# NVlabs/InstantSplat

Hardware: AMD Instinct MI355X
Metric: train_iters_per_sec (higher is better)
Workload: dtype f32

## Files before the change

### instantsplat_amd/csrc/api.hip

```cpp
#include <stdio.h>
#include "common.h"
#include <dlfcn.h>
#include <cstdlib>

int gs_launch_preprocess_fwd(hipStream_t, int, int, int, const float*, const float*, const float*, const float*, const float*, const float*,
                             const float*, const float*, const CamParams&, int32_t*, GsRec*, float*, uint2*, uint8_t*, float*, uint8_t*,
                             const GsPosed&, const GsPrologue&);
int gs_launch_count_tiles(hipStream_t, int, int, int, const uint2*, uint32_t*, uint32_t*, uint32_t*);
int gs_launch_preprocess_bwd(hipStream_t, int, int, int, const float*, const float*, const float*, const float*, const float*, int, int,
                             const CamParams&, const int32_t*, const GsRec*, const float*, const uint8_t*, const GsGrad*, float*, float*,
                             float*, float*, float*, float*, float*, float*, float*, const GsPosed&, float*, bool);
int gs_launch_mark_visible(hipStream_t, int, const float*, const float*, uint8_t*);
int gs_launch_scan_tiles(hipStream_t, int, const uint32_t*, uint32_t*, int32_t*, uint32_t*, uint32_t*, uint32_t*, uint32_t*, int);
int gs_launch_binning(hipStream_t, int, int, int, const float*, const uint2*, const uint32_t*, uint32_t*, uint64_t*, uint32_t*, uint32_t,
                      const uint32_t*, const uint32_t*, const uint32_t*);
int gs_launch_composite_fwd(hipStream_t, int, int, int, int, uint32_t, const uint32_t*, const uint32_t*, const GsRec*, const float*,
                            float*, float*, uint32_t*, const uint32_t*, const uint32_t*, const uint32_t*, uint4*, float4*, uint32_t,
                            const uint32_t*, unsigned long long*, uint32_t, uint32_t*, unsigned long long*, bool);
int gs_launch_composite_bwd(hipStream_t, int, int, int, uint32_t, const uint32_t*, const uint32_t*, const GsRec*, const float*,
                            const float*, const uint32_t*, const float*, GsGrad*, const float*, const uint4*,
                            const float4*, const uint32_t*, uint32_t, bool, const unsigned long long*, uint32_t, const uint32_t*,
                            unsigned long long*, const uint32_t*, float*);
int gs_launch_det_prepare(hipStream_t, int, int, int, uint32_t, const uint32_t*, const uint32_t*, const uint2*, char*, uint32_t*, float*);
int gs_launch_det_gather(hipStream_t, int, uint32_t, const char*, const float*, GsGrad*);
int gs_launch_frame_stats(hipStream_t, int, int, int, int, const uint32_t*, const uint32_t*, int64_t*);

namespace {
constexpr int PROF_KINDS = 6, PROF_MAX = 8192;
struct ProfState {
  bool on = false;
  unsigned long long* work_counters = nullptr;
  hipEvent_t ev[PROF_KINDS][PROF_MAX][2];
  int created[PROF_KINDS] = {};
  int used[PROF_KINDS] = {};
  int period = 1;
  int seen[PROF_KINDS] = {};
} g_prof;
}

GsProfScope::GsProfScope(int kind, hipStream_t stream) : s(stream) {
  if (!g_prof.on || kind < 0 || kind >= PROF_KINDS || g_prof.used[kind] >= PROF_MAX) return;
  if (g_prof.seen[kind]++ % g_prof.period != 0) return;
  const int i = g_prof.used[kind];
  if (i >= g_prof.created[kind]) {
    if (hipEventCreate(&g_prof.ev[kind][i][0]) != hipSuccess || hipEventCreate(&g_prof.ev[kind][i][1]) != hipSuccess) return;
    g_prof.created[kind] = i + 1;
  }
  (void)hipEventRecord(g_prof.ev[kind][i][0], s);
  stop = g_prof.ev[kind][i][1];
  g_prof.used[kind] = i + 1;
  active = true;
}
GsProfScope::~GsProfScope() { if (active) (void)hipEventRecord(stop, s); }
typedef GsProfScope ProfScope;

bool g_ranges_on = false;
thread_local bool g_krange_open = false;
namespace {
struct Roctx {
  int (*push)(const char*) = nullptr;
  int (*pop)() = nullptr;
  bool tried = false;
  unsigned long long pushed = 0;
} g_roctx;
bool roctx_open() {
  if (!g_roctx.tried) {
    g_roctx.tried = true;
    for (const char* name : {"librocprofiler-sdk-roctx.so", "librocprofiler-sdk-roctx.so.1", "libroctx64.so", "libroctx64.so.4"}) {
      void* h = dlopen(name, RTLD_NOW | RTLD_GLOBAL);
      if (!h) continue;
      g_roctx.push = (int (*)(const char*))dlsym(h, "roctxRangePushA");
      g_roctx.pop = (int (*)())dlsym(h, "roctxRangePop");
      if (g_roctx.push && g_roctx.pop) break;
      g_roctx.push = nullptr; g_roctx.pop = nullptr;
    }
  }
  return g_roctx.push != nullptr;
}
struct RoctxEnv {
  RoctxEnv() { const char* e = getenv("MI355GS_ROCTX"); if (e && e[0] == '1' && roctx_open()) g_ranges_on = true; }
} g_roctx_env;
}
void gs_range_push(const char* name) { ++g_roctx.pushed; (void)g_roctx.push(name); }
void gs_range_pop() { (void)g_roctx.pop(); }

void gs_log_error(const char* where, const char* what) { fprintf(stderr, "[mi355gs] %s failed: %s\n", where, what); }

static int g_scale_grad_exact = 0;
static int g_deterministic = 0;
GsKnobs gs_knobs() { return GsKnobs{gs_min_units(), g_deterministic}; }

static CamParams make_cam(const float* view, const float* proj, const float* campos, float tanfovx, float tanfovy,
                          float scale_modifier, int W, int H) {
  CamParams cp;
  cp.view = view; cp.proj = proj; cp.campos = campos;
  cp.tanfovx = tanfovx; cp.tanfovy = tanfovy;
  cp.focal_x = W / (2.0f * tanfovx); cp.focal_y = H / (2.0f * tanfovy);
  cp.scale_modifier = scale_modifier;
  cp.scale_grad_factor = g_scale_grad_exact ? scale_modifier : 1.0f;
  cp.W = W; cp.H = H;
  cp.gx = (W + GS_TILE - 1) / GS_TILE; cp.gy = (H + GS_TILE - 1) / GS_TILE;
  return cp;
}

static inline uint32_t clamp_capacity(int64_t c) { return c <= 0 ? 0u : (c > 0x7fffffffLL ? 0x7fffffffu : (uint32_t)c); }

namespace {
__global__ void k_view_consts(float* consts) {
  const int i = threadIdx.x;
  if (i < 16) consts[i] = (i % 5 == 0) ? 1.f : 0.f;
  else if (i < 19) consts[i] = 0.f;
}
}
int gs_write_view_consts(hipStream_t stream, float* consts, const char* name) {
  const int debug = 0;
  GS_KRANGE(name);
  hipLaunchKernelGGL(k_view_consts, dim3(1), dim3(64), 0, stream, consts);
  GS_CHECK_LAUNCH(name);
  return MI355GS_OK;
}


int gs_frame_project(hipStream_t stream, const GsScene& sc, const GsView& vw, const GsFrameBufs& fb, const GsFrameCtx& cx,
                     int32_t* num_rendered, uint8_t* visible, int debug) {
  GsRange range("mi355gs_raster_forward_preprocess");
  const int P = sc.P, D = sc.D, M = sc.M, W = vw.W, H = vw.H;
  if (P < 0 || W <= 0 || H <= 0 || W > 65535 * GS_TILE || H > 65535 * GS_TILE || D < 0 || D > 3) return MI355GS_EINVAL;
  if (!fb.geom || !fb.tiles || !num_rendered || !vw.view || !vw.proj || !vw.campos) return MI355GS_EINVAL;
  if (P > 0 && (!sc.means3D || !sc.opacities || !fb.radii)) return MI355GS_EINVAL;
  if (P > 0 && ((sc.shs == nullptr) == (sc.colors_precomp == nullptr))) return MI355GS_EINVAL;
  if (P > 0 && sc.shs && M < (D + 1) * (D + 1)) return MI355GS_EINVAL;
  if (sc.shs_rest && (!sc.shs || M < 2)) return MI355GS_EINVAL;
  if (P > 0 && !sc.cov3D_precomp && (!sc.scales || !sc.rotations)) return MI355GS_EINVAL;
  const GeomLayout gl(P);
  const TilesLayout tl(W, H);
  char* g = (char*)fb.geom;
  char* t = (char*)fb.tiles;
  GsPrologue pro;
  if (cx.prologue) {
    pro = *cx.prologue;
  } else {
    pro.tile_counters = (uint32_t*)(t + tl.count); pro.n_counters = (int)((tl.start - tl.count) / 4);
    if (fb.grad_scratch) { pro.grad_records = (float4*)fb.grad_scratch; pro.n_vec = gs_grad_gate_offset(P) / 16 + 2; }
    if (P <= 0) {
      if (hipMemsetAsync(t + tl.count, 0, tl.start - tl.count, stream) != hipSuccess) return MI355GS_ELAUNCH;
      if (fb.grad_scratch && hipMemsetAsync(fb.grad_scratch, 0, gs_grad_gate_offset(P) + 32, stream) != hipSuccess) return MI355GS_ELAUNCH;
    }
  }
  const CamParams cp = make_cam(vw.view, vw.proj, vw.campos, vw.tanfovx, vw.tanfovy, sc.scale_modifier, W, H);
  GS_KRANGE("preprocess_fwd");
  gs_launch_preprocess_fwd(stream, P, D, M, sc.means3D, sc.shs, sc.shs_rest, sc.colors_precomp, sc.opacities, sc.scales, sc.rotations,
                           sc.cov3D_precomp, cp, fb.radii, (GsRec*)(g + gl.rec), (float*)(g + gl.cov3D), (uint2*)(g + gl.rect),
                           (uint8_t*)(g + gl.clamped), (float*)(g + gl.depth), visible, cx.posed, pro);
  GS_CHECK_LAUNCH("preprocess_fwd");
  GS_KRANGE("count_tiles");
  gs_launch_count_tiles(stream, P, tl.T, tl.gx, (const uint2*)(g + gl.rect), (uint32_t*)(t + tl.count), (uint32_t*)(g + gl.bin_entries),
                        (uint32_t*)(g + gl.bin_n));
  GS_CHECK_LAUNCH("count_tiles");
  GS_KRANGE("scan_tiles");
  gs_launch_scan_tiles(stream, tl.T, (const uint32_t*)(t + tl.count), (uint32_t*)(t + tl.start), num_rendered,
                       (uint32_t*)(t + tl.order), (uint32_t*)(t + tl.meta), (uint32_t*)(t + tl.seg_first), (uint32_t*)(t + tl.part_first),
                       fb.knobs.min_units);
  GS_CHECK_LAUNCH("scan_tiles");
  return MI355GS_OK;
}

int gs_frame_render(hipStream_t stream, int P, const GsView& vw, const GsFrameBufs& fb, const float* bg, float* out_color, bool train,
                    int debug) {
  GsRange range(train ? "mi355gs_raster_forward_render" : "mi355gs_raster_forward_render_only");
  const int W = vw.W, H = vw.H;
  if (P < 0 || W <= 0 || H <= 0 || !fb.geom || !fb.tiles || !bg || !out_color) return MI355GS_EINVAL;
  const uint32_t cap = clamp_capacity(fb.capacity);
  if (cap > 0 && !fb.binning) return MI355GS_EINVAL;
  const GeomLayout gl(P);
  const TilesLayout tl(W, H);
  const BinningLayout bl(fb.capacity, tl.T, fb.knobs);
  const char* g = (const char*)fb.geom;
  char* t = (char*)fb.tiles;
  char* b = (char*)fb.binning;
  GS_KRANGE("binning");
  gs_launch_binning(stream, P, tl.T, tl.gx, (const float*)(g + gl.depth), (const uint2*)(g + gl.rect),
                    (const uint32_t*)(t + tl.start), (uint32_t*)(t + tl.cursor), (uint64_t*)(b + bl.keys),
                    (uint32_t*)(b + bl.list), cap, (const uint32_t*)(t + tl.order), (const uint32_t*)(g + gl.bin_entries),
                    (const uint32_t*)(g + gl.bin_n));
  GS_CHECK_LAUNCH("binning");
  {
    ProfScope prof(train ? 0 : 2, stream);
    GS_KRANGE("composite_fwd");
    gs_launch_composite_fwd(stream, tl.T, tl.gx, W, H, cap, (const uint32_t*)(t + tl.start), (const uint32_t*)(b + bl.list),
                            (const GsRec*)(g + gl.rec), bg, out_color, (float*)(t + tl.final_T), (uint32_t*)(t + tl.n_contrib),
                            (const uint32_t*)(t + tl.order), (const uint32_t*)(t + tl.seg_first), (const uint32_t*)(t + tl.part_first),
                            train ? (uint4*)(b + bl.unit_tile) : nullptr, train ? (float4*)(b + bl.bstate) : nullptr, bl.max_units,
                            (const uint32_t*)(t + tl.meta), train ? (unsigned long long*)(b + bl.hitmask) : nullptr, bl.max_chunks,
                            (uint32_t*)(t + tl.qmax), train ? g_prof.work_counters : nullptr, train);
  }
  GS_CHECK_LAUNCH("composite_fwd");
  return MI355GS_OK;
}

int gs_frame_backward(hipStream_t stream, const GsScene& sc, const GsView& vw, const GsFrameBufs& fb, const GsFrameCtx& cx,
                      const float* bg, const float* out_color, const float* dL_dpix, const GsGradOut& o, bool grad_scratch_is_clear,
                      int debug) {
  GsRange range("mi355gs_raster_backward");
  const int P = sc.P, D = sc.D, W = vw.W, H = vw.H;
  if (P < 0 || W <= 0 || H <= 0 || D < 0 || D > 3) return MI355GS_EINVAL;
  if (!fb.geom || !fb.tiles || !dL_dpix || !out_color || !fb.grad_scratch || !bg || !vw.view || !vw.proj || !vw.campos) return MI355GS_EINVAL;
  const bool outs = !(cx.pose_only && cx.posed.pose);
  if (P > 0 && (!sc.means3D || !fb.radii || (outs && (!o.means3D || !o.means2D || !o.opacities)))) return MI355GS_EINVAL;
  const int use_shs = sc.shs != nullptr, use_cov = sc.cov3D_precomp != nullptr;
  if (P > 0 && outs && use_shs && !o.shs) return MI355GS_EINVAL;
  if (sc.shs_rest && !use_shs) return MI355GS_EINVAL;
  if (P > 0 && outs && !use_shs && !o.colors) return MI355GS_EINVAL;
  if (P > 0 && !use_cov && (!sc.scales || !sc.rotations || (outs && (!o.scales || !o.rotations)))) return MI355GS_EINVAL;
  if (P > 0 && outs && use_cov && !o.cov3D) return MI355GS_EINVAL;
  if (P == 0) return MI355GS_OK;
  const uint32_t cap = clamp_capacity(fb.capacity);
  if (cap > 0 && !fb.binning) return MI355GS_EINVAL;
  const GeomLayout gl(P);
  const TilesLayout tl(W, H);
  const BinningLayout bl(fb.capacity, tl.T, fb.knobs);
  const char* g = (const char*)fb.geom;
  const char* t = (const char*)fb.tiles;
  char* b = (char*)fb.binning;
  GsGrad* grads = (GsGrad*)fb.grad_scratch;
  const size_t clear_bytes = cx.gate_tail ? gs_grad_gate_offset(P) + 8 * sizeof(float) : (size_t)P * sizeof(GsGrad);
  if (!cx.prologue && !grad_scratch_is_clear && hipMemsetAsync(grads, 0, clear_bytes, stream) != hipSuccess) return MI355GS_ELAUNCH;
  if (cap > 0) {
    const bool det = fb.knobs.det != 0;
    char* det_scratch = (char*)fb.grad_scratch + gs_grad_gate_offset(P) + 256;
    uint32_t* rowidx = det ? (uint32_t*)(b + bl.det_rowidx) : nullptr;
    float* rows = det ? (float*)(b + bl.det_rows) : nullptr;
    if (det) {
      GS_KRANGE("det_prepare");
      const int rc = gs_launch_det_prepare(stream, P, tl.T, tl.gx, cap, (const uint32_t*)(t + tl.start), (const uint32_t*)(b + bl.list),
                                           (const uint2*)(g + gl.rect), det_scratch, rowidx, rows);
      GS_CHECK_LAUNCH("det_prepare");
      if (rc != 0) return MI355GS_ELAUNCH;
    }
    {
      ProfScope prof(1, stream);
      GS_KRANGE("composite_bwd");
      gs_launch_composite_bwd(stream, tl.gx, W, H, cap, (const uint32_t*)(t + tl.start), (const uint32_t*)(b + bl.list),
                              (const GsRec*)(g + gl.rec), bg, (const float*)(t + tl.final_T), (const uint32_t*)(t + tl.n_contrib),
                              dL_dpix, grads, out_color, (const uint4*)(b + bl.unit_tile),
                              (const float4*)(b + bl.bstate), (const uint32_t*)(t + tl.meta), bl.max_units, bl.may_loop,
                              (const unsigned long long*)(b + bl.hitmask), bl.max_chunks, (const uint32_t*)(t + tl.qmax),
                              det ? nullptr : g_prof.work_counters, rowidx, rows);
    }
    GS_CHECK_LAUNCH("composite_bwd");
    if (det) {
      GS_KRANGE("det_gather");
      gs_launch_det_gather(stream, P, cap, det_scratch, rows, grads);
      GS_CHECK_LAUNCH("det_gather");
    }
  }
  const CamParams cp = make_cam(vw.view, vw.proj, vw.campos, vw.tanfovx, vw.tanfovy, sc.scale_modifier, W, H);
  GS_KRANGE("preprocess_bwd");
  gs_launch_preprocess_bwd(stream, P, D, sc.M, sc.means3D, sc.shs, sc.shs_rest, sc.scales, sc.rotations, use_shs, use_cov, cp, fb.radii,
                           (const GsRec*)(g + gl.rec), (const float*)(g + gl.cov3D), (const uint8_t*)(g + gl.clamped), grads, o.means3D,
                           o.means2D, o.shs, o.shs_rest, o.colors, o.opacities, o.scales, o.rotations, o.cov3D, cx.posed, cx.gate,
                           cx.pose_only);
  GS_CHECK_LAUNCH("preprocess_bwd");
  return MI355GS_OK;
}

extern "C" {

int mi355gs_abi_version(void) { return MI355GS_ABI_VERSION; }

const char* mi355gs_error_string(int code) {
  switch (code) {
    case MI355GS_OK: return "ok";
    case MI355GS_EINVAL: return "invalid argument";
    case MI355GS_ELAUNCH: return "HIP launch or runtime failure";
    case MI355GS_EOVERFLOW: return "instance capacity exceeded";
    default: return "unknown error";
  }
}

size_t mi355gs_raster_geom_bytes(int P) { return GeomLayout(P).total; }
size_t mi355gs_raster_tiles_bytes(int W, int H) { return (W > 0 && H > 0) ? TilesLayout(W, H).total : 0; }
size_t mi355gs_raster_binning_bytes(int64_t n, int W, int H) { return (W > 0 && H > 0) ? gs_binning_bytes(n, W, H, gs_knobs(), true) : 0; }
size_t mi355gs_raster_binning_bytes_render_only(int64_t n, int W, int H) { return (W > 0 && H > 0) ? gs_binning_bytes(n, W, H, gs_knobs(), false) : 0; }
size_t mi355gs_raster_grad_gate_offset(int P) { return gs_grad_gate_offset(P); }
size_t mi355gs_raster_grad_scratch_bytes(int P) { return gs_grad_scratch_bytes(P, g_deterministic); }

int mi355gs_raster_forward_preprocess(void* stream, int P, int D, int M, int W, int H, const float* means3D, const float* shs,
                                      const float* shs_rest, const float* colors_precomp, const float* opacities, const float* scales,
                                      float scale_modifier, const float* rotations, const float* cov3D_precomp,
                                      const float* viewmatrix, const float* projmatrix, const float* campos, float tanfovx,
                                      float tanfovy, int prefiltered, int32_t* radii, void* geom, void* tiles,
                                      int32_t* num_rendered, uint8_t* visible, void* grad_scratch, int debug) {
  (void)prefiltered;
  return gs_frame_project((hipStream_t)stream, {P, D, M, means3D, shs, shs_rest, colors_precomp, opacities, scales, rotations, cov3D_precomp, scale_modifier},
                          {W, H, viewmatrix, projmatrix, campos, tanfovx, tanfovy}, {geom, tiles, nullptr, 0, radii, grad_scratch, gs_knobs()},
                          GsFrameCtx(), num_rendered, visible, debug);
}

int mi355gs_raster_forward_render(void* stream, int P, int W, int H, int64_t capacity, const float* bg, const void* geom,
                                  void* tiles, void* binning, float* out_color, int debug) {
  return gs_frame_render((hipStream_t)stream, P, {W, H}, {const_cast<void*>(geom), tiles, binning, capacity, nullptr, nullptr, gs_knobs()}, bg,
                         out_color, true, debug);
}

int mi355gs_raster_forward_render_only(void* stream, int P, int W, int H, int64_t capacity, const float* bg, const void* geom,
                                       void* tiles, void* binning, float* out_color, int debug) {
  return gs_frame_render((hipStream_t)stream, P, {W, H}, {const_cast<void*>(geom), tiles, binning, capacity, nullptr, nullptr, gs_knobs()}, bg,
                         out_color, false, debug);
}

int mi355gs_raster_backward(void* stream, int P, int D, int M, int W, int H, const float* bg, const float* means3D,
                            const float* shs, const float* shs_rest, const float* colors_precomp, const float* opacities, const float* scales,
                            float scale_modifier, const float* rotations, const float* cov3D_precomp, const float* viewmatrix,
                            const float* projmatrix, const float* campos, float tanfovx, float tanfovy, const void* geom,
                            void* tiles, const void* binning, int64_t capacity, const int32_t* radii, const float* out_color,
                            const float* dL_dpix, void* grad_scratch, float* dL_dmeans3D, float* dL_dmeans2D, float* dL_dshs,
                            float* dL_dshs_rest, float* dL_dcolors, float* dL_dopacities, float* dL_dscales, float* dL_drotations, float* dL_dcov3D,
                            int grad_scratch_is_clear, int debug) {
  const GsGradOut o = {dL_dmeans3D, dL_dmeans2D, dL_dshs, dL_dshs_rest, dL_dcolors, dL_dopacities, dL_dscales, dL_drotations, dL_dcov3D};
  return gs_frame_backward((hipStream_t)stream, {P, D, M, means3D, shs, shs_rest, colors_precomp, opacities, scales, rotations, cov3D_precomp, scale_modifier},
                           {W, H, viewmatrix, projmatrix, campos, tanfovx, tanfovy},
                           {const_cast<void*>(geom), tiles, const_cast<void*>(binning), capacity, const_cast<int32_t*>(radii), grad_scratch, gs_knobs()},
                           GsFrameCtx(), bg, out_color, dL_dpix, o, grad_scratch_is_clear != 0, debug);
}

int mi355gs_tune_deterministic(int on) {
  const int old = g_deterministic;
  if (on >= 0) g_deterministic = on ? 1 : 0;
  return old;
}

int mi355gs_tune_scale_grad(int mode) {
  const int old = g_scale_grad_exact;
  if (mode >= 0) g_scale_grad_exact = mode ? 1 : 0;
  return old;
}

int mi355gs_raster_frame_stats(void* stream_, int W, int H, const void* tiles, int64_t* stats) {
  GS_RANGE();
  hipStream_t stream = (hipStream_t)stream_;
  const int debug = 0;
  if (W <= 0 || H <= 0 || !tiles || !stats) return MI355GS_EINVAL;
  const TilesLayout tl(W, H);
  const char* t = (const char*)tiles;
  if (hipMemsetAsync(stats, 0, 2 * sizeof(int64_t), stream) != hipSuccess) return MI355GS_ELAUNCH;
  GS_KRANGE("frame_stats");
  gs_launch_frame_stats(stream, tl.T, tl.gx, W, H, (const uint32_t*)(t + tl.start), (const uint32_t*)(t + tl.n_contrib), stats);
  GS_CHECK_LAUNCH("frame_stats");
  return MI355GS_OK;
}

int mi355gs_profile_begin(void) {
  g_prof.on = true;
  for (int k = 0; k < PROF_KINDS; ++k) g_prof.used[k] = g_prof.seen[k] = 0;
  return MI355GS_OK;
}

int mi355gs_profile_set_period(int every) {
  const int old = g_prof.period;
  if (every > 0) g_prof.period = every;
  return old;
}

int mi355gs_profile_work_counters(void* counters) {
  g_prof.work_counters = (unsigned long long*)counters;
  return MI355GS_OK;
}

int mi355gs_profile_read(int kind, double* total_ms, int* launches) {
  if (kind < 0 || kind >= PROF_KINDS || !total_ms || !launches) return MI355GS_EINVAL;
  double tot = 0.0;
  for (int i = 0; i < g_prof.used[kind]; ++i) {
    float ms = 0.f;
    if (hipEventSynchronize(g_prof.ev[kind][i][1]) != hipSuccess) return MI355GS_ELAUNCH;
    if (hipEventElapsedTime(&ms, g_prof.ev[kind][i][0], g_prof.ev[kind][i][1]) != hipSuccess) return MI355GS_ELAUNCH;
    tot += ms;
  }
  *total_ms = tot;
  *launches = g_prof.used[kind];
  return MI355GS_OK;
}

int mi355gs_profile_end(void) {
  g_prof.on = false;
  return MI355GS_OK;
}

int mi355gs_profile_ranges(int on) {
  if (on == 1) {
    if (!roctx_open()) return MI355GS_EINVAL;
    g_ranges_on = true;
  } else if (on == 0) {
    g_ranges_on = false;
  }
  return (int)(g_roctx.pushed & 0x7fffffffull);
}

int mi355gs_raster_mark_visible(void* stream_, int P, const float* means3D, const float* viewmatrix, const float* projmatrix,
                                uint8_t* present) {
  GS_RANGE();
  (void)projmatrix;
  const int debug = 0;
  void* stream = stream_;
  if (P < 0 || (P > 0 && (!means3D || !viewmatrix || !present))) return MI355GS_EINVAL;
  GS_KRANGE("mark_visible");
  gs_launch_mark_visible((hipStream_t)stream, P, means3D, viewmatrix, present);
  GS_CHECK_LAUNCH("mark_visible");
  return MI355GS_OK;
}

}
```

### instantsplat_amd/csrc/binning.hip

```cpp
#include "common.h"

namespace {

constexpr int SCAN_THREADS = 1024;
constexpr size_t SCAN_STAGE_MAX_BYTES = 48 * 1024;
constexpr int SORT_THREADS = 256;
constexpr int SORT_SMALL_CAP = GS_SORT_SMALL_CAP;
constexpr int SORT_LDS_CAP = 8192;

#ifdef GS_SCAN_PROBE
__device__ long long g_scan_probe[16];
#define SCAN_STAMP(k) do { if (threadIdx.x == 0) g_scan_probe[k] = wall_clock64(); } while (0)
#else
#define SCAN_STAMP(k) do { } while (0)
#endif
constexpr int SCAN_PER_MAX = (int)(SCAN_STAGE_MAX_BYTES / (SCAN_THREADS * 4));

template <bool STAGED>
__global__ __launch_bounds__(SCAN_THREADS) void k_scan_tiles(int T, const uint32_t* count, uint32_t* start, int32_t* num_rendered,
                                                               uint32_t* __restrict__ order, uint32_t* __restrict__ meta,
                                                               uint32_t* __restrict__ seg_first, uint32_t* __restrict__ part_first,
                                                               uint32_t min_units) {
  __shared__ uint32_t wave_tot[SCAN_THREADS / GS_WAVE];
  HIP_DYNAMIC_SHARED(uint32_t, s_stage)
  const int tid = threadIdx.x, lane = tid & 63, wave = tid >> 6;
  const int per = (T + SCAN_THREADS - 1) / SCAN_THREADS;
  const int lo = tid * per, hi = min(T, lo + per);
  SCAN_STAMP(0);
  uint32_t own[STAGED ? SCAN_PER_MAX : 1];
  if constexpr (STAGED) {
    for (int e = tid; e < T; e += SCAN_THREADS) s_stage[e] = count[e];
    __syncthreads();
#pragma unroll
    for (int k = 0; k < SCAN_PER_MAX; ++k) own[k] = lo + k < hi ? s_stage[lo + k] : 0u;
  }
  auto for_own = [&](auto&& f) {
    if constexpr (STAGED) {
#pragma unroll
      for (int k = 0; k < SCAN_PER_MAX; ++k)
        if (lo + k < hi) f(lo + k, own[k]);
    } else {
      for (int i = lo; i < hi; ++i) f(i, count[i]);
    }
  };
  auto emit = [&](uint32_t* out, auto&& value) {
    if constexpr (STAGED) {
      __syncthreads();
      for_own([&](int i, uint32_t c) { s_stage[i] = value(i, c); });
      __syncthreads();
      for (int e = tid; e < T; e += SCAN_THREADS) out[e] = s_stage[e];
    } else {
      for_own([&](int i, uint32_t c) { out[i] = value(i, c); });
    }
  };
  SCAN_STAMP(1);
  uint32_t local = 0;
  for_own([&](int, uint32_t c) { local += c; });
  const uint32_t incl = gs_wave_scan_incl_u32(local);
  if (lane == 63) wave_tot[wave] = incl;
  __syncthreads();
  uint32_t wave_off = 0, total = 0;
#pragma unroll
  for (int w = 0; w < SCAN_THREADS / GS_WAVE; ++w) {
    const uint32_t v = wave_tot[w];
    if (w < wave) wave_off += v;
    total += v;
  }
  SCAN_STAMP(2);
  if (order) {
    __shared__ uint32_t hist[SCAN_THREADS];
    __shared__ uint32_t s_max;
    uint32_t mx = 0;
    for_own([&](int, uint32_t c) { mx = max(mx, c); });
    mx = gs_wave_max_u32(mx);
    hist[tid] = 0u;
    if (tid == 0) s_max = 0u;
    __syncthreads();
    if (lane == 0) atomicMax(&s_max, mx);
    __syncthreads();
    const uint32_t cmax = max(s_max, 1u);
    const float bscale = (float)(SCAN_THREADS - 1) / (float)cmax;
    auto bucket = [&](uint32_t c) { return (uint32_t)(SCAN_THREADS - 1) - min((uint32_t)(SCAN_THREADS - 1), (uint32_t)((float)c * bscale)); };
    SCAN_STAMP(3);
    for_own([&](int, uint32_t c) { atomicAdd(&hist[bucket(c)], 1u); });
    __syncthreads();
    SCAN_STAMP(4);
    const uint32_t h = hist[tid];
    const uint32_t hi_ = gs_wave_scan_incl_u32(h);
    __shared__ uint32_t hist_wave[SCAN_THREADS / GS_WAVE];
    if (lane == 63) hist_wave[wave] = hi_;
    __syncthreads();
    uint32_t hoff = 0;
#pragma unroll
    for (int w = 0; w < SCAN_THREADS / GS_WAVE; ++w)
      if (w < wave) hoff += hist_wave[w];
    hist[tid] = hoff + hi_ - h;
    __syncthreads();
    SCAN_STAMP(5);
    if constexpr (STAGED) {
      for_own([&](int i, uint32_t c) { s_stage[atomicAdd(&hist[bucket(c)], 1u)] = (uint32_t)i; });
      __syncthreads();
      for (int e = tid; e < T; e += SCAN_THREADS) order[e] = s_stage[e];
    } else {
      for_own([&](int i, uint32_t c) { order[atomicAdd(&hist[bucket(c)], 1u)] = (uint32_t)i; });
    }
    __syncthreads();
    SCAN_STAMP(6);
  }
  if (seg_first) {
    const uint32_t level = (uint32_t)gs_unit_level_for((long long)total, (long long)min_units);
    const uint32_t chunks = 1u << level;
    const uint32_t seg_len = chunks * GS_SEG;
    static_assert((GS_SEG & (GS_SEG - 1)) == 0, "GS_SEG must be a power of two");
    const uint32_t seg_shift = level + (uint32_t)__builtin_ctz(GS_SEG), seg_mask = seg_len - 1u;
    auto units_of = [&](uint32_t c) { return (c + seg_mask) >> seg_shift; };
    auto short_of = [&](uint32_t c) { return (uint32_t)((c & seg_mask) != 0u); };
    uint32_t lseg = 0, lpart = 0;
    for_own([&](int, uint32_t c) { lseg += units_of(c); lpart += short_of(c); });
    const uint32_t iseg = gs_wave_scan_incl_u32(lseg), ipart = gs_wave_scan_incl_u32(lpart);
    __shared__ uint32_t seg_wave[SCAN_THREADS / GS_WAVE];
    __shared__ uint32_t part_wave[SCAN_THREADS / GS_WAVE];
    if (lane == 63) { seg_wave[wave] = iseg; part_wave[wave] = ipart; }
    __syncthreads();
    uint32_t soff = 0, stot = 0, poff = 0, ptot = 0;
#pragma unroll
    for (int w = 0; w < SCAN_THREADS / GS_WAVE; ++w) {
      if (w < wave) { soff += seg_wave[w]; poff += part_wave[w]; }
      stot += seg_wave[w]; ptot += part_wave[w];
    }
    uint32_t srun = soff + iseg - lseg, prun = poff + ipart - lpart;
    emit(seg_first, [&](int, uint32_t c) { const uint32_t v = srun; srun += units_of(c); return v; });
    emit(part_first, [&](int, uint32_t c) { const uint32_t v = prun; prun += short_of(c); return v; });
    if (tid == 0) { part_first[T] = ptot; meta[3] = ptot; }
    if (tid == 0) { seg_first[T] = stot; meta[1] = stot; meta[2] = chunks; }
  }
  SCAN_STAMP(7);
  uint32_t run = wave_off + incl - local;
  emit(start, [&](int, uint32_t c) { const uint32_t v = run; run += c; return v; });
  if (tid == 0) {
    start[T] = total;
    *num_rendered = (int32_t)total;
  }
  SCAN_STAMP(8);
}

constexpr int SCAN_CHUNK = 4096;

template <bool RECT>
__device__ __forceinline__ uint32_t scan_input(const uint32_t* __restrict__ in, int i, int n) {
  if (i >= n) return 0u;
  if constexpr (!RECT) return in[i];
  else {
    if (i == n - 1) return 0u;
    const uint2 r = reinterpret_cast<const uint2*>(in)[i];
    const int x0 = r.x & 0xffff, y0 = r.x >> 16, x1 = r.y & 0xffff, y1 = r.y >> 16;
    return (x1 > x0 && y1 > y0) ? (uint32_t)((x1 - x0) * (y1 - y0)) : 0u;
  }
}

template <bool RECT>
__global__ __launch_bounds__(256) void k_scan_block_sums(int n, const uint32_t* __restrict__ in, uint32_t* __restrict__ sums) {
  __shared__ uint32_t s_red[4];
  const int base = blockIdx.x * SCAN_CHUNK;
  uint32_t acc = 0;
  for (int i = threadIdx.x; i < SCAN_CHUNK; i += 256) acc += scan_input<RECT>(in, base + i, n);
#pragma unroll
  for (int m = 32; m >= 1; m >>= 1) acc += __shfl_xor(acc, m);
  if ((threadIdx.x & 63) == 0) s_red[threadIdx.x >> 6] = acc;
  __syncthreads();
  if (threadIdx.x == 0) sums[blockIdx.x] = s_red[0] + s_red[1] + s_red[2] + s_red[3];
}

template <bool RECT>
__global__ __launch_bounds__(256) void k_scan_apply(int n, const uint32_t* __restrict__ in, const uint32_t* __restrict__ block_off,
                                                    uint32_t* __restrict__ out) {
  __shared__ uint32_t s_wave[4];
  const int tid = threadIdx.x, lane = tid & 63, wave = tid >> 6;
  uint32_t run = block_off[blockIdx.x];
  for (int it = 0; it < SCAN_CHUNK / 256; ++it) {
    const int i = blockIdx.x * SCAN_CHUNK + it * 256 + tid;
    const uint32_t v = scan_input<RECT>(in, i, n);
    const uint32_t incl = gs_wave_scan_incl_u32(v);
    __syncthreads();
    if (lane == 63) s_wave[wave] = incl;
    __syncthreads();
    uint32_t woff = 0;
#pragma unroll
    for (int w = 0; w < 4; ++w) woff += w < wave ? s_wave[w] : 0u;
    if (i < n) out[i] = run + woff + incl - v;
    run += s_wave[0] + s_wave[1] + s_wave[2] + s_wave[3];
  }
}

constexpr int BIN_CHUNK = GS_BIN_CHUNK;
static_assert(BIN_CHUNK == 512, "two Gaussians per thread (own_depth selection in k_scatter_lds)");
constexpr int BIN_MAX_LDS_TILES = 16384;
static_assert(BIN_MAX_LDS_TILES <= 64 * 256, "k_count_tiles_lds keeps one bit per bin of a thread in a 64-bit mask");

__device__ __forceinline__ bool unpack_rect(uint2 r, int& x0, int& y0, int& x1, int& y1) {
  x0 = r.x & 0xffff; y0 = r.x >> 16; x1 = r.y & 0xffff; y1 = r.y >> 16;
  return x1 > x0 && y1 > y0;
}

constexpr int BIN_WIDE = 8;

constexpr int BIN_PER_THREAD = BIN_CHUNK / 256;

template <class F>
__device__ __forceinline__ void for_each_instance(int lo, int hi, const uint2 (&own)[BIN_PER_THREAD], const uint2* __restrict__ rects,
                                                  uint32_t* s_wide, uint2* s_wide_rect, uint32_t* s_nwide, F&& f) {
  const int tid = threadIdx.x;
#pragma unroll
  for (int j = 0; j < BIN_PER_THREAD; ++j) {
    const int i = lo + tid + 256 * j;
    int x0, y0, x1, y1;
    if (i >= hi || !unpack_rect(own[j], x0, y0, x1, y1)) continue;
    if ((x1 - x0) * (y1 - y0) > BIN_WIDE) {
      const uint32_t slot = atomicAdd(s_nwide, 1u);
      s_wide[slot] = (uint32_t)i; s_wide_rect[slot] = own[j];
      continue;
    }
    for (int y = y0; y < y1; ++y)
      for (int x = x0; x < x1; ++x) f(i, j, x, y);
  }
  __syncthreads();
  const int nwide = (int)*s_nwide;
  for (int q = tid >> 4; q < nwide; q += 16) {
    const int i = (int)s_wide[q];
    int x0, y0, x1, y1;
    unpack_rect(s_wide_rect[q], x0, y0, x1, y1);
    const int w = x1 - x0, n = w * (y1 - y0);
    const int dq = 16 / w, dr = 16 - dq * w;
    int j = tid & 15, row = j / w, col = j - row * w;
    for (; j < n; j += 16) {
      f(i, -1, x0 + col, y0 + row);
      col += dr; row += dq;
      if (col >= w) { col -= w; row += 1; }
    }
  }
}

__global__ __launch_bounds__(256) void k_count_tiles_lds(int P, int T, int gx, const uint2* __restrict__ rects,
                                                          uint32_t* __restrict__ tile_count, uint32_t* __restrict__ entries,
                                                          uint32_t* __restrict__ entry_n) {
  HIP_DYNAMIC_SHARED(uint32_t, s_bins)
  __shared__ uint32_t s_wide[BIN_CHUNK];
  __shared__ uint2 s_wide_rect[BIN_CHUNK];
  __shared__ uint32_t s_nwide;
  __shared__ uint32_t s_wave_nz[4];
  const int tid = threadIdx.x;
  const int lo = blockIdx.x * BIN_CHUNK, hi = min(P, lo + BIN_CHUNK);
  uint2 own[BIN_PER_THREAD];
#pragma unroll
  for (int j = 0; j < BIN_PER_THREAD; ++j) own[j] = rects[min(lo + tid + 256 * j, P - 1)];
  for (int t = tid; t < T; t += 256) s_bins[t] = 0;
  if (tid == 0) s_nwide = 0;
  __syncthreads();
  for_each_instance(lo, hi, own, rects, s_wide, s_wide_rect, &s_nwide, [&](int, int, int x, int y) { atomicAdd(&s_bins[y * gx + x], 1u); });
  __syncthreads();
  unsigned long long mask = 0ull;
  {
    int k = 0;
    for (int t = tid; t < T; t += 256, ++k) {
      const uint32_t c = s_bins[t];
      if (c) { atomicAdd(&tile_count[t], c); mask |= 1ull << k; }
    }
  }
  const uint32_t nz = (uint32_t)__popcll(mask);
  const uint32_t incl = gs_wave_scan_incl_u32(nz);
  if ((tid & 63) == 63) s_wave_nz[tid >> 6] = incl;
  __syncthreads();
  uint32_t off = incl - nz, total = 0;
#pragma unroll
  for (int w = 0; w < 4; ++w) {
    if (w < (tid >> 6)) off += s_wave_nz[w];
    total += s_wave_nz[w];
  }
  if (tid == 0) entry_n[blockIdx.x] = total <= (uint32_t)GS_BIN_ENTRIES ? total : 0xffffffffu;
  if (total > (uint32_t)GS_BIN_ENTRIES) return;
  uint32_t* mine = entries + (size_t)blockIdx.x * GS_BIN_ENTRIES + off;
  while (mask) {
    const int t = tid + 256 * (__ffsll((long long)mask) - 1);
    mask &= mask - 1ull;
    *mine++ = (uint32_t)t | (s_bins[t] << 16);
  }
}

__global__ __launch_bounds__(256) void k_scatter_lds(int P, int T, int gx, const float* __restrict__ depths,
                                                      const uint2* __restrict__ rects, const uint32_t* __restrict__ start,
                                                      uint32_t* __restrict__ cursor, uint64_t* __restrict__ keys, uint32_t capacity,
                                                      const uint32_t* __restrict__ entries, const uint32_t* __restrict__ entry_n) {
  HIP_DYNAMIC_SHARED(uint32_t, s_bins)
  __shared__ uint32_t s_wide[BIN_CHUNK];
  __shared__ uint2 s_wide_rect[BIN_CHUNK];
  __shared__ uint32_t s_nwide;
  const int tid = threadIdx.x;
  const int lo = blockIdx.x * BIN_CHUNK, hi = min(P, lo + BIN_CHUNK);
  uint2 own[BIN_PER_THREAD];
  uint32_t own_depth[BIN_PER_THREAD];
#pragma unroll
  for (int j = 0; j < BIN_PER_THREAD; ++j) {
    const int ic = min(lo + tid + 256 * j, P - 1);
    own[j] = rects[ic];
    own_depth[j] = __float_as_uint(depths[ic]);
  }
  const uint32_t n_entries = entry_n[blockIdx.x];
  if (n_entries != 0xffffffffu) {
    const uint32_t* mine = entries + (size_t)blockIdx.x * GS_BIN_ENTRIES;
    for (uint32_t e0 = 0; e0 < n_entries; e0 += 1024) {
      uint32_t en[4], r[4], st[4];
#pragma unroll
      for (int j = 0; j < 4; ++j) {
        const uint32_t e = e0 + tid + 256 * j;
        en[j] = e < n_entries ? mine[e] : 0u;
      }
#pragma unroll
      for (int j = 0; j < 4; ++j) {
        r[j] = 0u; st[j] = 0u;
        if (en[j]) { r[j] = atomicAdd(&cursor[en[j] & 0xffffu], en[j] >> 16); st[j] = start[en[j] & 0xffffu]; }
      }
#pragma unroll
      for (int j = 0; j < 4; ++j)
        if (en[j]) s_bins[en[j] & 0xffffu] = st[j] + r[j];
    }
  } else {
    for (int t = tid; t < T; t += 256) s_bins[t] = 0;
    if (tid == 0) s_nwide = 0;
    __syncthreads();
    for_each_instance(lo, hi, own, rects, s_wide, s_wide_rect, &s_nwide, [&](int, int, int x, int y) { atomicAdd(&s_bins[y * gx + x], 1u); });
    __syncthreads();
    for (int t0 = 0; t0 < T; t0 += 1024) {
      uint32_t c[4], r[4], st[4];
#pragma unroll
      for (int j = 0; j < 4; ++j) {
        const int t = t0 + tid + 256 * j;
        c[j] = t < T ? s_bins[t] : 0u;
      }
#pragma unroll
      for (int j = 0; j < 4; ++j) {
        const int t = t0 + tid + 256 * j;
        r[j] = 0u; st[j] = 0u;
        if (c[j]) { r[j] = atomicAdd(&cursor[t], c[j]); st[j] = start[t]; }
      }
#pragma unroll
      for (int j = 0; j < 4; ++j)
        if (c[j]) s_bins[t0 + tid + 256 * j] = st[j] + r[j];
    }
  }
  if (tid == 0) s_nwide = 0;
  __syncthreads();
  for_each_instance(lo, hi, own, rects, s_wide, s_wide_rect, &s_nwide, [&](int i, int j, int x, int y) {
    const uint32_t depth = j == 0 ? own_depth[0] : (j == 1 ? own_depth[BIN_PER_THREAD - 1] : __float_as_uint(depths[i]));
    const uint64_t key = ((uint64_t)depth << 32) | (uint32_t)i;
    const uint32_t pos = atomicAdd(&s_bins[y * gx + x], 1u);
    if (pos < capacity) keys[pos] = key;
  });
}

__global__ __launch_bounds__(256) void k_count_tiles_direct(int P, int gx, const uint2* __restrict__ rects,
                                                             uint32_t* __restrict__ tile_count) {
  const int i = blockIdx.x * blockDim.x + threadIdx.x;
  if (i >= P) return;
  int x0, y0, x1, y1;
  if (!unpack_rect(rects[i], x0, y0, x1, y1)) return;
  for (int y = y0; y < y1; ++y)
    for (int x = x0; x < x1; ++x) atomicAdd(&tile_count[y * gx + x], 1u);
}

__global__ __launch_bounds__(256) void k_scatter_direct(int P, int gx, const float* __restrict__ depths, const uint2* __restrict__ rects,
                                                         const uint32_t* __restrict__ start, uint32_t* __restrict__ cursor,
                                                         uint64_t* __restrict__ keys, uint32_t capacity) {
  const int i = blockIdx.x * blockDim.x + threadIdx.x;
  if (i >= P) return;
  int x0, y0, x1, y1;
  if (!unpack_rect(rects[i], x0, y0, x1, y1)) return;
  const uint64_t key = ((uint64_t)__float_as_uint(depths[i]) << 32) | (uint32_t)i;
  for (int y = y0; y < y1; ++y)
    for (int x = x0; x < x1; ++x) {
      const int t = y * gx + x;
      const uint32_t pos = start[t] + atomicAdd(&cursor[t], 1u);
      if (pos < capacity) keys[pos] = key;
    }
}

template <class KeyPtr>
__device__ __forceinline__ void bitonic_sort_any(KeyPtr a, int n, int tid, int nthreads) {
  int np2 = 1;
  while (np2 < n) np2 <<= 1;
  const int half = np2 >> 1;
  for (int k = 2; k <= np2; k <<= 1) {
    const int hk = k >> 1;
    for (int t = tid; t < half; t += nthreads) {
      const int blk = t / hk, off = t - blk * hk;
      const int i = blk * k + off, j = blk * k + (k - 1 - off);
      if (j < n) {
        const uint64_t x = a[i], y = a[j];
        if (x > y) { a[i] = y; a[j] = x; }
      }
    }
    __syncthreads();
    for (int d = hk >> 1; d >= 1; d >>= 1) {
      for (int t = tid; t < half; t += nthreads) {
        const int i = (t / d) * (2 * d) + (t % d), j = i + d;
        if (j < n) {
          const uint64_t x = a[i], y = a[j];
          if (x > y) { a[i] = y; a[j] = x; }
        }
      }
      __syncthreads();
    }
  }
}

template <int CTRL>
__device__ __forceinline__ uint32_t sort_dpp(uint32_t v) {
  return (uint32_t)__builtin_amdgcn_update_dpp(0, (int)v, CTRL, 0xF, 0xF, true);
}
template <int LM>
__device__ __forceinline__ uint32_t lane_xchg32(uint32_t v) {
  if constexpr (LM >= 16) return (uint32_t)__builtin_amdgcn_ds_bpermute((int)(((threadIdx.x & 63) ^ LM) << 2), (int)v);
  else if constexpr (LM == 1) return sort_dpp<0xB1>(v);
  else if constexpr (LM == 2) return sort_dpp<0x4E>(v);
  else if constexpr (LM == 3) return sort_dpp<0x1B>(v);
  else if constexpr (LM == 4) {
    const int lo = __builtin_amdgcn_update_dpp(0, (int)v, 0x104, 0xF, 0x5, false);
    return (uint32_t)__builtin_amdgcn_update_dpp(lo, (int)v, 0x114, 0xF, 0xA, false);
  }
  else if constexpr (LM == 7) return sort_dpp<0x141>(v);
  else if constexpr (LM == 8) return sort_dpp<0x128>(v);
  else {
    static_assert(LM == 15, "lane mask of a bitonic network inside a wave64");
    return sort_dpp<0x140>(v);
  }
}
template <int LM>
__device__ __forceinline__ uint64_t lane_xchg64(uint64_t v) {
  return ((uint64_t)lane_xchg32<LM>((uint32_t)(v >> 32)) << 32) | lane_xchg32<LM>((uint32_t)v);
}

template <int E, int KK>
__device__ __forceinline__ void sort_flip_stage(uint64_t (&k)[E], uint64_t* __restrict__ s_keys, int base) {
  constexpr int m = KK - 1;
  if constexpr (KK <= E) {
#pragma unroll
    for (int e = 0; e < E; ++e) {
      const int pe = e ^ (m & (E - 1));
      if (e < pe) { const uint64_t a = k[e], b = k[pe]; if (a > b) { k[e] = b; k[pe] = a; } }
    }
  } else if constexpr (KK <= 64 * E) {
    constexpr int lm = (m / E) & 63;
    uint64_t other[E];
#pragma unroll
    for (int e = 0; e < E; ++e) other[e] = lane_xchg64<lm>(k[E - 1 - e]);
    const bool lower = (base & (KK >> 1)) == 0;
#pragma unroll
    for (int e = 0; e < E; ++e) { const uint64_t a = k[e], b = other[e]; k[e] = ((b < a) == lower) ? b : a; }
  } else {
    __syncthreads();
#pragma unroll
    for (int e = 0; e < E; ++e) s_keys[base + e] = k[e];
    __syncthreads();
    const bool lower = (base & (KK >> 1)) == 0;
#pragma unroll
    for (int e = 0; e < E; ++e) { const uint64_t a = k[e], b = s_keys[(base + e) ^ m]; k[e] = ((b < a) == lower) ? b : a; }
  }
}

template <int E, int D>
__device__ __forceinline__ void sort_disperse_from(uint64_t (&k)[E], uint64_t* __restrict__ s_keys, int base) {
  if constexpr (D >= 1) {
    if constexpr (D < E) {
#pragma unroll
      for (int e = 0; e < E; ++e) {
        const int pe = e ^ D;
        if (e < pe) { const uint64_t a = k[e], b = k[pe]; if (a > b) { k[e] = b; k[pe] = a; } }
      }
    } else if constexpr (D < 64 * E) {
      const bool lower = (base & D) == 0;
#pragma unroll
      for (int e = 0; e < E; ++e) { const uint64_t a = k[e], b = lane_xchg64<D / E>(a); k[e] = ((b < a) == lower) ? b : a; }
    } else {
      __syncthreads();
#pragma unroll
      for (int e = 0; e < E; ++e) s_keys[base + e] = k[e];
      __syncthreads();
      const bool lower = (base & D) == 0;
#pragma unroll
      for (int e = 0; e < E; ++e) { const uint64_t a = k[e], b = s_keys[(base + e) ^ D]; k[e] = ((b < a) == lower) ? b : a; }
    }
    sort_disperse_from<E, D / 2>(k, s_keys, base);
  }
}

template <int E, int KK, int NP2>
__device__ __forceinline__ void sort_merge_from(uint64_t (&k)[E], uint64_t* __restrict__ s_keys, int base) {
  if constexpr (KK <= NP2) {
    sort_flip_stage<E, KK>(k, s_keys, base);
    sort_disperse_from<E, KK / 4>(k, s_keys, base);
    sort_merge_from<E, KK * 2, NP2>(k, s_keys, base);
  }
}

template <int E>
__device__ __forceinline__ void sort_tile_regs(uint64_t* __restrict__ s_keys, const uint64_t* keys, uint32_t* __restrict__ list,
                                               uint32_t s, int n, uint64_t* keys_out = nullptr) {
  const int tid = threadIdx.x, lane = tid & 63, wave = tid >> 6;
  const int base = wave * (64 * E) + lane * E;
  uint64_t k[E];
#pragma unroll
  for (int e = 0; e < E; ++e) k[e] = (base + e < n) ? keys[s + base + e] : ~0ull;
  sort_merge_from<E, 2, SORT_THREADS * E>(k, s_keys, base);
  if (keys_out) {
#pragma unroll
    for (int e = 0; e < E; ++e)
      if (base + e < n) keys_out[s + base + e] = k[e];
  } else {
#pragma unroll
    for (int e = 0; e < E; ++e)
      if (base + e < n) list[s + base + e] = (uint32_t)k[e];
  }
}

template <int NMAX>
__device__ __forceinline__ uint32_t sort_count_below(const uint64_t* __restrict__ run, int n, uint64_t key) {
  int lo = 0;
#pragma unroll
  for (int step = NMAX; step >= 1; step >>= 1)
    if (lo + step <= n && run[lo + step - 1] < key) lo += step;
  return (uint32_t)lo;
}
template <int EA, int EB>
__device__ __forceinline__ void sort_tile_two_runs(uint64_t* __restrict__ s_keys, const uint64_t* keys, uint32_t* __restrict__ list,
                                                   uint32_t s, int n) {
  constexpr int NA = SORT_THREADS * EA, NBMAX = SORT_THREADS * EB;
  static_assert(NA + NBMAX <= SORT_SMALL_CAP, "both sorted runs are parked in the kernel's LDS array");
  const int tid = threadIdx.x, lane = tid & 63, wave = tid >> 6;
  const int base_a = wave * (64 * EA) + lane * EA, base_b = wave * (64 * EB) + lane * EB, nb = n - NA;
  uint64_t ka[EA], kb[EB];
#pragma unroll
  for (int e = 0; e < EA; ++e) ka[e] = keys[s + base_a + e];
#pragma unroll
  for (int e = 0; e < EB; ++e) kb[e] = (base_b + e < nb) ? keys[s + NA + base_b + e] : ~0ull;
  sort_merge_from<EA, 2, NA>(ka, s_keys, base_a);
  sort_merge_from<EB, 2, NBMAX>(kb, s_keys, base_b);
  __syncthreads();
#pragma unroll
  for (int e = 0; e < EA; ++e) s_keys[base_a + e] = ka[e];
#pragma unroll
  for (int e = 0; e < EB; ++e) s_keys[NA + base_b + e] = kb[e];
  __syncthreads();
#pragma unroll
  for (int e = 0; e < EA; ++e) list[s + base_a + e + sort_count_below<NBMAX>(s_keys + NA, nb, ka[e])] = (uint32_t)ka[e];
#pragma unroll
  for (int e = 0; e < EB; ++e)
    if (base_b + e < nb) list[s + base_b + e + sort_count_below<NA>(s_keys, NA, kb[e])] = (uint32_t)kb[e];
}

__device__ __forceinline__ void sort_long_tile(uint64_t* __restrict__ s_keys, uint64_t* keys, uint32_t* __restrict__ list, uint32_t s, int n) {
  constexpr int RUN = SORT_SMALL_CAP, E = RUN / SORT_THREADS;
  const int nrun = (n + RUN - 1) / RUN, tid = threadIdx.x;
  for (int r = 0; r < nrun; ++r) {
    __syncthreads();
    sort_tile_regs<E>(s_keys, keys, list, s + (uint32_t)r * RUN, min(RUN, n - r * RUN), keys);
  }
  for (int r = 0; r < nrun; ++r) {
    const int rn = min(RUN, n - r * RUN);
    uint64_t k[E];
    uint32_t rank[E];
    __syncthreads();
#pragma unroll
    for (int e = 0; e < E; ++e) {
      const int i = tid * E + e;
      k[e] = i < rn ? keys[s + (uint32_t)r * RUN + i] : ~0ull;
      rank[e] = (uint32_t)i;
    }
    for (int r2 = 0; r2 < nrun; ++r2) {
      if (r2 == r) continue;
      const int n2 = min(RUN, n - r2 * RUN);
      __syncthreads();
      for (int i = tid; i < n2; i += SORT_THREADS) s_keys[i] = keys[s + (uint32_t)r2 * RUN + i];
      __syncthreads();
#pragma unroll
      for (int e = 0; e < E; ++e) {
        int lo = 0, hi = n2;
        while (lo < hi) {
          const int mid = (lo + hi) >> 1;
          if (s_keys[mid] < k[e]) lo = mid + 1; else hi = mid;
        }
        rank[e] += (uint32_t)lo;
      }
    }
#pragma unroll
    for (int e = 0; e < E; ++e)
      if (tid * E + e < rn) list[s + rank[e]] = (uint32_t)k[e];
  }
}

__device__ __forceinline__ void sort_one_tile(int tile, const uint32_t* __restrict__ start, uint64_t* keys,
                                              uint32_t* __restrict__ list, uint32_t capacity) {
  __shared__ uint64_t s_keys[SORT_SMALL_CAP];
  const uint32_t s = min(start[tile], capacity), e = min(start[tile + 1], capacity);
  const int n = (int)(e - s);
  if (n <= 0) return;
  if (n <= SORT_THREADS) sort_tile_regs<1>(s_keys, keys, list, s, n);
  else if (n <= SORT_THREADS * 2) sort_tile_regs<2>(s_keys, keys, list, s, n);
  else if (n <= SORT_THREADS * 3) sort_tile_two_runs<2, 1>(s_keys, keys, list, s, n);
  else if (n <= SORT_THREADS * 4) sort_tile_regs<4>(s_keys, keys, list, s, n);
  else if (n <= SORT_THREADS * 5) sort_tile_two_runs<4, 1>(s_keys, keys, list, s, n);
  else if (n <= SORT_THREADS * 6) sort_tile_two_runs<4, 2>(s_keys, keys, list, s, n);
  else if (n <= SORT_SMALL_CAP) sort_tile_regs<8>(s_keys, keys, list, s, n);
  else if (n <= SORT_LDS_CAP) sort_long_tile(s_keys, keys, list, s, n);
  else {
    uint64_t* seg = keys + s;
    bitonic_sort_any(seg, n, (int)threadIdx.x, SORT_THREADS);
    for (int i = threadIdx.x; i < n; i += SORT_THREADS) list[s + i] = (uint32_t)seg[i];
  }
}

__global__ __launch_bounds__(SORT_THREADS) void k_sort_tiles(int T, const uint32_t* __restrict__ start, uint64_t* keys,
                                                              uint32_t* __restrict__ list, uint32_t capacity,
                                                              const uint32_t* __restrict__ order) {
  sort_one_tile((int)order[blockIdx.x], start, keys, list, capacity);
}

}

static int g_min_units = GS_MIN_UNITS;
extern "C" int mi355gs_tune_min_units(int min_units) {
  const int old = g_min_units;
  if (min_units > 0) g_min_units = min_units;
  return old;
}
int gs_min_units() { return g_min_units; }

int gs_launch_scan_tiles(hipStream_t stream, int T, const uint32_t* count, uint32_t* start, int32_t* num_rendered, uint32_t* order,
                         uint32_t* meta, uint32_t* seg_first, uint32_t* part_first, int min_units) {
  const size_t stage_bytes = (size_t)((T + SCAN_THREADS - 1) / SCAN_THREADS) * SCAN_THREADS * 4;
  if (T > SCAN_THREADS && stage_bytes <= SCAN_STAGE_MAX_BYTES)
    hipLaunchKernelGGL(k_scan_tiles<true>, dim3(1), dim3(SCAN_THREADS), stage_bytes, stream, T, count, start, num_rendered, order, meta,
                       seg_first, part_first, (uint32_t)min_units);
  else
    hipLaunchKernelGGL(k_scan_tiles<false>, dim3(1), dim3(SCAN_THREADS), 0, stream, T, count, start, num_rendered, order, meta, seg_first,
                       part_first, (uint32_t)min_units);
  return 0;
}

template <bool RECT>
static int scan_large(hipStream_t stream, int n, const uint32_t* in, uint32_t* out, uint32_t* block_sums, int32_t* total) {
  const int nb = (n + SCAN_CHUNK - 1) / SCAN_CHUNK;
  hipLaunchKernelGGL(k_scan_block_sums<RECT>, dim3(nb), dim3(256), 0, stream, n, in, block_sums);
  hipLaunchKernelGGL(k_scan_tiles<false>, dim3(1), dim3(SCAN_THREADS), 0, stream, nb, (const uint32_t*)block_sums, block_sums, total,
                     (uint32_t*)nullptr, (uint32_t*)nullptr, (uint32_t*)nullptr, (uint32_t*)nullptr, 0u);
  hipLaunchKernelGGL(k_scan_apply<RECT>, dim3(nb), dim3(256), 0, stream, n, in, (const uint32_t*)block_sums, out);
  return 0;
}
int gs_launch_scan_large(hipStream_t stream, int n, const uint32_t* in, uint32_t* out, uint32_t* block_sums, int32_t* total) {
  return scan_large<false>(stream, n, in, out, block_sums, total);
}
int gs_launch_scan_rect_areas(hipStream_t stream, int P, const uint2* rects, uint32_t* off, uint32_t* block_sums, int32_t* total) {
  return scan_large<true>(stream, P + 1, reinterpret_cast<const uint32_t*>(rects), off, block_sums, total);
}

int gs_launch_count_tiles(hipStream_t stream, int P, int T, int gx, const uint2* rects, uint32_t* tile_count, uint32_t* entries,
                          uint32_t* entry_n) {
  if (P <= 0) return 0;
  if (T <= BIN_MAX_LDS_TILES) {
    GsProfScope prof(5, stream);
    hipLaunchKernelGGL(k_count_tiles_lds, dim3((P + BIN_CHUNK - 1) / BIN_CHUNK), dim3(256), (size_t)T * 4, stream, P, T, gx, rects, tile_count,
                       entries, entry_n);
  }
  else
    hipLaunchKernelGGL(k_count_tiles_direct, dim3((P + 255) / 256), dim3(256), 0, stream, P, gx, rects, tile_count);
  return 0;
}

int gs_launch_binning(hipStream_t stream, int P, int T, int gx, const float* depths, const uint2* rects, const uint32_t* start,
                      uint32_t* cursor, uint64_t* keys, uint32_t* list, uint32_t capacity, const uint32_t* order, const uint32_t* entries,
                      const uint32_t* entry_n) {
  if (P <= 0 || capacity == 0) return 0;
  if (T <= BIN_MAX_LDS_TILES)
    hipLaunchKernelGGL(k_scatter_lds, dim3((P + BIN_CHUNK - 1) / BIN_CHUNK), dim3(256), (size_t)T * 4, stream, P, T, gx, depths, rects,
                       start, cursor, keys, capacity, entries, entry_n);
  else
    hipLaunchKernelGGL(k_scatter_direct, dim3((P + 255) / 256), dim3(256), 0, stream, P, gx, depths, rects, start, cursor, keys, capacity);
  {
    GsProfScope prof(4, stream);
    hipLaunchKernelGGL(k_sort_tiles, dim3(T), dim3(SORT_THREADS), 0, stream, T, start, keys, list, capacity, order);
  }
  return 0;
}
```

### instantsplat_amd/csrc/common.h

```cpp
#pragma once
#include <hip/hip_runtime.h>
#include <stdint.h>
#include <stddef.h>
#include "../../include/mi355gs.h"
#include <type_traits>

#define GS_LOG2E 1.4426950408889634f
#define GS_TILE 16
#define GS_TILE_PIX 256
#define GS_WAVE 64

struct alignas(16) GsRec {
  float4 q0;
  float4 q1;
  float4 q2;
};

struct alignas(16) GsGrad {
  float4 g0;
  float4 g1;
  float4 g2;
};

static inline size_t gs_align(size_t x) { return (x + 255) & ~(size_t)255; }

struct GsCarver {
  char* base;
  size_t off = 0;
  template <class T> T* take(size_t n) {
    T* p = base ? (T*)(base + off) : nullptr;
    off += gs_align(n * sizeof(T));
    return p;
  }
};
int gs_write_view_consts(hipStream_t stream, float* consts, const char* name);

constexpr int GS_BIN_CHUNK = 512;
constexpr int GS_BIN_ENTRIES = 1024;

struct GeomLayout {
  size_t rec, cov3D, rect, clamped, depth, bin_entries, bin_n, total;
  __host__ explicit GeomLayout(int P) {
    size_t n = P > 0 ? (size_t)P : 1, o = 0;
    rec = o; o += gs_align(n * sizeof(GsRec));
    cov3D = o; o += gs_align(n * 6 * sizeof(float));
    rect = o; o += gs_align(n * sizeof(uint2));
    clamped = o; o += gs_align(n);
    depth = o; o += gs_align(n * sizeof(float));
    const size_t chunks = (n + GS_BIN_CHUNK - 1) / GS_BIN_CHUNK;
    bin_entries = o; o += gs_align(chunks * GS_BIN_ENTRIES * sizeof(uint32_t));
    bin_n = o; o += gs_align(chunks * sizeof(uint32_t));
    total = o;
  }
};

constexpr int GS_SORT_SMALL_CAP = 2048;

constexpr int GS_UNIT_LEVELS = 4;
__host__ __device__ inline int gs_unit_level_for(long long instances, long long min_units) {
  int level = 0;
  while (level + 1 < GS_UNIT_LEVELS && (instances >> (7 + level)) >= min_units) ++level;
  return level;
}
struct GsKnobs {
  int min_units;
  int det;
};
GsKnobs gs_knobs();
struct DetScratchLayout {
  size_t off, block_sums, total;
  __host__ explicit DetScratchLayout(int P) {
    const size_t n = (size_t)(P > 0 ? P : 1) + 1;
    size_t o = 0;
    off = o; o += gs_align((n + 1) * 4);
    block_sums = o; o += gs_align(((n + 4095) / 4096 + 2) * 4);
    total = o;
  }
};
int gs_min_units();
constexpr int GS_MIN_UNITS = 40960;

struct TilesLayout {
  size_t count, start, cursor, final_T, n_contrib, order, seg_first, part_first, meta, qmax, total;
  int gx, gy, T;
  __host__ TilesLayout(int W, int H) {
    gx = (W + GS_TILE - 1) / GS_TILE; gy = (H + GS_TILE - 1) / GS_TILE; T = gx * gy;
    size_t o = 0, npix = (size_t)W * H;
    count = o; o += gs_align((size_t)T * 4);
    cursor = o; o += gs_align((size_t)T * 4);
    start = o; o += gs_align(((size_t)T + 1) * 4);
    final_T = o; o += gs_align(npix * 4);
    n_contrib = o; o += gs_align(npix * 4);
    order = o; o += gs_align((size_t)T * 4);
    seg_first = o; o += gs_align(((size_t)T + 1) * 4);
    part_first = o; o += gs_align(((size_t)T + 1) * 4);
    meta = o; o += gs_align(16);
    qmax = o; o += gs_align((size_t)T * 4 * 4);
    total = o;
  }
};

constexpr int GS_SEG = 64;

struct BinningLayout {
  size_t keys, list, unit_tile, bstate, hitmask, det_rows, det_rowidx, total;
  uint32_t max_chunks;
  uint32_t max_units;
  bool may_loop;
  __host__ BinningLayout(int64_t R, int T, const GsKnobs& knobs) {
    size_t n = R > 0 ? (size_t)R : 1, o = 0;
    keys = o; o += gs_align(n * 8);
    list = o; o += gs_align(n * 4);
    const size_t mu = (size_t)knobs.min_units, top = (size_t)GS_SEG << (GS_UNIT_LEVELS - 1);
    const size_t by_chunks = (n + GS_SEG - 1) / GS_SEG, by_rule = 2 * mu + 1, by_top = (n + top - 1) / top;
    const size_t lim = by_chunks < by_rule ? by_chunks : by_rule;
    may_loop = gs_unit_level_for((long long)n, (long long)mu) > 0;
    max_units = (uint32_t)((lim > by_top ? lim : by_top) + (size_t)(T > 0 ? T : 1));
    unit_tile = o; o += gs_align((size_t)max_units * 16);
    bstate = o; o += gs_align((size_t)max_units * 256 * sizeof(float4));
    max_chunks = (uint32_t)(by_chunks + 8 * (size_t)(T > 0 ? T : 1) + 8);
    hitmask = o; o += gs_align((size_t)max_chunks * 4 * sizeof(uint64_t));
    det_rows = det_rowidx = o;
    if (knobs.det) {
      det_rows = o; o += gs_align(n * sizeof(GsGrad));
      det_rowidx = o; o += gs_align(n * 4);
    }
    total = o;
  }
};


__device__ __forceinline__ float3 gs_tp43(const float* m, float3 p) {
  return make_float3(m[0] * p.x + m[4] * p.y + m[8] * p.z + m[12], m[1] * p.x + m[5] * p.y + m[9] * p.z + m[13],
                     m[2] * p.x + m[6] * p.y + m[10] * p.z + m[14]);
}
__device__ __forceinline__ float4 gs_tp44(const float* m, float3 p) {
  return make_float4(m[0] * p.x + m[4] * p.y + m[8] * p.z + m[12], m[1] * p.x + m[5] * p.y + m[9] * p.z + m[13],
                     m[2] * p.x + m[6] * p.y + m[10] * p.z + m[14], m[3] * p.x + m[7] * p.y + m[11] * p.z + m[15]);
}

struct CamParams {
  const float* view;
  const float* proj;
  const float* campos;
  float tanfovx, tanfovy, focal_x, focal_y, scale_modifier;
  float scale_grad_factor;
  int W, H, gx, gy;
};

template <int CTRL, int ROW_MASK = 0xF, class T>
__device__ __forceinline__ T gs_dpp(T v) {
  static_assert(sizeof(T) == 4 || sizeof(T) == 8, "one or two 32-bit moves");
  uint32_t w[sizeof(T) / 4];
  __builtin_memcpy(w, &v, sizeof(T));
  for (size_t i = 0; i < sizeof(T) / 4; ++i) w[i] = (uint32_t)__builtin_amdgcn_update_dpp(0, (int)w[i], CTRL, ROW_MASK, 0xF, false);
  __builtin_memcpy(&v, w, sizeof(T));
  return v;
}
template <class T>
__device__ __forceinline__ T gs_wave_sum_row3(T v) {
  v += gs_dpp<0xB1>(v);
  v += gs_dpp<0x4E>(v);
  v += gs_dpp<0x141>(v);
  v += gs_dpp<0x140>(v);
  v += gs_dpp<0x142, 0xA>(v);
  v += gs_dpp<0x143, 0xC>(v);
  return v;
}
__device__ __forceinline__ double gs_wave_sum_row3_f64(double v) { return gs_wave_sum_row3(v); }

__device__ __forceinline__ void gs_finish_two_means(int nblocks, double inv_n, const float* __restrict__ partial, float& mean0, float& mean1) {
  __shared__ double s_a[16], s_b[16];
  double a = 0.0, b = 0.0;
  for (int i = threadIdx.x; i < nblocks; i += 1024) { a += (double)partial[2 * i]; b += (double)partial[2 * i + 1]; }
  a = gs_wave_sum_row3(a); b = gs_wave_sum_row3(b);
  if ((threadIdx.x & 63) == 63) { s_a[threadIdx.x >> 6] = a; s_b[threadIdx.x >> 6] = b; }
  __syncthreads();
  if (threadIdx.x != 0) return;
  double ta = 0.0, tb = 0.0;
  for (int w = 0; w < 16; ++w) { ta += s_a[w]; tb += s_b[w]; }
  mean0 = (float)(ta * inv_n); mean1 = (float)(tb * inv_n);
}
__device__ __forceinline__ float gs_l1_ssim_loss(float lambda_dssim, float l1_mean, float ssim_mean) {
  return (1.0f - lambda_dssim) * l1_mean + lambda_dssim * (1.0f - ssim_mean);
}

typedef float gs_v2f __attribute__((vector_size(8)));
__device__ __forceinline__ gs_v2f gs_fma2(gs_v2f a, gs_v2f b, gs_v2f c) { return a * b + c; }

__device__ __forceinline__ uint32_t gs_wave_max_u32(uint32_t v) {
  auto dpp = [](uint32_t x, auto ctrl) { return (uint32_t)__builtin_amdgcn_update_dpp(0, (int)x, decltype(ctrl)::value, 0xF, 0xF, true); };
  v = max(v, dpp(v, std::integral_constant<int, 0xB1>{}));
  v = max(v, dpp(v, std::integral_constant<int, 0x4E>{}));
  v = max(v, dpp(v, std::integral_constant<int, 0x141>{}));
  v = max(v, dpp(v, std::integral_constant<int, 0x140>{}));
  const auto a = __builtin_amdgcn_permlane16_swap(v, v, false, false);
  v = max(a[0], a[1]);
  const auto b = __builtin_amdgcn_permlane32_swap(v, v, false, false);
  return max(b[0], b[1]);
}

__device__ __forceinline__ uint32_t gs_wave_scan_incl_u32(uint32_t v) {
  auto up = [](uint32_t x, auto ctrl, auto rows) {
    return (uint32_t)__builtin_amdgcn_update_dpp(0, (int)x, decltype(ctrl)::value, decltype(rows)::value, 0xF, false);
  };
  using all = std::integral_constant<int, 0xF>;
  v += up(v, std::integral_constant<int, 0x111>{}, all{});
  v += up(v, std::integral_constant<int, 0x112>{}, all{});
  v += up(v, std::integral_constant<int, 0x114>{}, all{});
  v += up(v, std::integral_constant<int, 0x118>{}, all{});
  v += up(v, std::integral_constant<int, 0x142>{}, std::integral_constant<int, 0xA>{});
  v += up(v, std::integral_constant<int, 0x143>{}, std::integral_constant<int, 0xC>{});
  return v;
}

__device__ __forceinline__ float gs_sum_rows(float v) {
  const unsigned u = __float_as_uint(v);
  const auto a = __builtin_amdgcn_permlane16_swap(u, u, false, false);
  const float s = __uint_as_float(a[0]) + __uint_as_float(a[1]);
  const unsigned w = __float_as_uint(s);
  const auto b = __builtin_amdgcn_permlane32_swap(w, w, false, false);
  return __uint_as_float(b[0]) + __uint_as_float(b[1]);
}

__device__ __forceinline__ uint32_t gs_physical_cu() {
  const uint32_t hw = __builtin_amdgcn_s_getreg(4 | (31 << 11));
  const uint32_t xcc = __builtin_amdgcn_s_getreg(20 | (3 << 11));
  return ((xcc & 7u) << 6) | (((hw >> 13) & 3u) << 4) | ((hw >> 8) & 15u);
}

extern thread_local bool g_krange_open;
void gs_range_pop();
#define GS_CHECK_LAUNCH(name)                                                   \
  do {                                                                          \
    if (g_krange_open) { g_krange_open = false; gs_range_pop(); }               \
    hipError_t e_ = hipGetLastError();                                          \
    if (e_ == hipSuccess && debug) e_ = hipStreamSynchronize((hipStream_t)stream); \
    if (e_ != hipSuccess) {                                                     \
      gs_log_error(name, hipGetErrorString(e_));                                \
      return MI355GS_ELAUNCH;                                                   \
    }                                                                           \
  } while (0)

void gs_log_error(const char* where, const char* what);

extern bool g_ranges_on;
void gs_range_push(const char* name);
void gs_range_pop();
struct GsRange {
  bool active;
  explicit GsRange(const char* name) : active(g_ranges_on) { if (active) gs_range_push(name); }
  ~GsRange() { if (active) gs_range_pop(); }
  GsRange(const GsRange&) = delete;
  GsRange& operator=(const GsRange&) = delete;
};
#define GS_RANGE() GsRange gs_range_(__func__)
extern thread_local bool g_krange_open;
#define GS_KRANGE(name) do { if (g_ranges_on) { gs_range_push(name); g_krange_open = true; } } while (0)

struct GsProfScope {
  hipStream_t s; hipEvent_t stop; bool active = false;
  GsProfScope(int kind, hipStream_t stream);
  ~GsProfScope();
};


struct GsPrologue {
  float4* grad_records = nullptr; size_t n_vec = 0;
  uint32_t* tile_counters = nullptr; int n_counters = 0;
  float* g_poses = nullptr; int n_pose = 0;
  float* pose_scratch = nullptr;
  float* adam_scratch = nullptr;
};
struct GsPosed {
  const float* pose = nullptr;
  float* acc = nullptr;
  float* partial = nullptr;
};
enum { GS_GATE_XYZ = 0, GS_GATE_SH = 1, GS_GATE_SH_REST = 2, GS_GATE_OPACITY = 3, GS_GATE_SCALING = 4, GS_GATE_ROT = 5, GS_GATE_POSE = 6 };

struct GsScene {
  int P, D, M;
  const float *means3D, *shs, *shs_rest, *colors_precomp, *opacities, *scales, *rotations, *cov3D_precomp;
  float scale_modifier;
};
struct GsView {
  int W, H;
  const float *view, *proj, *campos;
  float tanfovx, tanfovy;
};
struct GsFrameBufs {
  void *geom, *tiles, *binning;
  int64_t capacity;
  int32_t* radii;
  void* grad_scratch;
  GsKnobs knobs;
};
struct GsFrameCtx {
  const GsPrologue* prologue = nullptr;
  GsPosed posed;
  float* gate = nullptr;
  bool gate_tail = false;
  bool pose_only = false;
};
struct GsGradOut { float *means3D, *means2D, *shs, *shs_rest, *colors, *opacities, *scales, *rotations, *cov3D; };
static inline size_t gs_grad_gate_offset(int P) { return gs_align((size_t)(P > 0 ? P : 1) * sizeof(GsGrad)); }
static inline size_t gs_grad_scratch_bytes(int P, int det) { return gs_grad_gate_offset(P) + 256 + (det ? DetScratchLayout(P).total : 0); }
static inline size_t gs_binning_bytes(int64_t n, int W, int H, const GsKnobs& k, bool train) {
  const BinningLayout bl(n, TilesLayout(W, H).T, k);
  return train ? bl.total : bl.unit_tile;
}
static inline const uint32_t* gs_frame_count(const void* tiles, int W, int H) {
  const TilesLayout tl(W, H);
  return (const uint32_t*)((const char*)tiles + tl.start) + tl.T;
}
int gs_frame_project(hipStream_t stream, const GsScene& sc, const GsView& vw, const GsFrameBufs& fb, const GsFrameCtx& cx,
                     int32_t* num_rendered, uint8_t* visible, int debug);
int gs_frame_render(hipStream_t stream, int P, const GsView& vw, const GsFrameBufs& fb, const float* bg, float* out_color, bool train,
                    int debug);
int gs_frame_backward(hipStream_t stream, const GsScene& sc, const GsView& vw, const GsFrameBufs& fb, const GsFrameCtx& cx,
                      const float* bg, const float* out_color, const float* dL_dpix, const GsGradOut& out, bool grad_scratch_is_clear,
                      int debug);

struct GsAdamFused {
  uint32_t* live; uint32_t seq;
  const uint32_t* commit_count; unsigned long long commit_capacity;
  uint32_t* commit_poison;
};
int gs_adam_multi(hipStream_t stream, int ntensors, const int64_t* numel, const int32_t* row, float* const* params,
                  const float* const* grads, float* const* exp_avg, float* const* exp_avg_sq, const float* const* per_point_lr,
                  const float* lr, float beta1, float beta2, float eps, const int32_t* step, float* scratch, const float* gate,
                  const int32_t* gate_index, uint32_t* live, uint32_t seq, const GsAdamFused* fused);

struct GsFrozenScene {
  int P, M, W, H;
  int64_t capacity;
  const float *xyz, *f_dc, *f_rest, *opacity, *scaling, *rotation;
  char *geom, *tiles, *binning;
  float *image, *consts;
  int32_t *radii, *num_rendered;

  bool init(int P_, int M_, int W_, int H_, int64_t capacity_, const float* xyz_, const float* f_dc_, const float* f_rest_,
            const float* opacity_, const float* scaling_, const float* rotation_, const void* workspace) {
    if (P_ <= 0 || M_ < 1 || M_ > 16 || W_ <= 0 || H_ <= 0 || W_ > 65535 * GS_TILE || H_ > 65535 * GS_TILE || capacity_ <= 0 || !workspace)
      return false;
    if (!xyz_ || !f_dc_ || (M_ > 1 && !f_rest_) || !opacity_ || !scaling_ || !rotation_) return false;
    P = P_; M = M_; W = W_; H = H_; capacity = capacity_;
    xyz = xyz_; f_dc = f_dc_; f_rest = M_ > 1 ? f_rest_ : nullptr; opacity = opacity_; scaling = scaling_; rotation = rotation_;
    return true;
  }
  void carve(GsCarver& c, const GsKnobs& knobs, bool train) {
    geom = c.take<char>(GeomLayout(P).total);
    tiles = c.take<char>(TilesLayout(W, H).total);
    binning = c.take<char>(gs_binning_bytes(capacity, W, H, knobs, train));
    image = c.take<float>(3 * (size_t)W * H);
    consts = c.take<float>(32);
    radii = c.take<int32_t>((size_t)P);
    num_rendered = c.take<int32_t>(1);
  }
  bool degree_ok(int D) const { return D >= 0 && D <= 3 && (D + 1) * (D + 1) <= M; }
  GsScene scene(int D) const {
    return {P, D, D == 0 ? 1 : M, xyz, f_dc, D == 0 ? nullptr : f_rest, nullptr, opacity, scaling, rotation, nullptr, 1.0f};
  }
  GsView view(const float* proj, float tanfovx, float tanfovy) const { return {W, H, consts, proj, consts + 16, tanfovx, tanfovy}; }
  GsFrameBufs bufs(const GsKnobs& knobs, void* grad_scratch) const { return {geom, tiles, binning, capacity, radii, grad_scratch, knobs}; }
  const uint32_t* count() const { return gs_frame_count(tiles, W, H); }
};
```

### instantsplat_amd/csrc/path.hip

```cpp
#include <stdlib.h>
#include <string.h>
#include "common.h"

namespace {

constexpr int RGB8_VEC = 4;

struct Rgb8x4 { uint32_t a, b, c; };

__device__ __forceinline__ uint32_t rgb8_quantize(float x) {
#pragma clang fp contract(off)
  const float y = x * 255.0f;
  const float z = y + 0.5f;
  return z > 0.0f ? (uint32_t)fminf(z, 255.0f) : 0u;
}

__global__ __launch_bounds__(256) void k_rgb8_from_planar(int npix, const float* __restrict__ img, uint8_t* __restrict__ out,
                                                          const uint32_t* __restrict__ count_src, int32_t* __restrict__ count_dst) {
  if (count_dst && blockIdx.x == 0 && threadIdx.x == 0) *count_dst = (int32_t)*count_src;
  const int i0 = (int)(blockIdx.x * 256u + threadIdx.x) * RGB8_VEC;
  if (i0 >= npix) return;
  const float* __restrict__ r = img;
  const float* __restrict__ g = img + npix;
  const float* __restrict__ b = img + 2 * (size_t)npix;
  if ((npix & (RGB8_VEC - 1)) == 0 && (((uintptr_t)img & 15) | ((uintptr_t)out & 3)) == 0) {
    const float4 R = reinterpret_cast<const float4*>(r)[i0 >> 2], G = reinterpret_cast<const float4*>(g)[i0 >> 2],
                 B = reinterpret_cast<const float4*>(b)[i0 >> 2];
    Rgb8x4 p;
    p.a = rgb8_quantize(R.x) | rgb8_quantize(G.x) << 8 | rgb8_quantize(B.x) << 16 | rgb8_quantize(R.y) << 24;
    p.b = rgb8_quantize(G.y) | rgb8_quantize(B.y) << 8 | rgb8_quantize(R.z) << 16 | rgb8_quantize(G.z) << 24;
    p.c = rgb8_quantize(B.z) | rgb8_quantize(R.w) << 8 | rgb8_quantize(G.w) << 16 | rgb8_quantize(B.w) << 24;
    *reinterpret_cast<Rgb8x4*>(out + 3 * (size_t)i0) = p;
  } else {
    const int i1 = min(npix, i0 + RGB8_VEC);
    for (int i = i0; i < i1; ++i) {
      out[3 * (size_t)i] = (uint8_t)rgb8_quantize(r[i]);
      out[3 * (size_t)i + 1] = (uint8_t)rgb8_quantize(g[i]);
      out[3 * (size_t)i + 2] = (uint8_t)rgb8_quantize(b[i]);
    }
  }
}

bool rgb8_size_ok(int W, int H) { return W > 0 && H > 0 && (long long)W * H <= 0x7fffffffLL - 256 * RGB8_VEC; }

int launch_rgb8(hipStream_t stream, int W, int H, const float* img, uint8_t* out, const uint32_t* count_src, int32_t* count_dst) {
  const int debug = 0;
  const int npix = W * H;
  const int per_block = 256 * RGB8_VEC;
  GS_KRANGE("rgb8_from_planar");
  hipLaunchKernelGGL(k_rgb8_from_planar, dim3((npix + per_block - 1) / per_block), dim3(256), 0, stream, npix, img, out, count_src,
                     count_dst);
  GS_CHECK_LAUNCH("rgb8_from_planar");
  return MI355GS_OK;
}

typedef GsFrozenScene Path;

size_t carve(Path& t, void* workspace) {
  GsCarver c{(char*)workspace};
  t.carve(c, gs_knobs(), false);
  return c.off;
}

}

extern "C" {

int mi355gs_rgb8_from_planar(void* stream, int H, int W, const float* img, uint8_t* out) {
  GS_RANGE();
  if (!img || !out || !rgb8_size_ok(W, H)) return MI355GS_EINVAL;
  return launch_rgb8((hipStream_t)stream, W, H, img, out, nullptr, nullptr);
}

size_t mi355gs_path_workspace_bytes(int P, int W, int H, int64_t capacity) {
  if (P <= 0 || !rgb8_size_ok(W, H) || capacity <= 0) return 0;
  Path t;
  memset(&t, 0, sizeof(t));
  t.P = P; t.W = W; t.H = H; t.capacity = capacity;
  return carve(t, nullptr);
}

void* mi355gs_path_create(int P, int M, int W, int H, int64_t capacity, const float* xyz, const float* f_dc, const float* f_rest,
                          const float* opacity, const float* scaling, const float* rotation, void* workspace) {
  if (!rgb8_size_ok(W, H)) return nullptr;
  Path* t = (Path*)calloc(1, sizeof(Path));
  if (!t) return nullptr;
  if (!t->init(P, M, W, H, capacity, xyz, f_dc, f_rest, opacity, scaling, rotation, workspace)) { free(t); return nullptr; }
  carve(*t, workspace);
  return t;
}

void mi355gs_path_destroy(void* handle) { free(handle); }

int mi355gs_path_render(void* handle, void* stream_, int sh_degree, const float* projmatrix, float tanfovx, float tanfovy,
                        const float* bg, const float* poses, int first, int n, uint8_t* frames, int32_t* counts) {
  GS_RANGE();
  Path* t = (Path*)handle;
  hipStream_t stream = (hipStream_t)stream_;
  if (!t || !t->degree_ok(sh_degree) || !projmatrix || !bg || !poses || !frames || !counts) return MI355GS_EINVAL;
  if (first < 0 || n < 0 || n > 0x7fffffff - first) return MI355GS_EINVAL;
  if (n == 0) return MI355GS_OK;
  int rc;
  if ((rc = gs_write_view_consts(stream, t->consts, "view_consts"))) return rc;
  const GsScene scene = t->scene(sh_degree);
  const GsView view = t->view(projmatrix, tanfovx, tanfovy);
  const GsFrameBufs bufs = t->bufs(gs_knobs(), nullptr);
  const size_t frame_bytes = (size_t)t->W * t->H * 3;
  for (int i = first; i < first + n; ++i) {
    GsFrameCtx cx;
    cx.posed.pose = poses + 7 * (size_t)i;
    if ((rc = gs_frame_project(stream, scene, view, bufs, cx, t->num_rendered, nullptr, 0))) return rc;
    if ((rc = gs_frame_render(stream, t->P, view, bufs, bg, t->image, false, 0))) return rc;
    if ((rc = launch_rgb8(stream, t->W, t->H, t->image, frames + frame_bytes * (size_t)i, t->count(), counts + i))) return rc;
  }
  return MI355GS_OK;
}

}
```

### instantsplat_amd/csrc/preprocess.hip

```cpp
#include "pose_math.h"

namespace {

constexpr float SH_C0 = 0.28209479177387814f;
constexpr float SH_C1 = 0.4886025119029199f;
constexpr float SH_C2_0 = 1.0925484305920792f, SH_C2_1 = -1.0925484305920792f, SH_C2_2 = 0.31539156525252005f,
                SH_C2_3 = -1.0925484305920792f, SH_C2_4 = 0.5462742152960396f;
constexpr float SH_C3_0 = -0.5900435899266435f, SH_C3_1 = 2.890611442640554f, SH_C3_2 = -0.4570457994644658f,
                SH_C3_3 = 0.3731763325901154f, SH_C3_4 = -0.4570457994644658f, SH_C3_5 = 1.445305721320277f,
                SH_C3_6 = -0.5900435899266435f;

struct Cov2D {
  float a, b, c;
};

struct Ewa {
  float tx, ty, tz, xmul, ymul;
  float M[6];
};

__device__ __forceinline__ Ewa ewa_setup(float3 pv, const float* view, const CamParams& cp) {
  Ewa e;
  const float limx = 1.3f * cp.tanfovx, limy = 1.3f * cp.tanfovy;
  const float txtz = pv.x / pv.z, tytz = pv.y / pv.z;
  e.tx = fminf(limx, fmaxf(-limx, txtz)) * pv.z;
  e.ty = fminf(limy, fmaxf(-limy, tytz)) * pv.z;
  e.tz = pv.z;
  e.xmul = (txtz < -limx || txtz > limx) ? 0.f : 1.f;
  e.ymul = (tytz < -limy || tytz > limy) ? 0.f : 1.f;
  const float j00 = cp.focal_x / e.tz, j02 = -(cp.focal_x * e.tx) / (e.tz * e.tz);
  const float j11 = cp.focal_y / e.tz, j12 = -(cp.focal_y * e.ty) / (e.tz * e.tz);
  e.M[0] = j00 * view[0] + j02 * view[2];
  e.M[1] = j00 * view[4] + j02 * view[6];
  e.M[2] = j00 * view[8] + j02 * view[10];
  e.M[3] = j11 * view[1] + j12 * view[2];
  e.M[4] = j11 * view[5] + j12 * view[6];
  e.M[5] = j11 * view[9] + j12 * view[10];
  return e;
}

__device__ __forceinline__ Cov2D ewa_cov2d(const Ewa& e, const float* cov) {
  const float* M = e.M;
  float MS[6];
  MS[0] = M[0] * cov[0] + M[1] * cov[1] + M[2] * cov[2];
  MS[1] = M[0] * cov[1] + M[1] * cov[3] + M[2] * cov[4];
  MS[2] = M[0] * cov[2] + M[1] * cov[4] + M[2] * cov[5];
  MS[3] = M[3] * cov[0] + M[4] * cov[1] + M[5] * cov[2];
  MS[4] = M[3] * cov[1] + M[4] * cov[3] + M[5] * cov[4];
  MS[5] = M[3] * cov[2] + M[4] * cov[4] + M[5] * cov[5];
  Cov2D c;
  c.a = MS[0] * M[0] + MS[1] * M[1] + MS[2] * M[2] + 0.3f;
  c.b = MS[0] * M[3] + MS[1] * M[4] + MS[2] * M[5];
  c.c = MS[3] * M[3] + MS[4] * M[4] + MS[5] * M[5] + 0.3f;
  return c;
}

__device__ __forceinline__ void quat_to_R(float r, float x, float y, float z, float* R) {
  R[0] = 1.f - 2.f * (y * y + z * z); R[1] = 2.f * (x * y - r * z); R[2] = 2.f * (x * z + r * y);
  R[3] = 2.f * (x * y + r * z); R[4] = 1.f - 2.f * (x * x + z * z); R[5] = 2.f * (y * z - r * x);
  R[6] = 2.f * (x * z - r * y); R[7] = 2.f * (y * z + r * x); R[8] = 1.f - 2.f * (x * x + y * y);
}

template <int NB>
__device__ __forceinline__ void sh_basis(float x, float y, float z, float* b) {
  b[0] = SH_C0;
  if (NB > 1) { b[1] = -SH_C1 * y; b[2] = SH_C1 * z; b[3] = -SH_C1 * x; }
  if (NB > 4) {
    const float xx = x * x, yy = y * y, zz = z * z, xy = x * y, yz = y * z, xz = x * z;
    b[4] = SH_C2_0 * xy; b[5] = SH_C2_1 * yz; b[6] = SH_C2_2 * (2.f * zz - xx - yy);
    b[7] = SH_C2_3 * xz; b[8] = SH_C2_4 * (xx - yy);
    if (NB > 9) {
      b[9] = SH_C3_0 * y * (3.f * xx - yy); b[10] = SH_C3_1 * xy * z;
      b[11] = SH_C3_2 * y * (4.f * zz - xx - yy); b[12] = SH_C3_3 * z * (2.f * zz - 3.f * xx - 3.f * yy);
      b[13] = SH_C3_4 * x * (4.f * zz - xx - yy); b[14] = SH_C3_5 * z * (xx - yy);
      b[15] = SH_C3_6 * x * (xx - 3.f * yy);
    }
  }
}

template <int NB>
__device__ __forceinline__ float3 sh_eval(const float* sh , float x, float y, float z) {
  float b[NB];
  sh_basis<NB>(x, y, z, b);
  float3 acc = make_float3(0.f, 0.f, 0.f);
#pragma unroll
  for (int k = 0; k < NB; ++k) {
    acc.x += b[k] * sh[3 * k]; acc.y += b[k] * sh[3 * k + 1]; acc.z += b[k] * sh[3 * k + 2];
  }
  return acc;
}

template <bool POSED, int D>
__global__ __launch_bounds__(256) void k_preprocess_fwd(
    int P, int M, const float* __restrict__ means3D, const float* __restrict__ shs, const float* __restrict__ shs_rest,
    const float* __restrict__ colors_precomp, const float* __restrict__ opacities, const float* __restrict__ scales,
    const float* __restrict__ rotations, const float* __restrict__ cov3D_precomp, CamParams cp,
    int32_t* __restrict__ radii, GsRec* __restrict__ recs, float* __restrict__ cov3Ds, uint2* __restrict__ rects,
    uint8_t* __restrict__ clamped, float* __restrict__ depths, uint8_t* __restrict__ visible, GsPosed posed, GsPrologue pro) {
  const int i = blockIdx.x * blockDim.x + threadIdx.x;
  {
    const size_t gid = (size_t)i, stride = (size_t)gridDim.x * blockDim.x;
    if (pro.grad_records) {
      const float4 z = make_float4(0.f, 0.f, 0.f, 0.f);
      for (size_t k = gid; k < pro.n_vec; k += stride) pro.grad_records[k] = z;
    }
    if (pro.tile_counters)
      for (size_t k = gid; k < (size_t)pro.n_counters; k += stride) pro.tile_counters[k] = 0u;
    if (pro.g_poses && gid < (size_t)pro.n_pose) pro.g_poses[gid] = 0.f;
    if (pro.pose_scratch && gid < 32) pro.pose_scratch[gid] = 0.f;
    if (pro.adam_scratch && gid < 8) pro.adam_scratch[gid] = 0.f;
  }
  if (i >= P) return;
  radii[i] = 0;
  if (visible) visible[i] = 0;
  rects[i] = make_uint2(0u, 0u);
  const float* view = cp.view;
  const float* proj = cp.proj;
  PoseMat pm;
  if (POSED) pm = load_pose(posed.pose);
  float3 m = make_float3(means3D[3 * (size_t)i], means3D[3 * (size_t)i + 1], means3D[3 * (size_t)i + 2]);
  if (POSED) m = pose_mean(pm, m.x, m.y, m.z);
  const float3 pv = gs_tp43(view, m);
  if (pv.z <= 0.2f) return;
  const float4 ph = gs_tp44(proj, m);
  const float pw = 1.0f / (ph.w + 0.0000001f);
  const float ndcx = ph.x * pw, ndcy = ph.y * pw;

  float cov[6];
  if (cov3D_precomp) {
#pragma unroll
    for (int k = 0; k < 6; ++k) cov[k] = cov3D_precomp[6 * (size_t)i + k];
  } else {
    float4 q = *reinterpret_cast<const float4*>(rotations + 4 * (size_t)i);
    float sc[3] = {scales[3 * (size_t)i], scales[3 * (size_t)i + 1], scales[3 * (size_t)i + 2]};
    if (POSED) {
      q = pose_rot(pm, q);
#pragma unroll
      for (int k = 0; k < 3; ++k) sc[k] = pose_scale(sc[k]);
    }
    float R[9];
    quat_to_R(q.x, q.y, q.z, q.w, R);
    const float s0 = cp.scale_modifier * sc[0], s1 = cp.scale_modifier * sc[1], s2 = cp.scale_modifier * sc[2];
    float L[9];
#pragma unroll
    for (int r = 0; r < 3; ++r) { L[3 * r] = R[3 * r] * s0; L[3 * r + 1] = R[3 * r + 1] * s1; L[3 * r + 2] = R[3 * r + 2] * s2; }
    cov[0] = L[0] * L[0] + L[1] * L[1] + L[2] * L[2];
    cov[1] = L[0] * L[3] + L[1] * L[4] + L[2] * L[5];
    cov[2] = L[0] * L[6] + L[1] * L[7] + L[2] * L[8];
    cov[3] = L[3] * L[3] + L[4] * L[4] + L[5] * L[5];
    cov[4] = L[3] * L[6] + L[4] * L[7] + L[5] * L[8];
    cov[5] = L[6] * L[6] + L[7] * L[7] + L[8] * L[8];
  }
#pragma unroll
  for (int k = 0; k < 6; ++k) cov3Ds[6 * (size_t)i + k] = cov[k];

  const Ewa e = ewa_setup(pv, view, cp);
  const Cov2D c2 = ewa_cov2d(e, cov);
  const float det = c2.a * c2.c - c2.b * c2.b;
  if (det == 0.0f) return;
  const float det_inv = 1.f / det;
  const float ca = c2.c * det_inv, cb = -c2.b * det_inv, cc = c2.a * det_inv;
  const float mid = 0.5f * (c2.a + c2.c);
  const float sq = sqrtf(fmaxf(0.1f, mid * mid - det));
  const float radius = ceilf(3.f * sqrtf(fmaxf(mid + sq, mid - sq)));
  const float px = ((ndcx + 1.0f) * cp.W - 1.0f) * 0.5f, py = ((ndcy + 1.0f) * cp.H - 1.0f) * 0.5f;
  const int rminx = min(cp.gx, max(0, (int)((px - radius) / GS_TILE)));
  const int rminy = min(cp.gy, max(0, (int)((py - radius) / GS_TILE)));
  const int rmaxx = min(cp.gx, max(0, (int)((px + radius + GS_TILE - 1) / GS_TILE)));
  const int rmaxy = min(cp.gy, max(0, (int)((py + radius + GS_TILE - 1) / GS_TILE)));
  if ((rmaxx - rminx) * (rmaxy - rminy) == 0) return;

  float3 rgb;
  uint8_t clamp_bits = 0;
  if (colors_precomp) {
    rgb = make_float3(colors_precomp[3 * (size_t)i], colors_precomp[3 * (size_t)i + 1], colors_precomp[3 * (size_t)i + 2]);
  } else {
    float dx = m.x - cp.campos[0], dy = m.y - cp.campos[1], dz = m.z - cp.campos[2];
    const float inv = 1.0f / sqrtf(dx * dx + dy * dy + dz * dz);
    dx *= inv; dy *= inv; dz *= inv;
    float3 v;
    constexpr int NBF = (D + 1) * (D + 1);
    if (shs_rest == nullptr) {
      v = sh_eval<NBF>(shs + (size_t)i * M * 3, dx, dy, dz);
    } else {
      float shl[NBF * 3];
      shl[0] = shs[3 * (size_t)i]; shl[1] = shs[3 * (size_t)i + 1]; shl[2] = shs[3 * (size_t)i + 2];
      const float* rest = shs_rest + (size_t)i * (M - 1) * 3;
#pragma unroll
      for (int k = 3; k < NBF * 3; ++k) shl[k] = rest[k - 3];
      v = sh_eval<NBF>(shl, dx, dy, dz);
    }
    v.x += 0.5f; v.y += 0.5f; v.z += 0.5f;
    clamp_bits = (uint8_t)((v.x < 0.f ? 1 : 0) | (v.y < 0.f ? 2 : 0) | (v.z < 0.f ? 4 : 0));
    rgb = make_float3(fmaxf(v.x, 0.f), fmaxf(v.y, 0.f), fmaxf(v.z, 0.f));
  }

  const float opac = POSED ? pose_opacity(opacities[i]) : opacities[i];
  float hx, hy;
  const float tau = __logf(255.0f * opac);
  const float cdet = ca * cc - cb * cb;
  if (!(tau > 0.f)) { hx = hy = -1e30f; }
  else if (!(cdet > 0.f) || ca * cc > 1000.f * cdet) { hx = hy = 1e30f; }
  else {
    const float s = 2.f * tau / cdet;
    hx = sqrtf(s * cc) * 1.01f + 0.5f;
    hy = sqrtf(s * ca) * 1.01f + 0.5f;
  }

  radii[i] = (int)radius;
  if (visible) visible[i] = 1;
  clamped[i] = clamp_bits;
  int bminx = rminx, bminy = rminy, bmaxx = rmaxx, bmaxy = rmaxy;
  if (hx < 1e29f) {
    if (hx < 0.f) { bmaxx = bminx; bmaxy = bminy; }
    else {
      bminx = max(bminx, (int)floorf((px - hx) * (1.0f / GS_TILE)));
      bminy = max(bminy, (int)floorf((py - hy) * (1.0f / GS_TILE)));
      bmaxx = min(bmaxx, (int)floorf((px + hx) * (1.0f / GS_TILE)) + 1);
      bmaxy = min(bmaxy, (int)floorf((py + hy) * (1.0f / GS_TILE)) + 1);
      if (bmaxx <= bminx || bmaxy <= bminy) { bmaxx = bminx; bmaxy = bminy; }
    }
  }
  rects[i] = make_uint2((uint32_t)bminx | ((uint32_t)bminy << 16), (uint32_t)bmaxx | ((uint32_t)bmaxy << 16));
  GsRec rec;
  rec.q0 = make_float4(px, py, hx, hy);
  rec.q1 = make_float4(-0.5f * GS_LOG2E * ca, -0.5f * GS_LOG2E * cc, -GS_LOG2E * cb, opac);
  rec.q2 = make_float4(rgb.x, rgb.y, rgb.z, pv.z);
  recs[i] = rec;
  depths[i] = pv.z;
}

template <int NB>
__device__ __forceinline__ void sh_backward(const float* sh, float* gsh, float x, float y, float z, float3 gr, float* gd) {
  float b[NB];
  sh_basis<NB>(x, y, z, b);
#pragma unroll
  for (int k = 0; k < NB; ++k) { gsh[3 * k] = b[k] * gr.x; gsh[3 * k + 1] = b[k] * gr.y; gsh[3 * k + 2] = b[k] * gr.z; }
  float w[NB];
#pragma unroll
  for (int k = 0; k < NB; ++k) w[k] = sh[3 * k] * gr.x + sh[3 * k + 1] * gr.y + sh[3 * k + 2] * gr.z;
  float gx = 0.f, gy = 0.f, gz = 0.f;
  if (NB > 1) { gy += -SH_C1 * w[1]; gz += SH_C1 * w[2]; gx += -SH_C1 * w[3]; }
  if (NB > 4) {
    const float xx = x * x, yy = y * y, zz = z * z;
    gx += SH_C2_0 * y * w[4]; gy += SH_C2_0 * x * w[4];
    gy += SH_C2_1 * z * w[5]; gz += SH_C2_1 * y * w[5];
    gx += SH_C2_2 * -2.f * x * w[6]; gy += SH_C2_2 * -2.f * y * w[6]; gz += SH_C2_2 * 4.f * z * w[6];
    gx += SH_C2_3 * z * w[7]; gz += SH_C2_3 * x * w[7];
    gx += SH_C2_4 * 2.f * x * w[8]; gy += SH_C2_4 * -2.f * y * w[8];
    if (NB > 9) {
      gx += SH_C3_0 * 6.f * x * y * w[9]; gy += SH_C3_0 * (3.f * xx - 3.f * yy) * w[9];
      gx += SH_C3_1 * y * z * w[10]; gy += SH_C3_1 * x * z * w[10]; gz += SH_C3_1 * x * y * w[10];
      gx += SH_C3_2 * -2.f * x * y * w[11]; gy += SH_C3_2 * (4.f * zz - xx - 3.f * yy) * w[11]; gz += SH_C3_2 * 8.f * y * z * w[11];
      gx += SH_C3_3 * -6.f * x * z * w[12]; gy += SH_C3_3 * -6.f * y * z * w[12]; gz += SH_C3_3 * (6.f * zz - 3.f * xx - 3.f * yy) * w[12];
      gx += SH_C3_4 * (4.f * zz - 3.f * xx - yy) * w[13]; gy += SH_C3_4 * -2.f * x * y * w[13]; gz += SH_C3_4 * 8.f * x * z * w[13];
      gx += SH_C3_5 * 2.f * x * z * w[14]; gy += SH_C3_5 * -2.f * y * z * w[14]; gz += SH_C3_5 * (xx - yy) * w[14];
      gx += SH_C3_6 * (3.f * xx - 3.f * yy) * w[15]; gy += SH_C3_6 * -6.f * x * y * w[15];
    }
  }
  gd[0] = gx; gd[1] = gy; gd[2] = gz;
}

template <bool POSED, int D, bool POSE_ONLY = false>
__global__ __launch_bounds__(256) void k_preprocess_bwd(
    int P, int M, const float* __restrict__ means3D, const float* __restrict__ shs, const float* __restrict__ shs_rest,
    const float* __restrict__ scales, const float* __restrict__ rotations, int use_shs, int use_cov_precomp, CamParams cp, const int32_t* __restrict__ radii,
    const GsRec* __restrict__ recs, const float* __restrict__ cov3Ds, const uint8_t* __restrict__ clamped, const GsGrad* __restrict__ grads,
    float* __restrict__ dL_dmeans3D, float* __restrict__ dL_dmeans2D, float* __restrict__ dL_dshs, float* __restrict__ dL_dshs_rest,
    float* __restrict__ dL_dcolors, float* __restrict__ dL_dopac, float* __restrict__ dL_dscales,
    float* __restrict__ dL_drots, float* __restrict__ dL_dcov3D, float* __restrict__ sh_gate, float* __restrict__ sh_rest_gate,
    GsPosed posed, float* __restrict__ gate, int gi_xyz, int gi_rot, int gi_scaling, int gi_opacity) {
  __shared__ float s_red[POSED ? 4 : 1][16];
  const int i_raw = blockIdx.x * blockDim.x + threadIdx.x;
  if (!POSED && i_raw >= P) return;
  const bool live = i_raw < P;
  const int i = live ? i_raw : 0;
  const bool vis = live && radii[i] > 0;
  PoseMat pm;
  if (POSED) pm = load_pose(posed.pose);
  GsGrad g;
  g.g0 = make_float4(0, 0, 0, 0); g.g1 = g.g0; g.g2 = g.g0;
  if (vis) {
    const GsGrad mo = grads[i];
    const float4 pre = recs[i].q1;
    const float4 con = make_float4(pre.x * (-2.0f / GS_LOG2E), pre.z * (-1.0f / GS_LOG2E), pre.y * (-2.0f / GS_LOG2E), pre.w);
    const float m1 = mo.g0.x, m2 = mo.g0.y, m3 = mo.g0.z, m4 = mo.g0.w, m5 = mo.g1.x, m0 = mo.g1.y;
    g.g0.x = -(con.x * m1 + con.y * m2) * (0.5f * cp.W);
    g.g0.y = -(con.z * m2 + con.y * m1) * (0.5f * cp.H);
    g.g0.z = -0.5f * m3;
    g.g0.w = -m4;
    g.g1.x = -0.5f * m5;
    g.g1.y = con.w != 0.f ? m0 / con.w : 0.f;
    g.g1.z = mo.g1.z; g.g1.w = mo.g1.w; g.g2.x = mo.g2.x;
  }
  float gm[3] = {0.f, 0.f, 0.f};
  float gcov[6] = {0.f, 0.f, 0.f, 0.f, 0.f, 0.f};
  float gs[3] = {0.f, 0.f, 0.f}, gq[4] = {0.f, 0.f, 0.f, 0.f};
  const float3 gcol = make_float3(g.g1.z, g.g1.w, g.g2.x);
  constexpr int nb = (D + 1) * (D + 1);
  const bool split = shs_rest != nullptr;
  float gsh_local[nb * 3];

  if (vis) {
    const float* view = cp.view;
    const float* proj = cp.proj;
    float3 m = make_float3(means3D[3 * (size_t)i], means3D[3 * (size_t)i + 1], means3D[3 * (size_t)i + 2]);
    if (POSED) m = pose_mean(pm, m.x, m.y, m.z);
    float cov[6];
#pragma unroll
    for (int k = 0; k < 6; ++k) cov[k] = cov3Ds[6 * (size_t)i + k];
    {
      const float3 pv = gs_tp43(view, m);
      const Ewa e = ewa_setup(pv, view, cp);
      const Cov2D c2 = ewa_cov2d(e, cov);
      const float a = c2.a, b = c2.b, c = c2.c;
      const float det = a * c - b * b;
      const float Dv = 1.f / (det * det + 0.0000001f);
      const float gA = g.g0.z, gB = g.g0.w, gC = g.g1.x;
      const float ga = Dv * (-c * c * gA + b * c * gB + (det - a * c) * gC);
      const float gc = Dv * ((det - a * c) * gA + a * b * gB - a * a * gC);
      const float gb = Dv * (2.f * b * c * gA - (det + 2.f * b * b) * gB + 2.f * a * b * gC);
      const float* Mx = e.M;
      float GM[6];
#pragma unroll
      for (int k = 0; k < 3; ++k) { GM[k] = ga * Mx[k] + 0.5f * gb * Mx[3 + k]; GM[3 + k] = 0.5f * gb * Mx[k] + gc * Mx[3 + k]; }
      gcov[0] = Mx[0] * GM[0] + Mx[3] * GM[3];
      gcov[1] = 2.f * (Mx[0] * GM[1] + Mx[3] * GM[4]);
      gcov[2] = 2.f * (Mx[0] * GM[2] + Mx[3] * GM[5]);
      gcov[3] = Mx[1] * GM[1] + Mx[4] * GM[4];
      gcov[4] = 2.f * (Mx[1] * GM[2] + Mx[4] * GM[5]);
      gcov[5] = Mx[2] * GM[2] + Mx[5] * GM[5];
      float gM[6];
      gM[0] = 2.f * (GM[0] * cov[0] + GM[1] * cov[1] + GM[2] * cov[2]);
      gM[1] = 2.f * (GM[0] * cov[1] + GM[1] * cov[3] + GM[2] * cov[4]);
      gM[2] = 2.f * (GM[0] * cov[2] + GM[1] * cov[4] + GM[2] * cov[5]);
      gM[3] = 2.f * (GM[3] * cov[0] + GM[4] * cov[1] + GM[5] * cov[2]);
      gM[4] = 2.f * (GM[3] * cov[1] + GM[4] * cov[3] + GM[5] * cov[4]);
      gM[5] = 2.f * (GM[3] * cov[2] + GM[4] * cov[4] + GM[5] * cov[5]);
      const float gJ00 = gM[0] * view[0] + gM[1] * view[4] + gM[2] * view[8];
      const float gJ02 = gM[0] * view[2] + gM[1] * view[6] + gM[2] * view[10];
      const float gJ11 = gM[3] * view[1] + gM[4] * view[5] + gM[5] * view[9];
      const float gJ12 = gM[3] * view[2] + gM[4] * view[6] + gM[5] * view[10];
      const float tz2 = 1.f / (e.tz * e.tz), tz3 = tz2 / e.tz;
      const float gtx = e.xmul * -cp.focal_x * tz2 * gJ02;
      const float gty = e.ymul * -cp.focal_y * tz2 * gJ12;
      const float gtz = -cp.focal_x * tz2 * gJ00 - cp.focal_y * tz2 * gJ11 + 2.f * cp.focal_x * e.tx * tz3 * gJ02 +
                        2.f * cp.focal_y * e.ty * tz3 * gJ12;
      gm[0] = view[0] * gtx + view[1] * gty + view[2] * gtz;
      gm[1] = view[4] * gtx + view[5] * gty + view[6] * gtz;
      gm[2] = view[8] * gtx + view[9] * gty + view[10] * gtz;
    }
    {
      const float4 ph = gs_tp44(proj, m);
      const float mw = 1.0f / (ph.w + 0.0000001f);
      const float mul1 = ph.x * mw * mw, mul2 = ph.y * mw * mw;
      const float g2x = g.g0.x, g2y = g.g0.y;
      gm[0] += (proj[0] * mw - proj[3] * mul1) * g2x + (proj[1] * mw - proj[3] * mul2) * g2y;
      gm[1] += (proj[4] * mw - proj[7] * mul1) * g2x + (proj[5] * mw - proj[7] * mul2) * g2y;
      gm[2] += (proj[8] * mw - proj[11] * mul1) * g2x + (proj[9] * mw - proj[11] * mul2) * g2y;
    }
    if (use_shs) {
      float dx = m.x - cp.campos[0], dy = m.y - cp.campos[1], dz = m.z - cp.campos[2];
      const float inv = 1.0f / sqrtf(dx * dx + dy * dy + dz * dz);
      dx *= inv; dy *= inv; dz *= inv;
      const uint8_t cl = clamped[i];
      const float3 gr = make_float3((cl & 1) ? 0.f : gcol.x, (cl & 2) ? 0.f : gcol.y, (cl & 4) ? 0.f : gcol.z);
      float shl[nb * 3];
      if (split) {
        shl[0] = shs[3 * (size_t)i]; shl[1] = shs[3 * (size_t)i + 1]; shl[2] = shs[3 * (size_t)i + 2];
        const float* rest = shs_rest + (size_t)i * (M - 1) * 3;
#pragma unroll
        for (int k = 3; k < nb * 3; ++k) shl[k] = rest[k - 3];
      } else {
        const float* src = shs + (size_t)i * M * 3;
#pragma unroll
        for (int k = 0; k < nb * 3; ++k) shl[k] = src[k];
      }
      float gd[3];
      sh_backward<nb>(shl, gsh_local, dx, dy, dz, gr, gd);
      const float dot = dx * gd[0] + dy * gd[1] + dz * gd[2];
      gm[0] += (gd[0] - dx * dot) * inv; gm[1] += (gd[1] - dy * dot) * inv; gm[2] += (gd[2] - dz * dot) * inv;
    }
    if (!use_cov_precomp) {
      float4 q = *reinterpret_cast<const float4*>(rotations + 4 * (size_t)i);
      float sc[3] = {scales[3 * (size_t)i], scales[3 * (size_t)i + 1], scales[3 * (size_t)i + 2]};
      if (POSED) {
        q = pose_rot(pm, q);
#pragma unroll
        for (int k = 0; k < 3; ++k) sc[k] = pose_scale(sc[k]);
      }
      float R[9];
      quat_to_R(q.x, q.y, q.z, q.w, R);
      const float mod = cp.scale_modifier;
      const float s[3] = {mod * sc[0], mod * sc[1], mod * sc[2]};
      float L[9];
#pragma unroll
      for (int r = 0; r < 3; ++r) { L[3 * r] = R[3 * r] * s[0]; L[3 * r + 1] = R[3 * r + 1] * s[1]; L[3 * r + 2] = R[3 * r + 2] * s[2]; }
      const float Gs[9] = {gcov[0], 0.5f * gcov[1], 0.5f * gcov[2], 0.5f * gcov[1], gcov[3], 0.5f * gcov[4],
                           0.5f * gcov[2], 0.5f * gcov[4], gcov[5]};
      float gL[9];
#pragma unroll
      for (int r = 0; r < 3; ++r)
#pragma unroll
        for (int k = 0; k < 3; ++k) gL[3 * r + k] = 2.f * (Gs[3 * r] * L[k] + Gs[3 * r + 1] * L[3 + k] + Gs[3 * r + 2] * L[6 + k]);
      float Rp[9];
#pragma unroll
      for (int k = 0; k < 3; ++k) {
        gs[k] = cp.scale_grad_factor * (R[k] * gL[k] + R[3 + k] * gL[3 + k] + R[6 + k] * gL[6 + k]);
#pragma unroll
        for (int r = 0; r < 3; ++r) Rp[3 * r + k] = gL[3 * r + k] * s[k];
      }
      const float r_ = q.x, x = q.y, y = q.z, z = q.w;
      gq[0] = 2.f * (z * (Rp[3] - Rp[1]) + y * (Rp[2] - Rp[6]) + x * (Rp[7] - Rp[5]));
      gq[1] = 2.f * (y * (Rp[1] + Rp[3]) + z * (Rp[2] + Rp[6]) + r_ * (Rp[7] - Rp[5])) - 4.f * x * (Rp[4] + Rp[8]);
      gq[2] = 2.f * (x * (Rp[1] + Rp[3]) + r_ * (Rp[2] - Rp[6]) + z * (Rp[5] + Rp[7])) - 4.f * y * (Rp[0] + Rp[8]);
      gq[3] = 2.f * (r_ * (Rp[3] - Rp[1]) + x * (Rp[2] + Rp[6]) + y * (Rp[5] + Rp[7])) - 4.f * z * (Rp[0] + Rp[4]);
    }
  }

  if (live && !POSE_ONLY) {
    if (!POSED) {
      dL_dmeans3D[3 * (size_t)i] = gm[0]; dL_dmeans3D[3 * (size_t)i + 1] = gm[1]; dL_dmeans3D[3 * (size_t)i + 2] = gm[2];
      dL_dopac[i] = g.g1.y;
      if (dL_dscales) { dL_dscales[3 * (size_t)i] = gs[0]; dL_dscales[3 * (size_t)i + 1] = gs[1]; dL_dscales[3 * (size_t)i + 2] = gs[2]; }
      if (dL_drots) *reinterpret_cast<float4*>(dL_drots + 4 * (size_t)i) = make_float4(gq[0], gq[1], gq[2], gq[3]);
    }
    dL_dmeans2D[3 * (size_t)i] = g.g0.x; dL_dmeans2D[3 * (size_t)i + 1] = g.g0.y; dL_dmeans2D[3 * (size_t)i + 2] = 0.f;
    if (dL_dcolors) { dL_dcolors[3 * (size_t)i] = gcol.x; dL_dcolors[3 * (size_t)i + 1] = gcol.y; dL_dcolors[3 * (size_t)i + 2] = gcol.z; }
    if (dL_dshs) {
      const bool have = vis && use_shs;
      bool nz_dc = false, nz_rest = false;
      if (!split) {
        float* gdst = dL_dshs + (size_t)i * M * 3;
#pragma unroll
        for (int k = 0; k < nb * 3; ++k) { const float v = have ? gsh_local[k] : 0.f; gdst[k] = v; nz_dc = nz_dc || v != 0.f; }
        for (int k = nb * 3; k < M * 3; ++k) gdst[k] = 0.f;
      } else {
        float* gdc = dL_dshs + 3 * (size_t)i;
#pragma unroll
        for (int c = 0; c < 3; ++c) { const float v = have ? gsh_local[c] : 0.f; gdc[c] = v; nz_dc = nz_dc || v != 0.f; }
        if (dL_dshs_rest) {
          float* grest = dL_dshs_rest + (size_t)i * (M - 1) * 3;
#pragma unroll
          for (int k = 3; k < nb * 3; ++k) { const float v = have ? gsh_local[k] : 0.f; grest[k - 3] = v; nz_rest = nz_rest || v != 0.f; }
          for (int k = nb * 3; k < M * 3; ++k) grest[k - 3] = 0.f;
        }
      }
      if (sh_gate && nz_dc) *sh_gate = 1.0f;
      if (sh_rest_gate && nz_rest) *sh_rest_gate = 1.0f;
    }
    if (dL_dcov3D) {
      const bool on = vis && use_cov_precomp;
#pragma unroll
      for (int k = 0; k < 6; ++k) dL_dcov3D[6 * (size_t)i + k] = on ? gcov[k] : 0.f;
    }
  }
  if (POSED) {
    float a[16];
#pragma unroll
    for (int k = 0; k < 16; ++k) a[k] = 0.f;
    bool nz_xyz = false, nz_rot = false, nz_sc = false, nz_op = false;
    if (live) {
      float act[3];
#pragma unroll
      for (int k = 0; k < 3; ++k) act[k] = pose_scale(scales[3 * (size_t)i + k]);
      const float o = vis ? recs[i].q1.w : 0.5f;
      const PoseGradOut r = pose_backward_one(pm, means3D[3 * (size_t)i], means3D[3 * (size_t)i + 1], means3D[3 * (size_t)i + 2],
                                              *reinterpret_cast<const float4*>(rotations + 4 * (size_t)i), act, o, gm[0], gm[1], gm[2],
                                              make_float4(gq[0], gq[1], gq[2], gq[3]), gs, g.g1.y, a);
      if (!POSE_ONLY) {
#pragma unroll
        for (int k = 0; k < 3; ++k) {
          dL_dmeans3D[3 * (size_t)i + k] = r.d_xyz[k];
          dL_dscales[3 * (size_t)i + k] = r.d_scaling[k];
          nz_xyz = nz_xyz || r.d_xyz[k] != 0.f;
          nz_sc = nz_sc || r.d_scaling[k] != 0.f;
        }
        *reinterpret_cast<float4*>(dL_drots + 4 * (size_t)i) = r.d_rot;
        nz_rot = nz_rot || r.d_rot.x != 0.f || r.d_rot.y != 0.f || r.d_rot.z != 0.f || r.d_rot.w != 0.f;
        dL_dopac[i] = r.d_opacity_logit;
        nz_op = nz_op || r.d_opacity_logit != 0.f;
      }
    }
    pose_accumulate(a, posed.acc, posed.partial, s_red);
    if (!POSE_ONLY && gate) {
      if (gi_xyz >= 0 && nz_xyz) gate[gi_xyz] = 1.0f;
      if (gi_rot >= 0 && nz_rot) gate[gi_rot] = 1.0f;
      if (gi_scaling >= 0 && nz_sc) gate[gi_scaling] = 1.0f;
      if (gi_opacity >= 0 && nz_op) gate[gi_opacity] = 1.0f;
    }
  }
}

__global__ __launch_bounds__(256) void k_mark_visible(int P, const float* __restrict__ means3D, const float* __restrict__ view,
                                                      uint8_t* __restrict__ present) {
  const int i = blockIdx.x * blockDim.x + threadIdx.x;
  if (i >= P) return;
  const float3 m = make_float3(means3D[3 * (size_t)i], means3D[3 * (size_t)i + 1], means3D[3 * (size_t)i + 2]);
  present[i] = gs_tp43(view, m).z > 0.2f ? 1 : 0;
}

}

int gs_launch_preprocess_fwd(hipStream_t stream, int P, int D, int M, const float* means3D, const float* shs, const float* shs_rest,
                             const float* colors_precomp, const float* opacities, const float* scales,
                             const float* rotations, const float* cov3D_precomp, const CamParams& cp, int32_t* radii,
                             GsRec* recs, float* cov3Ds, uint2* rects, uint8_t* clamped, float* depths, uint8_t* visible,
                             const GsPosed& posed_args, const GsPrologue& pro) {
  if (P <= 0) return 0;
  const bool posed = posed_args.pose != nullptr;
  const GsPosed pa = posed ? posed_args : GsPosed();
#define GS_FWD(POSED, DEG)                                                                                                              \
  hipLaunchKernelGGL((k_preprocess_fwd<POSED, DEG>), dim3((P + 255) / 256), dim3(256), 0, stream, P, M, means3D, shs, shs_rest,         \
                     colors_precomp, opacities, scales, rotations, cov3D_precomp, cp, radii, recs, cov3Ds, rects, clamped, depths, visible, pa, pro)
  const int deg = shs ? D : 0;
  if (posed) { if (deg == 0) GS_FWD(true, 0); else if (deg == 1) GS_FWD(true, 1); else if (deg == 2) GS_FWD(true, 2); else GS_FWD(true, 3); }
  else { if (deg == 0) GS_FWD(false, 0); else if (deg == 1) GS_FWD(false, 1); else if (deg == 2) GS_FWD(false, 2); else GS_FWD(false, 3); }
#undef GS_FWD
  return 0;
}

int gs_launch_preprocess_bwd(hipStream_t stream, int P, int D, int M, const float* means3D, const float* shs, const float* shs_rest,
                             const float* scales, const float* rotations, int use_shs, int use_cov_precomp,
                             const CamParams& cp, const int32_t* radii, const GsRec* recs, const float* cov3Ds, const uint8_t* clamped,
                             const GsGrad* grads, float* dL_dmeans3D, float* dL_dmeans2D, float* dL_dshs, float* dL_dshs_rest,
                             float* dL_dcolors, float* dL_dopac, float* dL_dscales, float* dL_drots, float* dL_dcov3D,
                             const GsPosed& posed_args, float* gate_flags, bool pose_only) {
  if (P <= 0) return 0;
  const bool posed = posed_args.pose != nullptr;
  const GsPosed pa = posed ? posed_args : GsPosed();
  float* sh_gate = gate_flags ? gate_flags + GS_GATE_SH : nullptr;
  float* sh_rest_gate = gate_flags ? gate_flags + GS_GATE_SH_REST : nullptr;
  float* gate = posed ? gate_flags : nullptr;
  const bool gi_on = posed && gate_flags;
  const int gi[4] = {gi_on ? GS_GATE_XYZ : -1, gi_on ? GS_GATE_ROT : -1, gi_on ? GS_GATE_SCALING : -1, gi_on ? GS_GATE_OPACITY : -1};
#define GS_BWD(POSED, DEG, ...)                                                                                                         \
  hipLaunchKernelGGL((k_preprocess_bwd<POSED, DEG, ##__VA_ARGS__>), dim3((P + 255) / 256), dim3(256), 0, stream, P, M, means3D, shs, shs_rest, scales, \
                     rotations, use_shs, use_cov_precomp, cp, radii, recs, cov3Ds, clamped, grads, dL_dmeans3D, dL_dmeans2D, dL_dshs,  \
                     dL_dshs_rest, dL_dcolors, dL_dopac, dL_dscales, dL_drots, dL_dcov3D, sh_gate, sh_rest_gate, pa, gate, gi[0],     \
                     gi[1], gi[2], gi[3])
  const int deg = use_shs ? D : 0;
  if (posed && pose_only) {
    if (deg == 0) GS_BWD(true, 0, true); else if (deg == 1) GS_BWD(true, 1, true); else if (deg == 2) GS_BWD(true, 2, true); else GS_BWD(true, 3, true);
  } else if (posed) { if (deg == 0) GS_BWD(true, 0); else if (deg == 1) GS_BWD(true, 1); else if (deg == 2) GS_BWD(true, 2); else GS_BWD(true, 3); }
  else { if (deg == 0) GS_BWD(false, 0); else if (deg == 1) GS_BWD(false, 1); else if (deg == 2) GS_BWD(false, 2); else GS_BWD(false, 3); }
#undef GS_BWD
  return 0;
}

int gs_launch_mark_visible(hipStream_t stream, int P, const float* means3D, const float* view, uint8_t* present) {
  if (P <= 0) return 0;
  hipLaunchKernelGGL(k_mark_visible, dim3((P + 255) / 256), dim3(256), 0, stream, P, means3D, view, present);
  return 0;
}
```

### instantsplat_amd/csrc/tracker.hip

```cpp
#include <stdlib.h>
#include <string.h>
#include <math.h>
#include "pose_math.h"

namespace {

constexpr int L1_PER_THREAD = 4;
constexpr int L1_BLOCK = 256 * L1_PER_THREAD;

int l1_nblocks(int W, int H) { return (int)((3LL * W * H + L1_BLOCK - 1) / L1_BLOCK); }

struct Tracker : GsFrozenScene {
  char* grad_scratch;
  float *dL_dimg, *loss_partial, *pose_partial;
  bool consts_ready;
  GsKnobs knobs;
};

size_t carve(Tracker& t, void* workspace) {
  GsCarver c{(char*)workspace};
  t.GsFrozenScene::carve(c, t.knobs, true);
  t.grad_scratch = c.take<char>(gs_grad_scratch_bytes(t.P, t.knobs.det));
  t.dL_dimg = c.take<float>(3 * (size_t)t.W * t.H);
  t.loss_partial = c.take<float>(2 * (size_t)l1_nblocks(t.W, t.H));
  t.pose_partial = c.take<float>(16 * (((size_t)t.P + 255) / 256));
  return c.off;
}

__global__ __launch_bounds__(256) void k_masked_l1(int n, const float* __restrict__ img, const float* __restrict__ gt,
                                                   float* __restrict__ dL_dimg, float* __restrict__ partial) {
  __shared__ float s_red[4][2];
  float a = 0.f, b = 0.f;
  const int base = blockIdx.x * L1_BLOCK + threadIdx.x;
#pragma unroll
  for (int j = 0; j < L1_PER_THREAD; ++j) {
    const int idx = base + j * 256;
    if (idx < n) {
      const float r = img[idx], d = r - gt[idx];
      const float m = r > 0.f ? 1.f : 0.f;
      const float sg = d > 0.f ? 1.f : (d < 0.f ? -1.f : d * 0.f);
      dL_dimg[idx] = sg * m;
      a += fabsf(d) * m;
      b += m;
    }
  }
  a = gs_wave_sum_row3(a); b = gs_wave_sum_row3(b);
  const int wave = threadIdx.x >> 6;
  if ((threadIdx.x & 63) == 63) { s_red[wave][0] = a; s_red[wave][1] = b; }
  __syncthreads();
  if (threadIdx.x == 0) {
    partial[2 * blockIdx.x] = (s_red[0][0] + s_red[1][0]) + (s_red[2][0] + s_red[3][0]);
    partial[2 * blockIdx.x + 1] = (s_red[0][1] + s_red[1][1]) + (s_red[2][1] + s_red[3][1]);
  }
}

constexpr float ADAM_WD = (float)1e-4;
constexpr float ADAM_LERP_W = (float)(1.0 - 0.9);
constexpr float ADAM_BETA2 = (float)0.999;
constexpr float ADAM_ONE_MINUS_BETA2 = (float)(1.0 - 0.999);
constexpr float ADAM_EPS = (float)1e-8;

__device__ __forceinline__ float tracker_adam(float p, float d, float& m, float& v, float step_size, float bc2_sqrt) {
#ifdef __clang__
#pragma clang fp contract(off)
#endif
  const float gr = fmaf(ADAM_WD, p, d);
  m = fmaf(ADAM_LERP_W, gr - m, m);
  const float gg = gr * gr;
  v = fmaf(ADAM_ONE_MINUS_BETA2, gg, v * ADAM_BETA2);
  const float denom = sqrtf(v) / bc2_sqrt + ADAM_EPS;
  const float q = m / denom;
  return fmaf(step_size, q, p);
}

__global__ __launch_bounds__(1024) void k_tracker_finish(const float* __restrict__ partial, int nrows, const float* __restrict__ loss_partial,
                                                         int loss_nblocks, const uint32_t* __restrict__ count, const uint32_t* __restrict__ qmax,
                                                         int nq, unsigned long long capacity,
                                                         const float4* __restrict__ sched, int iter, float* __restrict__ state,
                                                         float* __restrict__ pose_trace, float* __restrict__ loss_trace,
                                                         float* __restrict__ grad_trace) {
  __shared__ float s_sum[16][17];
  __shared__ float s_tot[16];
  __shared__ double s_la[16], s_lb[16];
  __shared__ uint32_t s_blended;
  const int k = threadIdx.x & 15, g = threadIdx.x >> 4;
  if (threadIdx.x == 0) s_blended = 0u;
  float v0 = 0.f, v1 = 0.f, v2 = 0.f, v3 = 0.f;
  {
    int r = g;
    for (; r + 192 < nrows; r += 256) {
      v0 += partial[(size_t)r * 16 + k]; v1 += partial[(size_t)(r + 64) * 16 + k];
      v2 += partial[(size_t)(r + 128) * 16 + k]; v3 += partial[(size_t)(r + 192) * 16 + k];
    }
    for (; r < nrows; r += 64) v0 += partial[(size_t)r * 16 + k];
  }
  {
    double a = 0.0, b = 0.0;
    for (int i = threadIdx.x; i < loss_nblocks; i += 1024) { a += (double)loss_partial[2 * i]; b += (double)loss_partial[2 * i + 1]; }
    a = gs_wave_sum_row3_f64(a); b = gs_wave_sum_row3_f64(b);
    if ((threadIdx.x & 63) == 63) { s_la[threadIdx.x >> 6] = a; s_lb[threadIdx.x >> 6] = b; }
  }
  const float wsum = gs_sum_rows((v0 + v1) + (v2 + v3));
  if ((threadIdx.x & 63) < 16) s_sum[threadIdx.x >> 6][k] = wsum;
  __syncthreads();
  bool masked_out = true;
  for (int w = 0; w < 16; ++w) masked_out = masked_out && s_lb[w] == 0.0;
  if (masked_out && *count > 0u) {
    uint32_t any = 0u;
    for (int i = threadIdx.x; i < nq; i += 1024) any |= qmax[i];
    if (any) s_blended = 1u;
  }
  if (threadIdx.x < 16) {
    float t = 0.f;
#pragma unroll
    for (int q = 0; q < 16; ++q) t += s_sum[q][threadIdx.x];
    s_tot[threadIdx.x] = t;
  }
  __syncthreads();
  if (threadIdx.x != 0) return;
  double la = 0.0, lb = 0.0;
  for (int w = 0; w < 16; ++w) { la += s_la[w]; lb += s_lb[w]; }
  float total[16];
#pragma unroll
  for (int c = 0; c < 16; ++c) total[c] = s_tot[c];
  float* pose = state + MI355GS_TRACKER_POSE;
  float d[7];
  pose_grad_from_sums(load_pose(pose), total, d);
  const uint32_t cnt = *count;
  const float loss = (float)(la / lb);
  const float inv = lb > 0.0 ? 1.0f / (float)lb : (s_blended ? __int_as_float(0x7fc00000) : 0.0f);
#pragma unroll
  for (int c = 0; c < 7; ++c) d[c] = lb > 0.0 ? d[c] * inv : inv;
  if (pose_trace)
    for (int c = 0; c < 7; ++c) pose_trace[7 * (size_t)iter + c] = pose[c];
  if (loss_trace) loss_trace[iter] = loss;
  if (grad_trace)
    for (int c = 0; c < 7; ++c) grad_trace[7 * (size_t)iter + c] = d[c];
  uint32_t* flag = reinterpret_cast<uint32_t*>(state + MI355GS_TRACKER_FLAG);
  uint32_t* seen = reinterpret_cast<uint32_t*>(state + MI355GS_TRACKER_COUNT);
  if (cnt > *seen) *seen = cnt;
  if ((unsigned long long)cnt > capacity) *flag = 1u;
  if (*flag) return;
  if (iter == 0) state[MI355GS_TRACKER_INITIAL] = loss;
  const float4 s = sched[iter];
  float* m = state + MI355GS_TRACKER_EXP_AVG;
  float* v = state + MI355GS_TRACKER_EXP_AVG_SQ;
#pragma unroll
  for (int c = 0; c < 7; ++c) {
    float mc = m[c], vc = v[c];
    pose[c] = tracker_adam(pose[c], d[c], mc, vc, c < 4 ? s.y : s.x, s.z);
    m[c] = mc; v[c] = vc;
  }
  if (loss < state[MI355GS_TRACKER_BEST]) {
    state[MI355GS_TRACKER_BEST] = loss;
    for (int c = 0; c < 7; ++c) state[MI355GS_TRACKER_CAND + c] = pose[c];
  }
}

int ensure_consts(Tracker* t, hipStream_t stream) {
  if (t->consts_ready) return MI355GS_OK;
  const int rc = gs_write_view_consts(stream, t->consts, "tracker_consts");
  t->consts_ready = rc == MI355GS_OK;
  return rc;
}

}

extern "C" {

size_t mi355gs_tracker_workspace_bytes(int P, int W, int H, int64_t capacity) {
  if (P <= 0 || W <= 0 || H <= 0 || capacity <= 0) return 0;
  Tracker t;
  memset(&t, 0, sizeof(t));
  t.P = P; t.W = W; t.H = H; t.capacity = capacity; t.knobs = gs_knobs();
  return carve(t, nullptr);
}

void* mi355gs_tracker_create(int P, int M, int W, int H, int64_t capacity, const float* xyz, const float* f_dc, const float* f_rest,
                             const float* opacity, const float* scaling, const float* rotation, void* workspace) {
  Tracker* t = (Tracker*)calloc(1, sizeof(Tracker));
  if (!t) return nullptr;
  if (!t->init(P, M, W, H, capacity, xyz, f_dc, f_rest, opacity, scaling, rotation, workspace)) { free(t); return nullptr; }
  t->knobs = gs_knobs();
  carve(*t, workspace);
  return t;
}

void mi355gs_tracker_destroy(void* handle) { free(handle); }

int mi355gs_tracker_count(void* handle, void* stream_, int sh_degree, const float* projmatrix, float tanfovx, float tanfovy,
                          const float* pose, int32_t* count_out) {
  GS_RANGE();
  Tracker* t = (Tracker*)handle;
  hipStream_t stream = (hipStream_t)stream_;
  if (!t || !t->degree_ok(sh_degree) || !projmatrix || !pose || !count_out) return MI355GS_EINVAL;
  int rc;
  if ((rc = ensure_consts(t, stream))) return rc;
  GsFrameCtx cx;
  cx.posed.pose = pose;
  return gs_frame_project(stream, t->scene(sh_degree), t->view(projmatrix, tanfovx, tanfovy), t->bufs(t->knobs, nullptr), cx, count_out,
                          nullptr, 0);
}

int mi355gs_tracker_run(void* handle, void* stream_, int sh_degree, const float* gt_image, const float* projmatrix, float tanfovx,
                        float tanfovy, const float* bg, const float* sched, int num_iter, int first_iter, int n_iters, float* state,
                        float* pose_trace, float* loss_trace, float* grad_trace) {
  GS_RANGE();
  Tracker* t = (Tracker*)handle;
  hipStream_t stream = (hipStream_t)stream_;
  const int debug = 0;
  if (!t || !t->degree_ok(sh_degree) || !gt_image || !projmatrix || !bg || !sched || !state) return MI355GS_EINVAL;
  if (num_iter <= 0 || first_iter < 0 || n_iters < 0 || first_iter > num_iter || n_iters > num_iter - first_iter) return MI355GS_EINVAL;
  if (n_iters == 0) return MI355GS_OK;
  int rc;
  if ((rc = ensure_consts(t, stream))) return rc;
  const int P = t->P, W = t->W, H = t->H;
  const TilesLayout tl(W, H);
  const int n_pix = 3 * W * H, l1_blocks = l1_nblocks(W, H), rows = (P + 255) / 256;
  const GsScene scene = t->scene(sh_degree);
  const GsView view = t->view(projmatrix, tanfovx, tanfovy);
  const GsFrameBufs bufs = t->bufs(t->knobs, t->grad_scratch);
  GsPrologue pro;
  pro.grad_records = (float4*)t->grad_scratch; pro.n_vec = (size_t)P * 3;
  pro.tile_counters = (uint32_t*)(t->tiles + tl.count); pro.n_counters = (int)((tl.start - tl.count) / 4);
  GsFrameCtx cx;
  cx.prologue = &pro;
  cx.posed.pose = state + MI355GS_TRACKER_POSE;
  cx.posed.acc = t->pose_partial;
  cx.posed.partial = t->pose_partial;
  cx.pose_only = true;
  for (int it = first_iter; it < first_iter + n_iters; ++it) {
    if ((rc = gs_frame_project(stream, scene, view, bufs, cx, t->num_rendered, nullptr, 0))) return rc;
    if ((rc = gs_frame_render(stream, P, view, bufs, bg, t->image, true, 0))) return rc;
    GS_KRANGE("masked_l1");
    hipLaunchKernelGGL(k_masked_l1, dim3(l1_blocks), dim3(256), 0, stream, n_pix, t->image, gt_image, t->dL_dimg, t->loss_partial);
    GS_CHECK_LAUNCH("masked_l1");
    if ((rc = gs_frame_backward(stream, scene, view, bufs, cx, bg, t->image, t->dL_dimg, GsGradOut(), false, 0))) return rc;
    GS_KRANGE("tracker_finish");
    hipLaunchKernelGGL(k_tracker_finish, dim3(1), dim3(1024), 0, stream, (const float*)t->pose_partial, rows,
                       (const float*)t->loss_partial, l1_blocks, t->count(), (const uint32_t*)(t->tiles + tl.qmax), 4 * tl.T,
                       (unsigned long long)t->capacity, (const float4*)sched, it, state,
                       pose_trace, loss_trace, grad_trace);
    GS_CHECK_LAUNCH("tracker_finish");
  }
  return MI355GS_OK;
}

}
```

### instantsplat_amd/csrc/trainer.hip

```cpp
#include <stdlib.h>
#include <string.h>
#include "common.h"

int gs_loss_fused(hipStream_t, int, int, int, const float*, const float*, float, float*, void*);
int gs_loss_fused_nblocks(int, int, int);
int gs_launch_pose_finish_partials(hipStream_t, const float*, const float*, int, float*, float*, const float*, int, double, float, float*, int,
                                   int);

namespace {

struct Trainer {
  int P, W, H, V;
  int64_t capacity;
  float *xyz, *f_dc, *f_rest, *opacity, *scaling, *rotation, *poses;
  float* m[7];
  float* v[7];
  const float* pplr;
  char *geom, *tiles, *binning, *grad_scratch, *ssim_scratch;
  float *image, *dL_dimg;
  int32_t* radii;
  float *g_means2D, *g_colors;
  float *g_xyz, *g_rot, *g_scaling, *g_opacity, *g_fdc, *g_frest, *g_poses;
  float *pose_scratch, *pose_partial, *adam_scratch, *consts;
  uint32_t* adam_live;
  uint32_t adam_seq;
  bool consts_ready;
  GsKnobs knobs;
};

size_t carve(Trainer& t, void* workspace) {
  GsCarver c{(char*)workspace};
  const size_t P = (size_t)(t.P > 0 ? t.P : 1), npix = (size_t)t.W * t.H;
  t.geom = c.take<char>(GeomLayout(t.P).total);
  t.tiles = c.take<char>(TilesLayout(t.W, t.H).total);
  t.binning = c.take<char>(gs_binning_bytes(t.capacity, t.W, t.H, t.knobs, true));
  t.grad_scratch = c.take<char>(gs_grad_scratch_bytes(t.P, t.knobs.det));
  t.ssim_scratch = c.take<char>(mi355gs_ssim_scratch_bytes(1, 3, t.H, t.W));
  t.image = c.take<float>(3 * npix); t.dL_dimg = c.take<float>(3 * npix);
  t.radii = c.take<int32_t>(P);
  t.g_means2D = c.take<float>(3 * P); t.g_colors = c.take<float>(3 * P);
  t.g_xyz = c.take<float>(3 * P); t.g_rot = c.take<float>(4 * P); t.g_scaling = c.take<float>(3 * P); t.g_opacity = c.take<float>(P);
  t.g_fdc = c.take<float>(3 * P); t.g_frest = c.take<float>(45 * P); t.g_poses = c.take<float>(7 * (size_t)t.V);
  t.pose_scratch = c.take<float>(32); t.pose_partial = c.take<float>(16 * ((P + 255) / 256)); t.adam_scratch = c.take<float>(8); t.consts = c.take<float>(32);
  t.adam_live = c.take<uint32_t>(16);
  return c.off;
}

int trainer_adam(Trainer* t, hipStream_t stream, const float* lr, const int32_t* step, float beta1, float beta2, float eps,
                 bool commit_gate) {
  const int P = t->P;
  const int64_t numel[7] = {3LL * P, 3LL * P, 45LL * P, (int64_t)P, 3LL * P, 4LL * P, 7LL * t->V};
  const int32_t row[7] = {3, 1, 1, 1, 1, 1, 1};
  float* params[7] = {t->xyz, t->f_dc, t->f_rest, t->opacity, t->scaling, t->rotation, t->poses};
  const float* grads[7] = {t->g_xyz, t->g_fdc, t->g_frest, t->g_opacity, t->g_scaling, t->g_rot, t->g_poses};
  const float* pplr[7] = {t->pplr, nullptr, nullptr, nullptr, nullptr, nullptr, nullptr};
  if (++t->adam_seq == 0u) t->adam_seq = 1u;
  GsAdamFused fused = {t->adam_live, t->adam_seq, nullptr, 0, nullptr};
  if (commit_gate) {
    fused.commit_count = gs_frame_count(t->tiles, t->W, t->H);
    fused.commit_capacity = (unsigned long long)t->capacity;
    fused.commit_poison = t->adam_live + 15;
  }
  return gs_adam_multi(stream, 7, numel, row, params, grads, t->m, t->v, pplr, lr, beta1, beta2, eps, step, t->adam_scratch, nullptr, nullptr,
                       nullptr, 0u, &fused);
}

GsScene posed_scene(int P, int D, const float* xyz, const float* f_dc, const float* f_rest, const float* opacity_logit,
                    const float* log_scales, float scale_modifier, const float* rotation) {
  return {P, D, D == 0 ? 1 : 16, xyz, f_dc, D == 0 ? nullptr : f_rest, nullptr, opacity_logit, log_scales, rotation, nullptr, scale_modifier};
}

}

extern "C" {

int mi355gs_posed_forward_preprocess(void* stream, int P, int D, int W, int H, const float* xyz, const float* f_dc,
                                     const float* f_rest, const float* opacity_logit, const float* log_scales, float scale_modifier,
                                     const float* rotation, const float* pose, const float* view_identity, const float* projmatrix,
                                     const float* origin, float tanfovx, float tanfovy, int32_t* radii, void* geom, void* tiles,
                                     int32_t* num_rendered, uint8_t* visible, void* grad_scratch, int debug) {
  GS_RANGE();
  if (!pose || D < 0 || D > 3 || (D > 0 && !f_rest)) return MI355GS_EINVAL;
  GsFrameCtx cx;
  cx.posed.pose = pose;
  return gs_frame_project((hipStream_t)stream, posed_scene(P, D, xyz, f_dc, f_rest, opacity_logit, log_scales, scale_modifier, rotation),
                          {W, H, view_identity, projmatrix, origin, tanfovx, tanfovy}, {geom, tiles, nullptr, 0, radii, grad_scratch, gs_knobs()},
                          cx, num_rendered, visible, debug);
}

int mi355gs_posed_backward(void* stream_, int P, int D, int W, int H, const float* bg, const float* xyz, const float* f_dc,
                           const float* f_rest, const float* opacity_logit, const float* log_scales, float scale_modifier,
                           const float* rotation, const float* pose, const float* view_identity, const float* projmatrix,
                           const float* origin, float tanfovx, float tanfovy, const void* geom, void* tiles, const void* binning,
                           int64_t capacity, const int32_t* radii, const float* out_color, const float* dL_dpix,
                           void* grad_scratch, float* pose_scratch, float* d_xyz, float* d_means2D, float* d_f_dc, float* d_f_rest,
                           float* d_opacity_logit, float* d_log_scales, float* d_rotation, float* d_pose, int pose_rows, int pose_row,
                           int grad_scratch_is_clear, int debug) {
  GS_RANGE();
  hipStream_t stream = (hipStream_t)stream_;
  if (!pose || !pose_scratch || !d_pose || D < 0 || D > 3 || (D > 0 && (!f_rest || !d_f_rest))) return MI355GS_EINVAL;
  if (pose_rows < 0 || (pose_rows > 0 && (pose_row < 0 || pose_row >= pose_rows))) return MI355GS_EINVAL;
  if (P <= 0)
    return hipMemsetAsync(d_pose, 0, (size_t)(pose_rows > 0 ? pose_rows : 1) * 7 * sizeof(float), stream) == hipSuccess ? MI355GS_OK : MI355GS_ELAUNCH;
  const int rows = (P + 255) / 256;
  float* gate = (float*)((char*)grad_scratch + gs_grad_gate_offset(P));
  GsFrameCtx cx;
  cx.posed.pose = pose;
  cx.posed.acc = pose_scratch + (size_t)16 * rows;
  cx.posed.partial = pose_scratch;
  cx.gate = gate; cx.gate_tail = true;
  const GsGradOut o = {d_xyz, d_means2D, d_f_dc, D == 0 ? nullptr : d_f_rest, nullptr, d_opacity_logit, d_log_scales, d_rotation, nullptr};
  const int rc = gs_frame_backward(stream, posed_scene(P, D, xyz, f_dc, f_rest, opacity_logit, log_scales, scale_modifier, rotation),
                                   {W, H, view_identity, projmatrix, origin, tanfovx, tanfovy},
                                   {const_cast<void*>(geom), tiles, const_cast<void*>(binning), capacity, const_cast<int32_t*>(radii), grad_scratch, gs_knobs()},
                                   cx, bg, out_color, dL_dpix, o, grad_scratch_is_clear != 0, debug);
  if (rc) return rc;
  GS_KRANGE("pose_finish");
  gs_launch_pose_finish_partials(stream, pose, pose_scratch, rows, d_pose, gate + GS_GATE_POSE, nullptr, 0, 0.0, 0.f, nullptr, pose_rows, pose_row);
  GS_CHECK_LAUNCH("pose_finish");
  return MI355GS_OK;
}

size_t mi355gs_trainer_workspace_bytes(int P, int W, int H, int V, int64_t capacity) {
  if (P < 0 || W <= 0 || H <= 0 || V <= 0 || capacity < 0) return 0;
  Trainer t;
  memset(&t, 0, sizeof(t));
  t.P = P; t.W = W; t.H = H; t.V = V; t.capacity = capacity; t.knobs = gs_knobs();
  return carve(t, nullptr);
}

void* mi355gs_trainer_create(int P, int W, int H, int V, int64_t capacity, float* xyz, float* f_dc, float* f_rest, float* opacity,
                             float* scaling, float* rotation, float* poses, float* const* exp_avg, float* const* exp_avg_sq,
                             const float* per_point_lr, void* workspace) {
  if (P <= 0 || W <= 0 || H <= 0 || V <= 0 || capacity <= 0 || !workspace || !exp_avg || !exp_avg_sq) return nullptr;
  if (!xyz || !f_dc || !f_rest || !opacity || !scaling || !rotation || !poses) return nullptr;
  Trainer* t = (Trainer*)calloc(1, sizeof(Trainer));
  if (!t) return nullptr;
  t->P = P; t->W = W; t->H = H; t->V = V; t->capacity = capacity;
  t->xyz = xyz; t->f_dc = f_dc; t->f_rest = f_rest; t->opacity = opacity; t->scaling = scaling; t->rotation = rotation; t->poses = poses;
  for (int k = 0; k < 7; ++k) {
    if (!exp_avg[k] || !exp_avg_sq[k]) { free(t); return nullptr; }
    t->m[k] = exp_avg[k]; t->v[k] = exp_avg_sq[k];
  }
  t->pplr = per_point_lr;
  t->knobs = gs_knobs();
  carve(*t, workspace);
  t->consts_ready = false;
  return t;
}

void mi355gs_trainer_destroy(void* handle) { free(handle); }

const float* mi355gs_trainer_grad(void* handle, int k) {
  Trainer* t = (Trainer*)handle;
  if (!t || k < 0 || k > 6) return nullptr;
  const float* g[7] = {t->g_xyz, t->g_fdc, t->g_frest, t->g_opacity, t->g_scaling, t->g_rot, t->g_poses};
  return g[k];
}

int mi355gs_trainer_step(void* handle, void* stream_, int view, int sh_degree, const float* gt_image, const float* projmatrix,
                         float tanfovx, float tanfovy, const float* bg, const float* lr, const int32_t* step, float beta1, float beta2, float eps,
                         float lambda_dssim, int do_optimizer_step, float* loss_out, int32_t* num_rendered_out) {
  GS_RANGE();
  Trainer* t = (Trainer*)handle;
  hipStream_t stream = (hipStream_t)stream_;
  const int debug = 0;
  if (!t || view < 0 || view >= t->V || sh_degree < 0 || sh_degree > 3 || !gt_image || !projmatrix || !bg || !lr || !step || !loss_out || !num_rendered_out)
    return MI355GS_EINVAL;
  const int P = t->P, W = t->W, H = t->H;
  if (!t->consts_ready) {
    if (int rc = gs_write_view_consts(stream, t->consts, "trainer_consts")) return rc;
    if (hipMemsetAsync(t->g_frest, 0, (size_t)P * 45 * sizeof(float), stream) != hipSuccess) return MI355GS_ELAUNCH;
    if (hipMemsetAsync(t->adam_live, 0, 16 * sizeof(uint32_t), stream) != hipSuccess) return MI355GS_ELAUNCH;
    t->consts_ready = true;
  }
  GsPrologue pro;
  {
    const TilesLayout tl(W, H);
    pro.grad_records = (float4*)t->grad_scratch; pro.n_vec = (size_t)P * 3;
    pro.tile_counters = (uint32_t*)(t->tiles + tl.count); pro.n_counters = (int)((tl.start - tl.count) / 4);
    pro.g_poses = t->g_poses; pro.n_pose = 7 * t->V; pro.pose_scratch = t->pose_scratch; pro.adam_scratch = t->adam_scratch;
  }
  const float* pose = t->poses + 7 * (size_t)view;
  GsFrameCtx cx;
  cx.prologue = &pro;
  cx.posed.pose = pose; cx.posed.acc = t->pose_scratch; cx.posed.partial = t->pose_partial;
  cx.gate = t->adam_scratch;
  const int D = sh_degree;
  const GsScene scene = posed_scene(P, D, t->xyz, t->f_dc, t->f_rest, t->opacity, t->scaling, 1.0f, t->rotation);
  const GsView vw = {W, H, t->consts, projmatrix, t->consts + 16, tanfovx, tanfovy};
  const GsFrameBufs bufs = {t->geom, t->tiles, t->binning, t->capacity, t->radii, t->grad_scratch, t->knobs};
  int rc;
  if ((rc = gs_frame_project(stream, scene, vw, bufs, cx, num_rendered_out, nullptr, 0))) return rc;
  if ((rc = gs_frame_render(stream, P, vw, bufs, bg, t->image, true, 0))) return rc;
  if ((rc = gs_loss_fused(stream, 3, H, W, t->image, gt_image, lambda_dssim, t->dL_dimg, t->ssim_scratch))) return rc;
  const GsGradOut o = {t->g_xyz, t->g_means2D, t->g_fdc, D == 0 ? nullptr : t->g_frest, t->g_colors, t->g_opacity, t->g_scaling, t->g_rot, nullptr};
  if ((rc = gs_frame_backward(stream, scene, vw, bufs, cx, bg, t->image, t->dL_dimg, o, false, 0))) return rc;
  GS_KRANGE("pose_finish");
  gs_launch_pose_finish_partials(stream, pose, t->pose_partial, (P + 255) / 256, t->g_poses + 7 * (size_t)view, t->adam_scratch + GS_GATE_POSE,
                                 (const float*)t->ssim_scratch, gs_loss_fused_nblocks(3, H, W), 1.0 / (3.0 * H * W), lambda_dssim, loss_out, 0, 0);
  GS_CHECK_LAUNCH("pose_finish");
  if (do_optimizer_step) return trainer_adam(t, stream, lr, step, beta1, beta2, eps, true);
  return MI355GS_OK;
}

int mi355gs_trainer_optimizer_step(void* handle, void* stream_, const float* lr, const int32_t* step, float beta1, float beta2,
                                   float eps, int commit_gate) {
  GS_RANGE();
  Trainer* t = (Trainer*)handle;
  if (!t || !lr || !step || !t->consts_ready) return MI355GS_EINVAL;
  return trainer_adam(t, (hipStream_t)stream_, lr, step, beta1, beta2, eps, commit_gate != 0);
}

}
```

Measured before the change: 3539.

## Fuse per-tile Gaussian counting into projection kernel and split binning into scatter and sort

The per-tile instance histogram that a separate count_tiles kernel used to compute is now built inside the preprocess/projection kernel using LDS bins, one Gaussian per thread. The scan kernel clears the tile counts after reading them, so the per-frame prologue no longer has to zero them, and the counts stay clean across iterations. The old binning kernel is split into a scatter kernel and a per-tile sort kernel. This saves a launch and a reread of the rects, but adds LDS pressure and extra syncs to the projection kernel, which may lower its occupancy.

```diff
diff --git a/instantsplat_amd/csrc/api.hip b/instantsplat_amd/csrc/api.hip
--- a/instantsplat_amd/csrc/api.hip
+++ b/instantsplat_amd/csrc/api.hip
@@ -5,15 +5,17 @@
 
 int gs_launch_preprocess_fwd(hipStream_t, int, int, int, const float*, const float*, const float*, const float*, const float*, const float*,
                              const float*, const float*, const CamParams&, int32_t*, GsRec*, float*, uint2*, uint8_t*, float*, uint8_t*,
-                             const GsPosed&, const GsPrologue&);
-int gs_launch_count_tiles(hipStream_t, int, int, int, const uint2*, uint32_t*, uint32_t*, uint32_t*);
+                             const GsPosed&, const GsPrologue&, const GsTileCount&);
+bool gs_bin_counts_in_projection(int);
+int gs_launch_count_tiles_direct(hipStream_t, int, int, const uint2*, uint32_t*);
 int gs_launch_preprocess_bwd(hipStream_t, int, int, int, const float*, const float*, const float*, const float*, const float*, int, int,
                              const CamParams&, const int32_t*, const GsRec*, const float*, const uint8_t*, const GsGrad*, float*, float*,
                              float*, float*, float*, float*, float*, float*, float*, const GsPosed&, float*, bool);
 int gs_launch_mark_visible(hipStream_t, int, const float*, const float*, uint8_t*);
-int gs_launch_scan_tiles(hipStream_t, int, const uint32_t*, uint32_t*, int32_t*, uint32_t*, uint32_t*, uint32_t*, uint32_t*, int);
-int gs_launch_binning(hipStream_t, int, int, int, const float*, const uint2*, const uint32_t*, uint32_t*, uint64_t*, uint32_t*, uint32_t,
-                      const uint32_t*, const uint32_t*, const uint32_t*);
+int gs_launch_scan_tiles(hipStream_t, int, uint32_t*, uint32_t*, int32_t*, uint32_t*, uint32_t*, uint32_t*, uint32_t*, int, bool);
+int gs_launch_scatter(hipStream_t, int, int, int, const float*, const uint2*, const uint32_t*, uint32_t*, uint64_t*, uint32_t, const uint32_t*,
+                      const uint32_t*);
+int gs_launch_sort_tiles(hipStream_t, int, int, const uint32_t*, uint64_t*, uint32_t*, uint32_t, const uint32_t*);
 int gs_launch_composite_fwd(hipStream_t, int, int, int, int, uint32_t, const uint32_t*, const uint32_t*, const GsRec*, const float*,
                             float*, float*, uint32_t*, const uint32_t*, const uint32_t*, const uint32_t*, uint4*, float4*, uint32_t,
                             const uint32_t*, unsigned long long*, uint32_t, uint32_t*, unsigned long long*, bool);
@@ -112,6 +114,12 @@
   else if (i < 19) consts[i] = 0.f;
 }
 }
+namespace {
+__global__ __launch_bounds__(256) void k_clear_words(uint32_t* words, int n) {
+  const int i = blockIdx.x * 256 + threadIdx.x;
+  if (i < n) words[i] = 0u;
+}
+}
 int gs_write_view_consts(hipStream_t stream, float* consts, const char* name) {
   const int debug = 0;
   GS_KRANGE(name);
@@ -136,11 +144,16 @@
   const TilesLayout tl(W, H);
   char* g = (char*)fb.geom;
   char* t = (char*)fb.tiles;
+  if (!cx.counters_clean && P > 0) {
+    GS_KRANGE("clear_tile_counts");
+    hipLaunchKernelGGL(k_clear_words, dim3((tl.T + 255) / 256), dim3(256), 0, stream, (uint32_t*)(t + tl.count), tl.T);
+    GS_CHECK_LAUNCH("clear_tile_counts");
+  }
   GsPrologue pro;
   if (cx.prologue) {
     pro = *cx.prologue;
   } else {
-    pro.tile_counters = (uint32_t*)(t + tl.count); pro.n_counters = (int)((tl.start - tl.count) / 4);
+    pro.tile_counters = (uint32_t*)(t + tl.cursor); pro.n_counters = (int)((tl.start - tl.cursor) / 4);
     if (fb.grad_scratch) { pro.grad_records = (float4*)fb.grad_scratch; pro.n_vec = gs_grad_gate_offset(P) / 16 + 2; }
     if (P <= 0) {
       if (hipMemsetAsync(t + tl.count, 0, tl.start - tl.count, stream) != hipSuccess) return MI355GS_ELAUNCH;
@@ -148,19 +161,26 @@
     }
   }
   const CamParams cp = make_cam(vw.view, vw.proj, vw.campos, vw.tanfovx, vw.tanfovy, sc.scale_modifier, W, H);
+  const bool in_projection = gs_bin_counts_in_projection(tl.T);
+  GsTileCount tc;
+  if (in_projection) {
+    tc.tile_count = (uint32_t*)(t + tl.count); tc.entries = (uint32_t*)(g + gl.bin_entries); tc.entry_n = (uint32_t*)(g + gl.bin_n);
+    tc.T = tl.T;
+  }
   GS_KRANGE("preprocess_fwd");
   gs_launch_preprocess_fwd(stream, P, D, M, sc.means3D, sc.shs, sc.shs_rest, sc.colors_precomp, sc.opacities, sc.scales, sc.rotations,
                            sc.cov3D_precomp, cp, fb.radii, (GsRec*)(g + gl.rec), (float*)(g + gl.cov3D), (uint2*)(g + gl.rect),
-                           (uint8_t*)(g + gl.clamped), (float*)(g + gl.depth), visible, cx.posed, pro);
+                           (uint8_t*)(g + gl.clamped), (float*)(g + gl.depth), visible, cx.posed, pro, tc);
   GS_CHECK_LAUNCH("preprocess_fwd");
-  GS_KRANGE("count_tiles");
-  gs_launch_count_tiles(stream, P, tl.T, tl.gx, (const uint2*)(g + gl.rect), (uint32_t*)(t + tl.count), (uint32_t*)(g + gl.bin_entries),
-                        (uint32_t*)(g + gl.bin_n));
-  GS_CHECK_LAUNCH("count_tiles");
+  if (!in_projection) {
+    GS_KRANGE("count_tiles");
+    gs_launch_count_tiles_direct(stream, P, tl.gx, (const uint2*)(g + gl.rect), (uint32_t*)(t + tl.count));
+    GS_CHECK_LAUNCH("count_tiles");
+  }
   GS_KRANGE("scan_tiles");
-  gs_launch_scan_tiles(stream, tl.T, (const uint32_t*)(t + tl.count), (uint32_t*)(t + tl.start), num_rendered,
+  gs_launch_scan_tiles(stream, tl.T, (uint32_t*)(t + tl.count), (uint32_t*)(t + tl.start), num_rendered,
                        (uint32_t*)(t + tl.order), (uint32_t*)(t + tl.meta), (uint32_t*)(t + tl.seg_first), (uint32_t*)(t + tl.part_first),
-                       fb.knobs.min_units);
+                       fb.knobs.min_units, true);
   GS_CHECK_LAUNCH("scan_tiles");
   return MI355GS_OK;
 }
@@ -178,12 +198,15 @@
   const char* g = (const char*)fb.geom;
   char* t = (char*)fb.tiles;
   char* b = (char*)fb.binning;
-  GS_KRANGE("binning");
-  gs_launch_binning(stream, P, tl.T, tl.gx, (const float*)(g + gl.depth), (const uint2*)(g + gl.rect),
-                    (const uint32_t*)(t + tl.start), (uint32_t*)(t + tl.cursor), (uint64_t*)(b + bl.keys),
-                    (uint32_t*)(b + bl.list), cap, (const uint32_t*)(t + tl.order), (const uint32_t*)(g + gl.bin_entries),
+  GS_KRANGE("scatter_tiles");
+  gs_launch_scatter(stream, P, tl.T, tl.gx, (const float*)(g + gl.depth), (const uint2*)(g + gl.rect), (const uint32_t*)(t + tl.start),
+                    (uint32_t*)(t + tl.cursor), (uint64_t*)(b + bl.keys), cap, (const uint32_t*)(g + gl.bin_entries),
                     (const uint32_t*)(g + gl.bin_n));
-  GS_CHECK_LAUNCH("binning");
+  GS_CHECK_LAUNCH("scatter_tiles");
+  GS_KRANGE("sort_tiles");
+  gs_launch_sort_tiles(stream, P, tl.T, (const uint32_t*)(t + tl.start), (uint64_t*)(b + bl.keys), (uint32_t*)(b + bl.list), cap,
+                       (const uint32_t*)(t + tl.order));
+  GS_CHECK_LAUNCH("sort_tiles");
   {
     ProfScope prof(train ? 0 : 2, stream);
     GS_KRANGE("composite_fwd");
diff --git a/instantsplat_amd/csrc/bin_walk.h b/instantsplat_amd/csrc/bin_walk.h
--- /dev/null
+++ b/instantsplat_amd/csrc/bin_walk.h
@@ -0,0 +1,87 @@
+#pragma once
+#include "common.h"
+
+static_assert(GS_BIN_GROUP == 256, "one Gaussian per thread of a 256-thread workgroup");
+
+__device__ __forceinline__ bool gs_unpack_rect(uint2 r, int& x0, int& y0, int& x1, int& y1) {
+  x0 = r.x & 0xffff; y0 = r.x >> 16; x1 = r.y & 0xffff; y1 = r.y >> 16;
+  return x1 > x0 && y1 > y0;
+}
+
+constexpr int GS_BIN_WIDE = 8;
+
+template <class F>
+__device__ __forceinline__ void gs_for_each_instance(int i, uint2 own, uint32_t* s_wide, uint2* s_wide_rect, uint32_t* s_nwide, F&& f) {
+  const int tid = threadIdx.x;
+  {
+    int x0, y0, x1, y1;
+    if (gs_unpack_rect(own, x0, y0, x1, y1)) {
+      if ((x1 - x0) * (y1 - y0) > GS_BIN_WIDE) {
+        const uint32_t slot = atomicAdd(s_nwide, 1u);
+        s_wide[slot] = (uint32_t)i; s_wide_rect[slot] = own;
+      } else {
+        for (int y = y0; y < y1; ++y)
+          for (int x = x0; x < x1; ++x) f(i, true, x, y);
+      }
+    }
+  }
+  __syncthreads();
+  const int nwide = (int)*s_nwide;
+  for (int q = tid >> 4; q < nwide; q += 16) {
+    const int iq = (int)s_wide[q];
+    int x0, y0, x1, y1;
+    gs_unpack_rect(s_wide_rect[q], x0, y0, x1, y1);
+    const int w = x1 - x0, n = w * (y1 - y0);
+    const int dq = 16 / w, dr = 16 - dq * w;
+    int j = tid & 15, row = j / w, col = j - row * w;
+    for (; j < n; j += 16) {
+      f(iq, false, x0 + col, y0 + row);
+      col += dr; row += dq;
+      if (col >= w) { col -= w; row += 1; }
+    }
+  }
+}
+
+__device__ __forceinline__ void gs_group_histogram(int T, int gx, int i, uint2 own, uint32_t* s_bins, uint32_t* s_wide,
+                                                   uint2* s_wide_rect, uint32_t* s_nwide) {
+  for (int t = threadIdx.x; t < T; t += GS_BIN_GROUP) s_bins[t] = 0;
+  if (threadIdx.x == 0) *s_nwide = 0;
+  __syncthreads();
+  gs_for_each_instance(i, own, s_wide, s_wide_rect, s_nwide, [&](int, bool, int x, int y) { atomicAdd(&s_bins[y * gx + x], 1u); });
+  __syncthreads();
+}
+
+__device__ __forceinline__ void gs_count_group(const GsTileCount& tc, int P, int gx, int i, uint2 own, uint32_t* s_bins) {
+  __shared__ uint32_t s_wide[GS_BIN_GROUP];
+  __shared__ uint2 s_wide_rect[GS_BIN_GROUP];
+  __shared__ uint32_t s_nwide;
+  __shared__ uint32_t s_wave_nz[GS_BIN_GROUP / GS_WAVE];
+  const int tid = threadIdx.x, T = tc.T;
+  gs_group_histogram(T, gx, i, own, s_bins, s_wide, s_wide_rect, &s_nwide);
+  unsigned long long mask = 0ull;
+  {
+    int k = 0;
+    for (int t = tid; t < T; t += GS_BIN_GROUP, ++k) {
+      const uint32_t c = s_bins[t];
+      if (c) { atomicAdd(&tc.tile_count[t], c); mask |= 1ull << k; }
+    }
+  }
+  const uint32_t nz = (uint32_t)__popcll(mask);
+  const uint32_t incl = gs_wave_scan_incl_u32(nz);
+  if ((tid & 63) == 63) s_wave_nz[tid >> 6] = incl;
+  __syncthreads();
+  uint32_t off = incl - nz, total = 0;
+#pragma unroll
+  for (int w = 0; w < GS_BIN_GROUP / GS_WAVE; ++w) {
+    if (w < (tid >> 6)) off += s_wave_nz[w];
+    total += s_wave_nz[w];
+  }
+  if (tid == 0) tc.entry_n[gs_bin_n_index((int)blockIdx.x, P)] = total <= (uint32_t)GS_BIN_GROUP_ENTRIES ? total : 0xffffffffu;
+  if (total > (uint32_t)GS_BIN_GROUP_ENTRIES) return;
+  uint32_t* mine = tc.entries + (size_t)blockIdx.x * GS_BIN_GROUP_ENTRIES + off;
+  while (mask) {
+    const int t = tid + GS_BIN_GROUP * (__ffsll((long long)mask) - 1);
+    mask &= mask - 1ull;
+    *mine++ = (uint32_t)t | (s_bins[t] << 16);
+  }
+}
diff --git a/instantsplat_amd/csrc/binning.hip b/instantsplat_amd/csrc/binning.hip
--- a/instantsplat_amd/csrc/binning.hip
+++ b/instantsplat_amd/csrc/binning.hip
@@ -1,4 +1,4 @@
-#include "common.h"
+#include "bin_walk.h"
 
 namespace {
 
@@ -17,10 +17,10 @@
 constexpr int SCAN_PER_MAX = (int)(SCAN_STAGE_MAX_BYTES / (SCAN_THREADS * 4));
 
 template <bool STAGED>
-__global__ __launch_bounds__(SCAN_THREADS) void k_scan_tiles(int T, const uint32_t* count, uint32_t* start, int32_t* num_rendered,
+__global__ __launch_bounds__(SCAN_THREADS) void k_scan_tiles(int T, uint32_t* count, uint32_t* start, int32_t* num_rendered,
                                                                uint32_t* __restrict__ order, uint32_t* __restrict__ meta,
                                                                uint32_t* __restrict__ seg_first, uint32_t* __restrict__ part_first,
-                                                               uint32_t min_units) {
+                                                               uint32_t min_units, bool clear) {
   __shared__ uint32_t wave_tot[SCAN_THREADS / GS_WAVE];
   HIP_DYNAMIC_SHARED(uint32_t, s_stage)
   const int tid = threadIdx.x, lane = tid & 63, wave = tid >> 6;
@@ -30,6 +30,8 @@
   uint32_t own[STAGED ? SCAN_PER_MAX : 1];
   if constexpr (STAGED) {
     for (int e = tid; e < T; e += SCAN_THREADS) s_stage[e] = count[e];
+    if (clear)
+      for (int e = tid; e < T; e += SCAN_THREADS) count[e] = 0u;
     __syncthreads();
 #pragma unroll
     for (int k = 0; k < SCAN_PER_MAX; ++k) own[k] = lo + k < hi ? s_stage[lo + k] : 0u;
@@ -141,6 +143,10 @@
     start[T] = total;
     *num_rendered = (int32_t)total;
   }
+  if constexpr (!STAGED) {
+    if (clear)
+      for (int i = lo; i < hi; ++i) count[i] = 0u;
+  }
   SCAN_STAMP(8);
 }
 
@@ -192,166 +198,67 @@
   }
 }
 
-constexpr int BIN_CHUNK = GS_BIN_CHUNK;
-static_assert(BIN_CHUNK == 512, "two Gaussians per thread (own_depth selection in k_scatter_lds)");
 constexpr int BIN_MAX_LDS_TILES = 16384;
-static_assert(BIN_MAX_LDS_TILES <= 64 * 256, "k_count_tiles_lds keeps one bit per bin of a thread in a 64-bit mask");
-
-__device__ __forceinline__ bool unpack_rect(uint2 r, int& x0, int& y0, int& x1, int& y1) {
-  x0 = r.x & 0xffff; y0 = r.x >> 16; x1 = r.y & 0xffff; y1 = r.y >> 16;
-  return x1 > x0 && y1 > y0;
-}
-
+static_assert(BIN_MAX_LDS_TILES <= 64 * GS_BIN_GROUP, "gs_count_group keeps one bit per bin of a thread in a 64-bit mask");
+static_assert(BIN_MAX_LDS_TILES <= 0x10000, "a packed entry holds the tile in 16 bits");
 constexpr int BIN_WIDE = 8;
-
-constexpr int BIN_PER_THREAD = BIN_CHUNK / 256;
-
-template <class F>
-__device__ __forceinline__ void for_each_instance(int lo, int hi, const uint2 (&own)[BIN_PER_THREAD], const uint2* __restrict__ rects,
-                                                  uint32_t* s_wide, uint2* s_wide_rect, uint32_t* s_nwide, F&& f) {
-  const int tid = threadIdx.x;
-#pragma unroll
-  for (int j = 0; j < BIN_PER_THREAD; ++j) {
-    const int i = lo + tid + 256 * j;
-    int x0, y0, x1, y1;
-    if (i >= hi || !unpack_rect(own[j], x0, y0, x1, y1)) continue;
-    if ((x1 - x0) * (y1 - y0) > BIN_WIDE) {
-      const uint32_t slot = atomicAdd(s_nwide, 1u);
-      s_wide[slot] = (uint32_t)i; s_wide_rect[slot] = own[j];
-      continue;
-    }
-    for (int y = y0; y < y1; ++y)
-      for (int x = x0; x < x1; ++x) f(i, j, x, y);
-  }
-  __syncthreads();
-  const int nwide = (int)*s_nwide;
-  for (int q = tid >> 4; q < nwide; q += 16) {
-    const int i = (int)s_wide[q];
-    int x0, y0, x1, y1;
-    unpack_rect(s_wide_rect[q], x0, y0, x1, y1);
-    const int w = x1 - x0, n = w * (y1 - y0);
-    const int dq = 16 / w, dr = 16 - dq * w;
-    int j = tid & 15, row = j / w, col = j - row * w;
-    for (; j < n; j += 16) {
-      f(i, -1, x0 + col, y0 + row);
-      col += dr; row += dq;
-      if (col >= w) { col -= w; row += 1; }
-    }
-  }
-}
-
-__global__ __launch_bounds__(256) void k_count_tiles_lds(int P, int T, int gx, const uint2* __restrict__ rects,
-                                                          uint32_t* __restrict__ tile_count, uint32_t* __restrict__ entries,
-                                                          uint32_t* __restrict__ entry_n) {
+static_assert(BIN_WIDE == GS_BIN_WIDE, "one threshold for the count in the projection and the scatter here");
+
+__global__ __launch_bounds__(GS_BIN_GROUP) void k_scatter_lds(int P, int T, int gx, const float* __restrict__ depths,
+                                                               const uint2* __restrict__ rects, const uint32_t* __restrict__ start,
+                                                               uint32_t* __restrict__ cursor, uint64_t* __restrict__ keys, uint32_t capacity,
+                                                               const uint32_t* __restrict__ entries, const uint32_t* __restrict__ entry_n) {
   HIP_DYNAMIC_SHARED(uint32_t, s_bins)
-  __shared__ uint32_t s_wide[BIN_CHUNK];
-  __shared__ uint2 s_wide_rect[BIN_CHUNK];
-  __shared__ uint32_t s_nwide;
-  __shared__ uint32_t s_wave_nz[4];
-  const int tid = threadIdx.x;
-  const int lo = blockIdx.x * BIN_CHUNK, hi = min(P, lo + BIN_CHUNK);
-  uint2 own[BIN_PER_THREAD];
-#pragma unroll
-  for (int j = 0; j < BIN_PER_THREAD; ++j) own[j] = rects[min(lo + tid + 256 * j, P - 1)];
-  for (int t = tid; t < T; t += 256) s_bins[t] = 0;
-  if (tid == 0) s_nwide = 0;
-  __syncthreads();
-  for_each_instance(lo, hi, own, rects, s_wide, s_wide_rect, &s_nwide, [&](int, int, int x, int y) { atomicAdd(&s_bins[y * gx + x], 1u); });
-  __syncthreads();
-  unsigned long long mask = 0ull;
-  {
-    int k = 0;
-    for (int t = tid; t < T; t += 256, ++k) {
-      const uint32_t c = s_bins[t];
-      if (c) { atomicAdd(&tile_count[t], c); mask |= 1ull << k; }
-    }
-  }
-  const uint32_t nz = (uint32_t)__popcll(mask);
-  const uint32_t incl = gs_wave_scan_incl_u32(nz);
-  if ((tid & 63) == 63) s_wave_nz[tid >> 6] = incl;
-  __syncthreads();
-  uint32_t off = incl - nz, total = 0;
-#pragma unroll
-  for (int w = 0; w < 4; ++w) {
-    if (w < (tid >> 6)) off += s_wave_nz[w];
-    total += s_wave_nz[w];
-  }
-  if (tid == 0) entry_n[blockIdx.x] = total <= (uint32_t)GS_BIN_ENTRIES ? total : 0xffffffffu;
-  if (total > (uint32_t)GS_BIN_ENTRIES) return;
-  uint32_t* mine = entries + (size_t)blockIdx.x * GS_BIN_ENTRIES + off;
-  while (mask) {
-    const int t = tid + 256 * (__ffsll((long long)mask) - 1);
-    mask &= mask - 1ull;
-    *mine++ = (uint32_t)t | (s_bins[t] << 16);
-  }
-}
-
-__global__ __launch_bounds__(256) void k_scatter_lds(int P, int T, int gx, const float* __restrict__ depths,
-                                                      const uint2* __restrict__ rects, const uint32_t* __restrict__ start,
-                                                      uint32_t* __restrict__ cursor, uint64_t* __restrict__ keys, uint32_t capacity,
-                                                      const uint32_t* __restrict__ entries, const uint32_t* __restrict__ entry_n) {
-  HIP_DYNAMIC_SHARED(uint32_t, s_bins)
-  __shared__ uint32_t s_wide[BIN_CHUNK];
-  __shared__ uint2 s_wide_rect[BIN_CHUNK];
+  __shared__ uint32_t s_wide[GS_BIN_GROUP];
+  __shared__ uint2 s_wide_rect[GS_BIN_GROUP];
   __shared__ uint32_t s_nwide;
   const int tid = threadIdx.x;
-  const int lo = blockIdx.x * BIN_CHUNK, hi = min(P, lo + BIN_CHUNK);
-  uint2 own[BIN_PER_THREAD];
-  uint32_t own_depth[BIN_PER_THREAD];
-#pragma unroll
-  for (int j = 0; j < BIN_PER_THREAD; ++j) {
-    const int ic = min(lo + tid + 256 * j, P - 1);
-    own[j] = rects[ic];
-    own_depth[j] = __float_as_uint(depths[ic]);
-  }
-  const uint32_t n_entries = entry_n[blockIdx.x];
+  const int i = blockIdx.x * GS_BIN_GROUP + tid;
+  const uint2 own = i < P ? rects[i] : make_uint2(0u, 0u);
+  const uint32_t own_depth = __float_as_uint(depths[min(i, P - 1)]);
+  const uint32_t n_entries = entry_n[gs_bin_n_index((int)blockIdx.x, P)];
   if (n_entries != 0xffffffffu) {
-    const uint32_t* mine = entries + (size_t)blockIdx.x * GS_BIN_ENTRIES;
-    for (uint32_t e0 = 0; e0 < n_entries; e0 += 1024) {
-      uint32_t en[4], r[4], st[4];
+    const uint32_t* mine = entries + (size_t)blockIdx.x * GS_BIN_GROUP_ENTRIES;
+    static_assert(GS_BIN_GROUP_ENTRIES <= 2 * GS_BIN_GROUP, "two entries per thread cover the list");
+    uint32_t en[2], r[2], st[2];
+#pragma unroll
+    for (int j = 0; j < 2; ++j) {
+      const uint32_t e = tid + GS_BIN_GROUP * j;
+      en[j] = e < n_entries ? mine[e] : 0u;
+    }
+#pragma unroll
+    for (int j = 0; j < 2; ++j) {
+      r[j] = 0u; st[j] = 0u;
+      if (en[j]) { r[j] = atomicAdd(&cursor[en[j] & 0xffffu], en[j] >> 16); st[j] = start[en[j] & 0xffffu]; }
+    }
+#pragma unroll
+    for (int j = 0; j < 2; ++j)
+      if (en[j]) s_bins[en[j] & 0xffffu] = st[j] + r[j];
+  } else {
+    gs_group_histogram(T, gx, i, own, s_bins, s_wide, s_wide_rect, &s_nwide);
+    for (int t0 = 0; t0 < T; t0 += 4 * GS_BIN_GROUP) {
+      uint32_t c[4], r[4], st[4];
 #pragma unroll
       for (int j = 0; j < 4; ++j) {
-        const uint32_t e = e0 + tid + 256 * j;
-        en[j] = e < n_entries ? mine[e] : 0u;
-      }
-#pragma unroll
-      for (int j = 0; j < 4; ++j) {
-        r[j] = 0u; st[j] = 0u;
-        if (en[j]) { r[j] = atomicAdd(&cursor[en[j] & 0xffffu], en[j] >> 16); st[j] = start[en[j] & 0xffffu]; }
-      }
-#pragma unroll
-      for (int j = 0; j < 4; ++j)
-        if (en[j]) s_bins[en[j] & 0xffffu] = st[j] + r[j];
-    }
-  } else {
-    for (int t = tid; t < T; t += 256) s_bins[t] = 0;
-    if (tid == 0) s_nwide = 0;
-    __syncthreads();
-    for_each_instance(lo, hi, own, rects, s_wide, s_wide_rect, &s_nwide, [&](int, int, int x, int y) { atomicAdd(&s_bins[y * gx + x], 1u); });
-    __syncthreads();
-    for (int t0 = 0; t0 < T; t0 += 1024) {
-      uint32_t c[4], r[4], st[4];
-#pragma unroll
-      for (int j = 0; j < 4; ++j) {
-        const int t = t0 + tid + 256 * j;
+        const int t = t0 + tid + GS_BIN_GROUP * j;
         c[j] = t < T ? s_bins[t] : 0u;
       }
 #pragma unroll
       for (int j = 0; j < 4; ++j) {
-        const int t = t0 + tid + 256 * j;
+        const int t = t0 + tid + GS_BIN_GROUP * j;
         r[j] = 0u; st[j] = 0u;
         if (c[j]) { r[j] = atomicAdd(&cursor[t], c[j]); st[j] = start[t]; }
       }
 #pragma unroll
       for (int j = 0; j < 4; ++j)
-        if (c[j]) s_bins[t0 + tid + 256 * j] = st[j] + r[j];
+        if (c[j]) s_bins[t0 + tid + GS_BIN_GROUP * j] = st[j] + r[j];
     }
   }
   if (tid == 0) s_nwide = 0;
   __syncthreads();
-  for_each_instance(lo, hi, own, rects, s_wide, s_wide_rect, &s_nwide, [&](int i, int j, int x, int y) {
-    const uint32_t depth = j == 0 ? own_depth[0] : (j == 1 ? own_depth[BIN_PER_THREAD - 1] : __float_as_uint(depths[i]));
-    const uint64_t key = ((uint64_t)depth << 32) | (uint32_t)i;
+  gs_for_each_instance(i, own, s_wide, s_wide_rect, &s_nwide, [&](int g, bool mine, int x, int y) {
+    const uint32_t depth = mine ? own_depth : __float_as_uint(depths[g]);
+    const uint64_t key = ((uint64_t)depth << 32) | (uint32_t)g;
     const uint32_t pos = atomicAdd(&s_bins[y * gx + x], 1u);
     if (pos < capacity) keys[pos] = key;
   });
@@ -362,7 +269,7 @@
   const int i = blockIdx.x * blockDim.x + threadIdx.x;
   if (i >= P) return;
   int x0, y0, x1, y1;
-  if (!unpack_rect(rects[i], x0, y0, x1, y1)) return;
+  if (!gs_unpack_rect(rects[i], x0, y0, x1, y1)) return;
   for (int y = y0; y < y1; ++y)
     for (int x = x0; x < x1; ++x) atomicAdd(&tile_count[y * gx + x], 1u);
 }
@@ -373,7 +280,7 @@
   const int i = blockIdx.x * blockDim.x + threadIdx.x;
   if (i >= P) return;
   int x0, y0, x1, y1;
-  if (!unpack_rect(rects[i], x0, y0, x1, y1)) return;
+  if (!gs_unpack_rect(rects[i], x0, y0, x1, y1)) return;
   const uint64_t key = ((uint64_t)__float_as_uint(depths[i]) << 32) | (uint32_t)i;
   for (int y = y0; y < y1; ++y)
     for (int x = x0; x < x1; ++x) {
@@ -633,15 +540,15 @@
 }
 int gs_min_units() { return g_min_units; }
 
-int gs_launch_scan_tiles(hipStream_t stream, int T, const uint32_t* count, uint32_t* start, int32_t* num_rendered, uint32_t* order,
-                         uint32_t* meta, uint32_t* seg_first, uint32_t* part_first, int min_units) {
+int gs_launch_scan_tiles(hipStream_t stream, int T, uint32_t* count, uint32_t* start, int32_t* num_rendered, uint32_t* order,
+                         uint32_t* meta, uint32_t* seg_first, uint32_t* part_first, int min_units, bool clear) {
   const size_t stage_bytes = (size_t)((T + SCAN_THREADS - 1) / SCAN_THREADS) * SCAN_THREADS * 4;
   if (T > SCAN_THREADS && stage_bytes <= SCAN_STAGE_MAX_BYTES)
     hipLaunchKernelGGL(k_scan_tiles<true>, dim3(1), dim3(SCAN_THREADS), stage_bytes, stream, T, count, start, num_rendered, order, meta,
-                       seg_first, part_first, (uint32_t)min_units);
+                       seg_first, part_first, (uint32_t)min_units, clear);
   else
     hipLaunchKernelGGL(k_scan_tiles<false>, dim3(1), dim3(SCAN_THREADS), 0, stream, T, count, start, num_rendered, order, meta, seg_first,
-                       part_first, (uint32_t)min_units);
+                       part_first, (uint32_t)min_units, clear);
   return 0;
 }
 
@@ -649,8 +556,8 @@
 static int scan_large(hipStream_t stream, int n, const uint32_t* in, uint32_t* out, uint32_t* block_sums, int32_t* total) {
   const int nb = (n + SCAN_CHUNK - 1) / SCAN_CHUNK;
   hipLaunchKernelGGL(k_scan_block_sums<RECT>, dim3(nb), dim3(256), 0, stream, n, in, block_sums);
-  hipLaunchKernelGGL(k_scan_tiles<false>, dim3(1), dim3(SCAN_THREADS), 0, stream, nb, (const uint32_t*)block_sums, block_sums, total,
-                     (uint32_t*)nullptr, (uint32_t*)nullptr, (uint32_t*)nullptr, (uint32_t*)nullptr, 0u);
+  hipLaunchKernelGGL(k_scan_tiles<false>, dim3(1), dim3(SCAN_THREADS), 0, stream, nb, block_sums, block_sums, total,
+                     (uint32_t*)nullptr, (uint32_t*)nullptr, (uint32_t*)nullptr, (uint32_t*)nullptr, 0u, false);
   hipLaunchKernelGGL(k_scan_apply<RECT>, dim3(nb), dim3(256), 0, stream, n, in, (const uint32_t*)block_sums, out);
   return 0;
 }
@@ -661,31 +568,27 @@
   return scan_large<true>(stream, P + 1, reinterpret_cast<const uint32_t*>(rects), off, block_sums, total);
 }
 
-int gs_launch_count_tiles(hipStream_t stream, int P, int T, int gx, const uint2* rects, uint32_t* tile_count, uint32_t* entries,
-                          uint32_t* entry_n) {
+bool gs_bin_counts_in_projection(int T) { return T <= BIN_MAX_LDS_TILES; }
+int gs_launch_count_tiles_direct(hipStream_t stream, int P, int gx, const uint2* rects, uint32_t* tile_count) {
   if (P <= 0) return 0;
-  if (T <= BIN_MAX_LDS_TILES) {
-    GsProfScope prof(5, stream);
-    hipLaunchKernelGGL(k_count_tiles_lds, dim3((P + BIN_CHUNK - 1) / BIN_CHUNK), dim3(256), (size_t)T * 4, stream, P, T, gx, rects, tile_count,
-                       entries, entry_n);
-  }
-  else
-    hipLaunchKernelGGL(k_count_tiles_direct, dim3((P + 255) / 256), dim3(256), 0, stream, P, gx, rects, tile_count);
+  hipLaunchKernelGGL(k_count_tiles_direct, dim3((P + 255) / 256), dim3(256), 0, stream, P, gx, rects, tile_count);
   return 0;
 }
 
-int gs_launch_binning(hipStream_t stream, int P, int T, int gx, const float* depths, const uint2* rects, const uint32_t* start,
-                      uint32_t* cursor, uint64_t* keys, uint32_t* list, uint32_t capacity, const uint32_t* order, const uint32_t* entries,
-                      const uint32_t* entry_n) {
+int gs_launch_scatter(hipStream_t stream, int P, int T, int gx, const float* depths, const uint2* rects, const uint32_t* start,
+                      uint32_t* cursor, uint64_t* keys, uint32_t capacity, const uint32_t* entries, const uint32_t* entry_n) {
   if (P <= 0 || capacity == 0) return 0;
   if (T <= BIN_MAX_LDS_TILES)
-    hipLaunchKernelGGL(k_scatter_lds, dim3((P + BIN_CHUNK - 1) / BIN_CHUNK), dim3(256), (size_t)T * 4, stream, P, T, gx, depths, rects,
-                       start, cursor, keys, capacity, entries, entry_n);
+    hipLaunchKernelGGL(k_scatter_lds, dim3((P + GS_BIN_GROUP - 1) / GS_BIN_GROUP), dim3(GS_BIN_GROUP), (size_t)T * 4, stream, P, T, gx, depths,
+                       rects, start, cursor, keys, capacity, entries, entry_n);
   else
     hipLaunchKernelGGL(k_scatter_direct, dim3((P + 255) / 256), dim3(256), 0, stream, P, gx, depths, rects, start, cursor, keys, capacity);
-  {
-    GsProfScope prof(4, stream);
-    hipLaunchKernelGGL(k_sort_tiles, dim3(T), dim3(SORT_THREADS), 0, stream, T, start, keys, list, capacity, order);
-  }
   return 0;
 }
+int gs_launch_sort_tiles(hipStream_t stream, int P, int T, const uint32_t* start, uint64_t* keys, uint32_t* list, uint32_t capacity,
+                         const uint32_t* order) {
+  if (P <= 0 || capacity == 0) return 0;
+  GsProfScope prof(4, stream);
+  hipLaunchKernelGGL(k_sort_tiles, dim3(T), dim3(SORT_THREADS), 0, stream, T, start, keys, list, capacity, order);
+  return 0;
+}
diff --git a/instantsplat_amd/csrc/common.h b/instantsplat_amd/csrc/common.h
--- a/instantsplat_amd/csrc/common.h
+++ b/instantsplat_amd/csrc/common.h
@@ -37,6 +37,14 @@
 
 constexpr int GS_BIN_CHUNK = 512;
 constexpr int GS_BIN_ENTRIES = 1024;
+constexpr int GS_BIN_GROUP = 256;
+constexpr int GS_BIN_GROUP_ENTRIES = GS_BIN_ENTRIES / (GS_BIN_CHUNK / GS_BIN_GROUP);
+static_assert(GS_BIN_CHUNK % GS_BIN_GROUP == 0 && GS_BIN_ENTRIES % (GS_BIN_CHUNK / GS_BIN_GROUP) == 0, "whole lists in a chunk's space");
+__host__ __device__ inline size_t gs_bin_n_index(int group, int P) {
+  constexpr int per = GS_BIN_CHUNK / GS_BIN_GROUP;
+  const size_t chunks = ((size_t)(P > 0 ? P : 1) + GS_BIN_CHUNK - 1) / GS_BIN_CHUNK;
+  return (size_t)(group % per) * chunks + (size_t)(group / per);
+}
 
 struct GeomLayout {
   size_t rec, cov3D, rect, clamped, depth, bin_entries, bin_n, total;
@@ -49,7 +57,7 @@
     depth = o; o += gs_align(n * sizeof(float));
     const size_t chunks = (n + GS_BIN_CHUNK - 1) / GS_BIN_CHUNK;
     bin_entries = o; o += gs_align(chunks * GS_BIN_ENTRIES * sizeof(uint32_t));
-    bin_n = o; o += gs_align(chunks * sizeof(uint32_t));
+    bin_n = o; o += gs_align(chunks * (GS_BIN_CHUNK / GS_BIN_GROUP) * sizeof(uint32_t));
     total = o;
   }
 };
@@ -272,6 +280,12 @@
   float* pose_scratch = nullptr;
   float* adam_scratch = nullptr;
 };
+struct GsTileCount {
+  uint32_t* tile_count = nullptr;
+  uint32_t* entries = nullptr;
+  uint32_t* entry_n = nullptr;
+  int T = 0;
+};
 struct GsPosed {
   const float* pose = nullptr;
   float* acc = nullptr;
@@ -298,6 +312,7 @@
 };
 struct GsFrameCtx {
   const GsPrologue* prologue = nullptr;
+  bool counters_clean = false;
   GsPosed posed;
   float* gate = nullptr;
   bool gate_tail = false;
diff --git a/instantsplat_amd/csrc/path.hip b/instantsplat_amd/csrc/path.hip
--- a/instantsplat_amd/csrc/path.hip
+++ b/instantsplat_amd/csrc/path.hip
@@ -102,12 +102,17 @@
   if (n == 0) return MI355GS_OK;
   int rc;
   if ((rc = gs_write_view_consts(stream, t->consts, "view_consts"))) return rc;
+  {
+    const TilesLayout tl(t->W, t->H);
+    if (hipMemsetAsync(t->tiles + tl.count, 0, tl.cursor - tl.count, stream) != hipSuccess) return MI355GS_ELAUNCH;
+  }
   const GsScene scene = t->scene(sh_degree);
   const GsView view = t->view(projmatrix, tanfovx, tanfovy);
   const GsFrameBufs bufs = t->bufs(gs_knobs(), nullptr);
   const size_t frame_bytes = (size_t)t->W * t->H * 3;
   for (int i = first; i < first + n; ++i) {
     GsFrameCtx cx;
+    cx.counters_clean = true;
     cx.posed.pose = poses + 7 * (size_t)i;
     if ((rc = gs_frame_project(stream, scene, view, bufs, cx, t->num_rendered, nullptr, 0))) return rc;
     if ((rc = gs_frame_render(stream, t->P, view, bufs, bg, t->image, false, 0))) return rc;
diff --git a/instantsplat_amd/csrc/preprocess.hip b/instantsplat_amd/csrc/preprocess.hip
--- a/instantsplat_amd/csrc/preprocess.hip
+++ b/instantsplat_amd/csrc/preprocess.hip
@@ -1,4 +1,5 @@
 #include "pose_math.h"
+#include "bin_walk.h"
 
 namespace {
 
@@ -96,7 +97,9 @@
     const float* __restrict__ colors_precomp, const float* __restrict__ opacities, const float* __restrict__ scales,
     const float* __restrict__ rotations, const float* __restrict__ cov3D_precomp, CamParams cp,
     int32_t* __restrict__ radii, GsRec* __restrict__ recs, float* __restrict__ cov3Ds, uint2* __restrict__ rects,
-    uint8_t* __restrict__ clamped, float* __restrict__ depths, uint8_t* __restrict__ visible, GsPosed posed, GsPrologue pro) {
+    uint8_t* __restrict__ clamped, float* __restrict__ depths, uint8_t* __restrict__ visible, GsPosed posed, GsPrologue pro,
+    GsTileCount tc) {
+  HIP_DYNAMIC_SHARED(uint32_t, s_bins)
   const int i = blockIdx.x * blockDim.x + threadIdx.x;
   {
     const size_t gid = (size_t)i, stride = (size_t)gridDim.x * blockDim.x;
@@ -110,124 +113,130 @@
     if (pro.pose_scratch && gid < 32) pro.pose_scratch[gid] = 0.f;
     if (pro.adam_scratch && gid < 8) pro.adam_scratch[gid] = 0.f;
   }
-  if (i >= P) return;
-  radii[i] = 0;
-  if (visible) visible[i] = 0;
-  rects[i] = make_uint2(0u, 0u);
-  const float* view = cp.view;
-  const float* proj = cp.proj;
-  PoseMat pm;
-  if (POSED) pm = load_pose(posed.pose);
-  float3 m = make_float3(means3D[3 * (size_t)i], means3D[3 * (size_t)i + 1], means3D[3 * (size_t)i + 2]);
-  if (POSED) m = pose_mean(pm, m.x, m.y, m.z);
-  const float3 pv = gs_tp43(view, m);
-  if (pv.z <= 0.2f) return;
-  const float4 ph = gs_tp44(proj, m);
-  const float pw = 1.0f / (ph.w + 0.0000001f);
-  const float ndcx = ph.x * pw, ndcy = ph.y * pw;
-
-  float cov[6];
-  if (cov3D_precomp) {
-#pragma unroll
-    for (int k = 0; k < 6; ++k) cov[k] = cov3D_precomp[6 * (size_t)i + k];
-  } else {
-    float4 q = *reinterpret_cast<const float4*>(rotations + 4 * (size_t)i);
-    float sc[3] = {scales[3 * (size_t)i], scales[3 * (size_t)i + 1], scales[3 * (size_t)i + 2]};
-    if (POSED) {
-      q = pose_rot(pm, q);
-#pragma unroll
-      for (int k = 0; k < 3; ++k) sc[k] = pose_scale(sc[k]);
-    }
-    float R[9];
-    quat_to_R(q.x, q.y, q.z, q.w, R);
-    const float s0 = cp.scale_modifier * sc[0], s1 = cp.scale_modifier * sc[1], s2 = cp.scale_modifier * sc[2];
-    float L[9];
-#pragma unroll
-    for (int r = 0; r < 3; ++r) { L[3 * r] = R[3 * r] * s0; L[3 * r + 1] = R[3 * r + 1] * s1; L[3 * r + 2] = R[3 * r + 2] * s2; }
-    cov[0] = L[0] * L[0] + L[1] * L[1] + L[2] * L[2];
-    cov[1] = L[0] * L[3] + L[1] * L[4] + L[2] * L[5];
-    cov[2] = L[0] * L[6] + L[1] * L[7] + L[2] * L[8];
-    cov[3] = L[3] * L[3] + L[4] * L[4] + L[5] * L[5];
-    cov[4] = L[3] * L[6] + L[4] * L[7] + L[5] * L[8];
-    cov[5] = L[6] * L[6] + L[7] * L[7] + L[8] * L[8];
-  }
-#pragma unroll
-  for (int k = 0; k < 6; ++k) cov3Ds[6 * (size_t)i + k] = cov[k];
-
-  const Ewa e = ewa_setup(pv, view, cp);
-  const Cov2D c2 = ewa_cov2d(e, cov);
-  const float det = c2.a * c2.c - c2.b * c2.b;
-  if (det == 0.0f) return;
-  const float det_inv = 1.f / det;
-  const float ca = c2.c * det_inv, cb = -c2.b * det_inv, cc = c2.a * det_inv;
-  const float mid = 0.5f * (c2.a + c2.c);
-  const float sq = sqrtf(fmaxf(0.1f, mid * mid - det));
-  const float radius = ceilf(3.f * sqrtf(fmaxf(mid + sq, mid - sq)));
-  const float px = ((ndcx + 1.0f) * cp.W - 1.0f) * 0.5f, py = ((ndcy + 1.0f) * cp.H - 1.0f) * 0.5f;
-  const int rminx = min(cp.gx, max(0, (int)((px - radius) / GS_TILE)));
-  const int rminy = min(cp.gy, max(0, (int)((py - radius) / GS_TILE)));
-  const int rmaxx = min(cp.gx, max(0, (int)((px + radius + GS_TILE - 1) / GS_TILE)));
-  const int rmaxy = min(cp.gy, max(0, (int)((py + radius + GS_TILE - 1) / GS_TILE)));
-  if ((rmaxx - rminx) * (rmaxy - rminy) == 0) return;
-
-  float3 rgb;
-  uint8_t clamp_bits = 0;
-  if (colors_precomp) {
-    rgb = make_float3(colors_precomp[3 * (size_t)i], colors_precomp[3 * (size_t)i + 1], colors_precomp[3 * (size_t)i + 2]);
-  } else {
-    float dx = m.x - cp.campos[0], dy = m.y - cp.campos[1], dz = m.z - cp.campos[2];
-    const float inv = 1.0f / sqrtf(dx * dx + dy * dy + dz * dz);
-    dx *= inv; dy *= inv; dz *= inv;
-    float3 v;
-    constexpr int NBF = (D + 1) * (D + 1);
-    if (shs_rest == nullptr) {
-      v = sh_eval<NBF>(shs + (size_t)i * M * 3, dx, dy, dz);
+  const uint2 rect = [&]() -> uint2 {
+    const uint2 no_rect = make_uint2(0u, 0u);
+    if (i >= P) return no_rect;
+    radii[i] = 0;
+    if (visible) visible[i] = 0;
+    rects[i] = no_rect;
+    const float* view = cp.view;
+    const float* proj = cp.proj;
+    PoseMat pm;
+    if (POSED) pm = load_pose(posed.pose);
+    float3 m = make_float3(means3D[3 * (size_t)i], means3D[3 * (size_t)i + 1], means3D[3 * (size_t)i + 2]);
+    if (POSED) m = pose_mean(pm, m.x, m.y, m.z);
+    const float3 pv = gs_tp43(view, m);
+    if (pv.z <= 0.2f) return no_rect;
+    const float4 ph = gs_tp44(proj, m);
+    const float pw = 1.0f / (ph.w + 0.0000001f);
+    const float ndcx = ph.x * pw, ndcy = ph.y * pw;
+
+    float cov[6];
+    if (cov3D_precomp) {
+#pragma unroll
+      for (int k = 0; k < 6; ++k) cov[k] = cov3D_precomp[6 * (size_t)i + k];
     } else {
-      float shl[NBF * 3];
-      shl[0] = shs[3 * (size_t)i]; shl[1] = shs[3 * (size_t)i + 1]; shl[2] = shs[3 * (size_t)i + 2];
-      const float* rest = shs_rest + (size_t)i * (M - 1) * 3;
-#pragma unroll
-      for (int k = 3; k < NBF * 3; ++k) shl[k] = rest[k - 3];
-      v = sh_eval<NBF>(shl, dx, dy, dz);
-    }
-    v.x += 0.5f; v.y += 0.5f; v.z += 0.5f;
-    clamp_bits = (uint8_t)((v.x < 0.f ? 1 : 0) | (v.y < 0.f ? 2 : 0) | (v.z < 0.f ? 4 : 0));
-    rgb = make_float3(fmaxf(v.x, 0.f), fmaxf(v.y, 0.f), fmaxf(v.z, 0.f));
-  }
-
-  const float opac = POSED ? pose_opacity(opacities[i]) : opacities[i];
-  float hx, hy;
-  const float tau = __logf(255.0f * opac);
-  const float cdet = ca * cc - cb * cb;
-  if (!(tau > 0.f)) { hx = hy = -1e30f; }
-  else if (!(cdet > 0.f) || ca * cc > 1000.f * cdet) { hx = hy = 1e30f; }
-  else {
-    const float s = 2.f * tau / cdet;
-    hx = sqrtf(s * cc) * 1.01f + 0.5f;
-    hy = sqrtf(s * ca) * 1.01f + 0.5f;
-  }
-
-  radii[i] = (int)radius;
-  if (visible) visible[i] = 1;
-  clamped[i] = clamp_bits;
-  int bminx = rminx, bminy = rminy, bmaxx = rmaxx, bmaxy = rmaxy;
-  if (hx < 1e29f) {
-    if (hx < 0.f) { bmaxx = bminx; bmaxy = bminy; }
+      float4 q = *reinterpret_cast<const float4*>(rotations + 4 * (size_t)i);
+      float sc[3] = {scales[3 * (size_t)i], scales[3 * (size_t)i + 1], scales[3 * (size_t)i + 2]};
+      if (POSED) {
+        q = pose_rot(pm, q);
+#pragma unroll
+        for (int k = 0; k < 3; ++k) sc[k] = pose_scale(sc[k]);
+      }
+      float R[9];
+      quat_to_R(q.x, q.y, q.z, q.w, R);
+      const float s0 = cp.scale_modifier * sc[0], s1 = cp.scale_modifier * sc[1], s2 = cp.scale_modifier * sc[2];
+      float L[9];
+#pragma unroll
+      for (int r = 0; r < 3; ++r) { L[3 * r] = R[3 * r] * s0; L[3 * r + 1] = R[3 * r + 1] * s1; L[3 * r + 2] = R[3 * r + 2] * s2; }
+      cov[0] = L[0] * L[0] + L[1] * L[1] + L[2] * L[2];
+      cov[1] = L[0] * L[3] + L[1] * L[4] + L[2] * L[5];
+      cov[2] = L[0] * L[6] + L[1] * L[7] + L[2] * L[8];
+      cov[3] = L[3] * L[3] + L[4] * L[4] + L[5] * L[5];
+      cov[4] = L[3] * L[6] + L[4] * L[7] + L[5] * L[8];
+      cov[5] = L[6] * L[6] + L[7] * L[7] + L[8] * L[8];
+    }
+#pragma unroll
+    for (int k = 0; k < 6; ++k) cov3Ds[6 * (size_t)i + k] = cov[k];
+
+    const Ewa e = ewa_setup(pv, view, cp);
+    const Cov2D c2 = ewa_cov2d(e, cov);
+    const float det = c2.a * c2.c - c2.b * c2.b;
+    if (det == 0.0f) return no_rect;
+    const float det_inv = 1.f / det;
+    const float ca = c2.c * det_inv, cb = -c2.b * det_inv, cc = c2.a * det_inv;
+    const float mid = 0.5f * (c2.a + c2.c);
+    const float sq = sqrtf(fmaxf(0.1f, mid * mid - det));
+    const float radius = ceilf(3.f * sqrtf(fmaxf(mid + sq, mid - sq)));
+    const float px = ((ndcx + 1.0f) * cp.W - 1.0f) * 0.5f, py = ((ndcy + 1.0f) * cp.H - 1.0f) * 0.5f;
+    const int rminx = min(cp.gx, max(0, (int)((px - radius) / GS_TILE)));
+    const int rminy = min(cp.gy, max(0, (int)((py - radius) / GS_TILE)));
+    const int rmaxx = min(cp.gx, max(0, (int)((px + radius + GS_TILE - 1) / GS_TILE)));
+    const int rmaxy = min(cp.gy, max(0, (int)((py + radius + GS_TILE - 1) / GS_TILE)));
+    if ((rmaxx - rminx) * (rmaxy - rminy) == 0) return no_rect;
+
+    float3 rgb;
+    uint8_t clamp_bits = 0;
+    if (colors_precomp) {
+      rgb = make_float3(colors_precomp[3 * (size_t)i], colors_precomp[3 * (size_t)i + 1], colors_precomp[3 * (size_t)i + 2]);
+    } else {
+      float dx = m.x - cp.campos[0], dy = m.y - cp.campos[1], dz = m.z - cp.campos[2];
+      const float inv = 1.0f / sqrtf(dx * dx + dy * dy + dz * dz);
+      dx *= inv; dy *= inv; dz *= inv;
+      float3 v;
+      constexpr int NBF = (D + 1) * (D + 1);
+      if (shs_rest == nullptr) {
+        v = sh_eval<NBF>(shs + (size_t)i * M * 3, dx, dy, dz);
+      } else {
+        float shl[NBF * 3];
+        shl[0] = shs[3 * (size_t)i]; shl[1] = shs[3 * (size_t)i + 1]; shl[2] = shs[3 * (size_t)i + 2];
+        const float* rest = shs_rest + (size_t)i * (M - 1) * 3;
+#pragma unroll
+        for (int k = 3; k < NBF * 3; ++k) shl[k] = rest[k - 3];
+        v = sh_eval<NBF>(shl, dx, dy, dz);
+      }
+      v.x += 0.5f; v.y += 0.5f; v.z += 0.5f;
+      clamp_bits = (uint8_t)((v.x < 0.f ? 1 : 0) | (v.y < 0.f ? 2 : 0) | (v.z < 0.f ? 4 : 0));
+      rgb = make_float3(fmaxf(v.x, 0.f), fmaxf(v.y, 0.f), fmaxf(v.z, 0.f));
+    }
+
+    const float opac = POSED ? pose_opacity(opacities[i]) : opacities[i];
+    float hx, hy;
+    const float tau = __logf(255.0f * opac);
+    const float cdet = ca * cc - cb * cb;
+    if (!(tau > 0.f)) { hx = hy = -1e30f; }
+    else if (!(cdet > 0.f) || ca * cc > 1000.f * cdet) { hx = hy = 1e30f; }
     else {
-      bminx = max(bminx, (int)floorf((px - hx) * (1.0f / GS_TILE)));
-      bminy = max(bminy, (int)floorf((py - hy) * (1.0f / GS_TILE)));
-      bmaxx = min(bmaxx, (int)floorf((px + hx) * (1.0f / GS_TILE)) + 1);
-      bmaxy = min(bmaxy, (int)floorf((py + hy) * (1.0f / GS_TILE)) + 1);
-      if (bmaxx <= bminx || bmaxy <= bminy) { bmaxx = bminx; bmaxy = bminy; }
-    }
-  }
-  rects[i] = make_uint2((uint32_t)bminx | ((uint32_t)bminy << 16), (uint32_t)bmaxx | ((uint32_t)bmaxy << 16));
-  GsRec rec;
-  rec.q0 = make_float4(px, py, hx, hy);
-  rec.q1 = make_float4(-0.5f * GS_LOG2E * ca, -0.5f * GS_LOG2E * cc, -GS_LOG2E * cb, opac);
-  rec.q2 = make_float4(rgb.x, rgb.y, rgb.z, pv.z);
-  recs[i] = rec;
-  depths[i] = pv.z;
+      const float s = 2.f * tau / cdet;
+      hx = sqrtf(s * cc) * 1.01f + 0.5f;
+      hy = sqrtf(s * ca) * 1.01f + 0.5f;
+    }
+
+    radii[i] = (int)radius;
+    if (visible) visible[i] = 1;
+    clamped[i] = clamp_bits;
+    int bminx = rminx, bminy = rminy, bmaxx = rmaxx, bmaxy = rmaxy;
+    if (hx < 1e29f) {
+      if (hx < 0.f) { bmaxx = bminx; bmaxy = bminy; }
+      else {
+        bminx = max(bminx, (int)floorf((px - hx) * (1.0f / GS_TILE)));
+        bminy = max(bminy, (int)floorf((py - hy) * (1.0f / GS_TILE)));
+        bmaxx = min(bmaxx, (int)floorf((px + hx) * (1.0f / GS_TILE)) + 1);
+        bmaxy = min(bmaxy, (int)floorf((py + hy) * (1.0f / GS_TILE)) + 1);
+        if (bmaxx <= bminx || bmaxy <= bminy) { bmaxx = bminx; bmaxy = bminy; }
+      }
+    }
+    const uint2 r = make_uint2((uint32_t)bminx | ((uint32_t)bminy << 16), (uint32_t)bmaxx | ((uint32_t)bmaxy << 16));
+    rects[i] = r;
+    GsRec rec;
+    rec.q0 = make_float4(px, py, hx, hy);
+    rec.q1 = make_float4(-0.5f * GS_LOG2E * ca, -0.5f * GS_LOG2E * cc, -GS_LOG2E * cb, opac);
+    rec.q2 = make_float4(rgb.x, rgb.y, rgb.z, pv.z);
+    recs[i] = rec;
+    depths[i] = pv.z;
+    return r;
+  }();
+  if (tc.tile_count) gs_count_group(tc, P, cp.gx, i, rect, s_bins);
 }
 
 template <int NB>
@@ -506,13 +515,14 @@
                              const float* colors_precomp, const float* opacities, const float* scales,
                              const float* rotations, const float* cov3D_precomp, const CamParams& cp, int32_t* radii,
                              GsRec* recs, float* cov3Ds, uint2* rects, uint8_t* clamped, float* depths, uint8_t* visible,
-                             const GsPosed& posed_args, const GsPrologue& pro) {
+                             const GsPosed& posed_args, const GsPrologue& pro, const GsTileCount& tc) {
   if (P <= 0) return 0;
+  const size_t lds = tc.tile_count ? (size_t)tc.T * 4 : 0;
   const bool posed = posed_args.pose != nullptr;
   const GsPosed pa = posed ? posed_args : GsPosed();
 #define GS_FWD(POSED, DEG)                                                                                                              \
-  hipLaunchKernelGGL((k_preprocess_fwd<POSED, DEG>), dim3((P + 255) / 256), dim3(256), 0, stream, P, M, means3D, shs, shs_rest,         \
-                     colors_precomp, opacities, scales, rotations, cov3D_precomp, cp, radii, recs, cov3Ds, rects, clamped, depths, visible, pa, pro)
+  hipLaunchKernelGGL((k_preprocess_fwd<POSED, DEG>), dim3((P + 255) / 256), dim3(256), lds, stream, P, M, means3D, shs, shs_rest,       \
+                     colors_precomp, opacities, scales, rotations, cov3D_precomp, cp, radii, recs, cov3Ds, rects, clamped, depths, visible, pa, pro, tc)
   const int deg = shs ? D : 0;
   if (posed) { if (deg == 0) GS_FWD(true, 0); else if (deg == 1) GS_FWD(true, 1); else if (deg == 2) GS_FWD(true, 2); else GS_FWD(true, 3); }
   else { if (deg == 0) GS_FWD(false, 0); else if (deg == 1) GS_FWD(false, 1); else if (deg == 2) GS_FWD(false, 2); else GS_FWD(false, 3); }
diff --git a/instantsplat_amd/csrc/tracker.hip b/instantsplat_amd/csrc/tracker.hip
--- a/instantsplat_amd/csrc/tracker.hip
+++ b/instantsplat_amd/csrc/tracker.hip
@@ -159,6 +159,8 @@
 
 int ensure_consts(Tracker* t, hipStream_t stream) {
   if (t->consts_ready) return MI355GS_OK;
+  const TilesLayout tl(t->W, t->H);
+  if (hipMemsetAsync(t->tiles + tl.count, 0, tl.cursor - tl.count, stream) != hipSuccess) return MI355GS_ELAUNCH;
   const int rc = gs_write_view_consts(stream, t->consts, "tracker_consts");
   t->consts_ready = rc == MI355GS_OK;
   return rc;
@@ -197,6 +199,7 @@
   int rc;
   if ((rc = ensure_consts(t, stream))) return rc;
   GsFrameCtx cx;
+  cx.counters_clean = true;
   cx.posed.pose = pose;
   return gs_frame_project(stream, t->scene(sh_degree), t->view(projmatrix, tanfovx, tanfovy), t->bufs(t->knobs, nullptr), cx, count_out,
                           nullptr, 0);
@@ -222,9 +225,10 @@
   const GsFrameBufs bufs = t->bufs(t->knobs, t->grad_scratch);
   GsPrologue pro;
   pro.grad_records = (float4*)t->grad_scratch; pro.n_vec = (size_t)P * 3;
-  pro.tile_counters = (uint32_t*)(t->tiles + tl.count); pro.n_counters = (int)((tl.start - tl.count) / 4);
+  pro.tile_counters = (uint32_t*)(t->tiles + tl.cursor); pro.n_counters = (int)((tl.start - tl.cursor) / 4);
   GsFrameCtx cx;
   cx.prologue = &pro;
+  cx.counters_clean = true;
   cx.posed.pose = state + MI355GS_TRACKER_POSE;
   cx.posed.acc = t->pose_partial;
   cx.posed.partial = t->pose_partial;
diff --git a/instantsplat_amd/csrc/trainer.hip b/instantsplat_amd/csrc/trainer.hip
--- a/instantsplat_amd/csrc/trainer.hip
+++ b/instantsplat_amd/csrc/trainer.hip
@@ -172,18 +172,21 @@
     if (int rc = gs_write_view_consts(stream, t->consts, "trainer_consts")) return rc;
     if (hipMemsetAsync(t->g_frest, 0, (size_t)P * 45 * sizeof(float), stream) != hipSuccess) return MI355GS_ELAUNCH;
     if (hipMemsetAsync(t->adam_live, 0, 16 * sizeof(uint32_t), stream) != hipSuccess) return MI355GS_ELAUNCH;
+    const TilesLayout tl0(W, H);
+    if (hipMemsetAsync(t->tiles + tl0.count, 0, tl0.cursor - tl0.count, stream) != hipSuccess) return MI355GS_ELAUNCH;
     t->consts_ready = true;
   }
   GsPrologue pro;
   {
     const TilesLayout tl(W, H);
     pro.grad_records = (float4*)t->grad_scratch; pro.n_vec = (size_t)P * 3;
-    pro.tile_counters = (uint32_t*)(t->tiles + tl.count); pro.n_counters = (int)((tl.start - tl.count) / 4);
+    pro.tile_counters = (uint32_t*)(t->tiles + tl.cursor); pro.n_counters = (int)((tl.start - tl.cursor) / 4);
     pro.g_poses = t->g_poses; pro.n_pose = 7 * t->V; pro.pose_scratch = t->pose_scratch; pro.adam_scratch = t->adam_scratch;
   }
   const float* pose = t->poses + 7 * (size_t)view;
   GsFrameCtx cx;
   cx.prologue = &pro;
+  cx.counters_clean = true;
   cx.posed.pose = pose; cx.posed.acc = t->pose_scratch; cx.posed.partial = t->pose_partial;
   cx.gate = t->adam_scratch;
   const int D = sh_degree;
```

After: 3575 (median of 6 runs). Within noise of the previous version (+1.0%).
